# RUCAIBox/RecBole-CDR

Measured on AMD Instinct MI355X. Metric: training interactions/sec, higher is better.
Workload: dtype f32; 1 GPU; C5: EMCDR-BPR D=128, 50000000 users x 10000000 items/domain (union tables 71.7 GB fp32), step = source batch + target batch of 1048576 triples each per rank, fwd+bwd+row-wise adam; batch_per_domain_per_rank=1048576, k_neg=1, optimizer=rowwise-adam

## Files before the change

include/cdr_hip.h:

```cpp
#ifndef CDR_HIP_H
#define CDR_HIP_H

#include <stddef.h>
#include <stdint.h>

#ifdef __cplusplus
extern "C" {
#endif

#define CDR_OK 0
#define CDR_EINVAL (-1)
#define CDR_ENOMEM (-2)
#define CDR_ENODEV (-3)

typedef struct cdr_ctx cdr_ctx;

int cdr_ctx_create(int device, cdr_ctx** out);
int cdr_ctx_destroy(cdr_ctx* ctx);
const char* cdr_last_error(void);
int cdr_ctx_scrub_next(cdr_ctx* ctx, void* ptr, size_t bytes);
int cdr_ctx_set_id_counters(cdr_ctx* ctx, uint32_t* user_counts, int64_t user_rows, uint32_t* item_counts, int64_t item_rows,
                            void* list_ws, size_t list_ws_bytes);
int cdr_id_count_workspace_bytes(int64_t B, size_t* bytes);
int cdr_norm_rec_floats(void);
int cdr_row_norms_build(void* stream, const float* table, int64_t rows, int D, float* n2);
int cdr_ctx_set_norm_cache(cdr_ctx* ctx, float* user_n2, int64_t user_rows, float* item_n2, int64_t item_rows);
#define CDR_ABI_VERSION 64
int cdr_abi_version(void);

#define CDR_TAG_BPR_FWD 1
#define CDR_TAG_POINT_FWD 2
#define CDR_TAG_BPR_FWD_GRAD 3
#define CDR_TAG_APPLY_UNSIGNED 4
#define CDR_TAG_APPLY_SIGNED 5
#define CDR_TAG_SORT 6
#define CDR_TAG_POINT_FWD_GRAD 7
#define CDR_TAG_BPR_PARTIAL_DIFF 8
#define CDR_TAG_BPR_GRAD_FROM_DIFF 9
#define CDR_TAG_POINT_PARTIAL_DOT 10
#define CDR_TAG_POINT_GRAD_FROM_DOT 11
#define CDR_TAG_CONET_FWD 12
#define CDR_TAG_CONET_BWD 13
#define CDR_TAG_BPR_FWD_KMAJOR 15
#define CDR_TAG_MAP_STEP 16
#define CDR_TAG_CONET_WGRAD 14
#define CDR_TAG_OCC_FLAGS 17
#define CDR_TAG_BPR_FWD_APPLY 18
#define CDR_TAG_BATCH_NORMS 19
#define CDR_TAG_CONET_FB 20
#define CDR_TAG_TRIPLET_FWD_GRAD 21
#define CDR_TAG_CLFM_FWD_GRAD 22
#define CDR_TAG_DTCDR_FWD_GRAD 23
#define CDR_TAG_DEEPAPF_FWD_GRAD 24
#define CDR_TAG_DCDCSR_MAP_FWD_GRAD 25
int cdr_timing_enable(cdr_ctx* ctx, int capacity);
int cdr_timing_collect(cdr_ctx* ctx, int* tags, float* ms, int max_n, int* n_out);

int cdr_bpr_fwd(cdr_ctx* ctx, void* stream,
                const float* user_tab, const float* item_tab, int D,
                const int64_t* uid, const int64_t* pid, const int64_t* nid, int64_t B,
                float gamma, float reg_weight,
                float* out4, float* gcoef );

int cdr_bpr_bwd_dense(cdr_ctx* ctx, void* stream,
                      const float* user_tab, const float* item_tab, int D,
                      const int64_t* uid, const int64_t* pid, const int64_t* nid, int64_t B,
                      const float* gcoef, const float* out4, float reg_weight, const float* grad_out,
                      float* grad_user_tab, float* grad_item_tab);

#define CDR_LOSS_MSE 0
#define CDR_LOSS_BCE 1
int cdr_point_fwd(cdr_ctx* ctx, void* stream, int loss_kind,
                  const float* user_tab, const float* item_tab,
                  const float* reg_user_tab, const float* reg_item_tab, int D,
                  const int64_t* uid, const int64_t* iid, const float* label, int64_t B,
                  float reg_weight, float* out4, float* gcoef, float* scores);

int cdr_point_bwd_dense(cdr_ctx* ctx, void* stream,
                        const float* user_tab, const float* item_tab,
                        const float* reg_user_tab, const float* reg_item_tab, int D,
                        const int64_t* uid, const int64_t* iid, int64_t B,
                        const float* gcoef, const float* out4, float reg_weight, const float* grad_out,
                        float* grad_user_tab, float* grad_item_tab,
                        float* grad_reg_user_tab, float* grad_reg_item_tab);
int cdr_point_fwd_pair(cdr_ctx* ctx, void* stream, int loss_kind, const float* const* user_tab, const float* const* item_tab,
                       const float* const* reg_user_tab, const float* const* reg_item_tab, int D, const int64_t* const* uid,
                       const int64_t* const* iid, const float* const* label, const int64_t* B, const float* reg_weight,
                       float* const* out4, float* const* gcoef, float* const* scores, const float* w, float* total);
int cdr_point_fwd_pair_ex(cdr_ctx* ctx, void* stream, int loss_kind, const float* const* user_tab, const float* const* item_tab,
                          const float* const* reg_user_tab, const float* const* reg_item_tab, int D, int reg_D, const int64_t* const* uid,
                          const int64_t* const* iid, const float* const* label, const int64_t* B, const float* reg_weight,
                          float* const* out4, float* const* gcoef, float* const* scores, const float* w, float* total);
int cdr_point_bwd_dense_pair(cdr_ctx* ctx, void* stream, const float* const* user_tab, const float* const* item_tab,
                             const float* const* reg_user_tab, const float* const* reg_item_tab, int D, const int64_t* const* uid,
                             const int64_t* const* iid, const int64_t* B, const float* const* gcoef, const float* const* out4,
                             const float* reg_weight, const float* const* grad_out, const float* grad_scale,
                             float* const* grad_user_tab, float* const* grad_item_tab, float* const* grad_reg_user_tab,
                             float* const* grad_reg_item_tab);

int cdr_gather_rows(void* stream, const float* tab, int D, const int64_t* ids, int64_t n, float* out);
int cdr_scatter_add_rows(void* stream, float* grad_tab, int D, const int64_t* ids, int64_t n,
                         const float* src, const float* scale);
int cdr_gather_rows_multi(void* stream, int count, const float* const* tabs, int D, const int64_t* const* ids, const int64_t* n,
                          float* const* outs, int64_t* bump_counter);
int cdr_scatter_add_rows_multi(void* stream, int count, float* const* grad_tabs, int D, const int64_t* const* ids, const int64_t* n,
                               const float* const* srcs);

int cdr_select_mapped(void* stream, const float* mapped, const float* tab, int D,
                      const int64_t* ids, int64_t n, int64_t n_overlap, float* out);

#define CDR_ACT_NONE 0
#define CDR_ACT_TANH 1
#define CDR_ACT_RELU 2
#define CDR_ACT_SIGMOID 3
int cdr_gemm_f32(void* stream, int transA, int transB, int64_t M, int64_t N, int64_t K,
                 const float* A, int64_t lda, const float* B, int64_t ldb,
                 float* C, int64_t ldc, const float* bias, int act, int accumulate);

int cdr_fullsort_scores_f32(void* stream, const float* user_e, int64_t U, int D,
                            const float* slab0, int64_t n0, const float* slab1, int64_t n1,
                            float* scores );

int cdr_fullsort_topk_workspace_bytes(int64_t U, int D, int64_t n0, int64_t n1, int k, size_t* bytes);
int cdr_fullsort_topk_f32(void* stream, const float* user_e, int64_t U, int D,
                          const float* slab0, int64_t n0, const float* slab1, int64_t n1, int k,
                          const int64_t* hist_indptr, const int64_t* hist_cols, int exclude_first_col,
                          float* out_vals , int64_t* out_idx , void* workspace, size_t workspace_bytes);

int cdr_fullsort_neg_sqdist_f32(void* stream, const float* user_e, int64_t U, int D,
                                const float* items, int64_t N, float* norm_scratch, float* scores);

int cdr_row_sqnorm_f32(void* stream, const float* X, int64_t rows, int D, float* out );

int cdr_fullsort_neg_sqdist_topk_workspace_bytes(int64_t U, int D, int64_t n0, int64_t n1, int k, size_t* bytes);
int cdr_fullsort_neg_sqdist_topk_f32(void* stream, const float* user_e, int64_t U, int D,
                                     const float* slab0, int64_t n0, const float* slab1, int64_t n1,
                                     const float* col_sqnorm, int k,
                                     const int64_t* hist_indptr, const int64_t* hist_cols, int exclude_first_col,
                                     float* out_vals , int64_t* out_idx , void* workspace, size_t workspace_bytes);

int cdr_fullsort_rank_workspace_bytes(int64_t U, int D, int64_t n0, int64_t n1, int64_t P, size_t* bytes);
int cdr_fullsort_rank_f32(void* stream, const float* user_e, int64_t U, int D,
                          const float* slab0, int64_t n0, const float* slab1, int64_t n1,
                          const int64_t* pos_indptr , const int64_t* pos_cols ,
                          const int64_t* hist_indptr, const int64_t* hist_cols, int exclude_first_col,
                          float* pos_score , int32_t* gt, int32_t* eq, int32_t* eq_before ,
                          int32_t* n_unmasked , void* workspace, size_t workspace_bytes);
int cdr_fullsort_neg_sqdist_rank_workspace_bytes(int64_t U, int D, int64_t n0, int64_t n1, int64_t P, size_t* bytes);
int cdr_fullsort_neg_sqdist_rank_f32(void* stream, const float* user_e, int64_t U, int D,
                                     const float* slab0, int64_t n0, const float* slab1, int64_t n1, const float* col_sqnorm,
                                     const int64_t* pos_indptr , const int64_t* pos_cols ,
                                     const int64_t* hist_indptr, const int64_t* hist_cols, int exclude_first_col,
                                     float* pos_score , int32_t* gt, int32_t* eq, int32_t* eq_before ,
                                     int32_t* n_unmasked , void* workspace, size_t workspace_bytes);
int cdr_rank_rows_f32(void* stream, const float* scores, int64_t ld, int64_t U, int64_t N, int64_t col_off,
                      const int64_t* pos_indptr, const int64_t* pos_cols, const int64_t* hist_indptr, const int64_t* hist_cols,
                      int exclude_first_col, const float* pos_score, int32_t* gt, int32_t* eq, int32_t* eq_before,
                      int32_t* n_unmasked, int accumulate);

int cdr_fullsort_topk_wide_workspace_bytes(int64_t U, int D, int64_t n0, int64_t n1, int k, size_t* bytes);
int cdr_fullsort_topk_wide_f32(void* stream, const float* user_e, int64_t U, int D,
                               const float* slab0, int64_t n0, const float* slab1, int64_t n1, int k,
                               const int64_t* hist_indptr, const int64_t* hist_cols, int exclude_first_col,
                               float* out_vals , int64_t* out_idx , void* workspace, size_t workspace_bytes);
int cdr_fullsort_neg_sqdist_topk_wide_workspace_bytes(int64_t U, int D, int64_t n0, int64_t n1, int k, size_t* bytes);
int cdr_fullsort_neg_sqdist_topk_wide_f32(void* stream, const float* user_e, int64_t U, int D,
                                          const float* slab0, int64_t n0, const float* slab1, int64_t n1,
                                          const float* col_sqnorm, int k,
                                          const int64_t* hist_indptr, const int64_t* hist_cols, int exclude_first_col,
                                          float* out_vals , int64_t* out_idx , void* workspace, size_t workspace_bytes);
int cdr_topk_rows_workspace_bytes(int64_t U, int64_t N, int k, size_t* bytes);
int cdr_topk_rows_f32(void* stream, const float* scores, int64_t ld, int64_t U, int64_t N, int64_t col_off, int k,
                      const int64_t* hist_indptr, const int64_t* hist_cols, int exclude_first_col,
                      float* vals , int64_t* idx , int accumulate, void* workspace, size_t workspace_bytes);

int cdr_candidate_scores_f32(void* stream, const float* user_e, int64_t U, int D,
                             const float* slab0, int64_t n0, const float* slab1, int64_t n1,
                             const int64_t* cand_row , const int64_t* cand_cols , int64_t C, int form,
                             float* scores );
// ... 511 lines not shown
```

recbole-cdr_amd/binding.py:

```python
import contextlib
import ctypes
import gc
import os
import subprocess
import threading

import torch


@contextlib.contextmanager
def capturing(graph, stream):
    gc.collect()
    was = gc.isenabled()
    gc.disable()
    try:
        with torch.cuda.graph(graph, stream=stream):
            yield
    finally:
        if was:
            gc.enable()


_HERE = os.path.dirname(os.path.abspath(__file__))
_LIB_PATH = os.environ.get('CDR_LIB_PATH') or os.path.join(_HERE, 'lib', 'libcdrhip.so')
ABI_VERSION = 64
SIGNIN_WORDS = 288

CDR_LOSS_MSE, CDR_LOSS_BCE = 0, 1
ACT_NONE, ACT_TANH, ACT_RELU, ACT_SIGMOID = 0, 1, 2, 3


class NativeLibraryError(RuntimeError):
    pass


def lib_path():
    return _LIB_PATH


def build(force=False):
    csrc = os.path.join(_HERE, 'csrc')
    cmd = ['make', '-C', csrc, '-j', str(min(8, os.cpu_count() or 1))]
    if force:
        subprocess.run(['make', '-C', csrc, 'clean'], check=True, stdout=subprocess.DEVNULL)
    r = subprocess.run(cmd, stdout=subprocess.PIPE, stderr=subprocess.STDOUT, text=True)
    if r.returncode != 0:
        raise NativeLibraryError('building libcdrhip.so failed:\n' + r.stdout[-4000:])
    return _LIB_PATH


_c_i64, _c_int, _c_f32, _c_ptr = ctypes.c_int64, ctypes.c_int, ctypes.c_float, ctypes.c_void_p

_SIGNATURES = {
    'cdr_ctx_create': [_c_int, ctypes.POINTER(_c_ptr)],
    'cdr_ctx_destroy': [_c_ptr],
    'cdr_abi_version': [],
    'cdr_ctx_scrub_next': [_c_ptr, _c_ptr, ctypes.c_size_t],
    'cdr_ctx_set_id_counters': [_c_ptr, _c_ptr, _c_i64, _c_ptr, _c_i64, _c_ptr, ctypes.c_size_t],
    'cdr_id_count_workspace_bytes': [_c_i64, ctypes.POINTER(ctypes.c_size_t)],
    'cdr_norm_rec_floats': [],
    'cdr_row_norms_build': [_c_ptr, _c_ptr, _c_i64, _c_int, _c_ptr],
    'cdr_ctx_set_norm_cache': [_c_ptr, _c_ptr, _c_i64, _c_ptr, _c_i64],
    'cdr_bpr_fwd': [_c_ptr, _c_ptr, _c_ptr, _c_ptr, _c_int, _c_ptr, _c_ptr, _c_ptr, _c_i64, _c_f32, _c_f32, _c_ptr, _c_ptr],
    'cdr_bpr_bwd_dense': [_c_ptr, _c_ptr, _c_ptr, _c_ptr, _c_int, _c_ptr, _c_ptr, _c_ptr, _c_i64, _c_ptr, _c_ptr, _c_f32,
                          _c_ptr, _c_ptr, _c_ptr],
    'cdr_point_fwd': [_c_ptr, _c_ptr, _c_int, _c_ptr, _c_ptr, _c_ptr, _c_ptr, _c_int, _c_ptr, _c_ptr, _c_ptr, _c_i64,
                      _c_f32, _c_ptr, _c_ptr, _c_ptr],
    'cdr_point_bwd_dense': [_c_ptr, _c_ptr, _c_ptr, _c_ptr, _c_ptr, _c_ptr, _c_int, _c_ptr, _c_ptr, _c_i64, _c_ptr, _c_ptr,
                            _c_f32, _c_ptr, _c_ptr, _c_ptr, _c_ptr, _c_ptr],
    'cdr_gather_rows': [_c_ptr, _c_ptr, _c_int, _c_ptr, _c_i64, _c_ptr],
    'cdr_gather_rows_multi': [_c_ptr, _c_int, _c_ptr, _c_int, _c_ptr, _c_ptr, _c_ptr, _c_ptr],
    'cdr_scatter_add_rows_multi': [_c_ptr, _c_int, _c_ptr, _c_int, _c_ptr, _c_ptr, _c_ptr],
    'cdr_sscdr_map_loss': [_c_ptr, _c_ptr, _c_ptr, _c_ptr, _c_i64, _c_int, _c_f32, _c_f32, _c_f32, _c_ptr, _c_ptr, _c_ptr],
    'cdr_scale2_unless_one': [_c_ptr, _c_ptr, _c_ptr, _c_i64, _c_ptr, _c_i64],
    'cdr_scatter_add_rows': [_c_ptr, _c_ptr, _c_int, _c_ptr, _c_i64, _c_ptr, _c_ptr],
    'cdr_select_mapped': [_c_ptr, _c_ptr, _c_ptr, _c_int, _c_ptr, _c_i64, _c_i64, _c_ptr],
    'cdr_gemm_f32': [_c_ptr, _c_int, _c_int, _c_i64, _c_i64, _c_i64, _c_ptr, _c_i64, _c_ptr, _c_i64, _c_ptr, _c_i64, _c_ptr,
                     _c_int, _c_int],
    'cdr_fullsort_scores_f32': [_c_ptr, _c_ptr, _c_i64, _c_int, _c_ptr, _c_i64, _c_ptr, _c_i64, _c_ptr],
    'cdr_fullsort_neg_sqdist_f32': [_c_ptr, _c_ptr, _c_i64, _c_int, _c_ptr, _c_i64, _c_ptr, _c_ptr],
    'cdr_act_bwd': [_c_ptr, _c_int, _c_ptr, _c_ptr, _c_ptr, _c_i64],
    'cdr_colsum': [_c_ptr, _c_ptr, _c_ptr, _c_i64, _c_i64, _c_ptr, _c_int],
    'cdr_linear_wgrad_small': [_c_ptr, _c_ptr, _c_ptr, _c_ptr, _c_int, _c_ptr, _c_i64, _c_int, _c_int, _c_ptr, _c_ptr, _c_ptr, ctypes.c_size_t],
    'cdr_linear_wgrad_small_workspace': [_c_i64, _c_int, _c_int, ctypes.POINTER(ctypes.c_size_t)],
    'cdr_linear_small': [_c_ptr, _c_int, _c_ptr, _c_i64, _c_ptr, _c_i64, _c_i64, _c_int, _c_int, _c_ptr, _c_int, _c_ptr, _c_i64, _c_ptr, _c_int],
    'cdr_mse_fwd': [_c_ptr, _c_ptr, _c_ptr, _c_ptr, _c_i64, _c_ptr],
    'cdr_mse_bwd': [_c_ptr, _c_ptr, _c_ptr, _c_i64, _c_ptr, _c_ptr, _c_ptr],
    'cdr_bpr_fwd_grad': [_c_ptr, _c_ptr, _c_ptr, _c_ptr, _c_int, _c_ptr, _c_ptr, _c_ptr, _c_i64, _c_i64, _c_f32, _c_f32, _c_ptr,
                         _c_ptr, _c_ptr, _c_int],
    'cdr_loss_finish_sums': [_c_ptr, _c_ptr, _c_i64, _c_f32, _c_ptr],
    'cdr_triplet_fwd_grad': [_c_ptr, _c_ptr, _c_ptr, _c_ptr, _c_int, _c_ptr, _c_ptr, _c_ptr, _c_i64, _c_f32, _c_f32, _c_ptr, _c_ptr, _c_ptr],
    'cdr_clfm_fwd_grad_workspace_bytes': [_c_i64, _c_int, _c_int, ctypes.POINTER(ctypes.c_size_t)],
    'cdr_clfm_fwd_grad': [_c_ptr, _c_ptr, _c_ptr, _c_ptr, _c_int, _c_int, _c_ptr, _c_ptr, _c_ptr, _c_ptr, _c_i64, _c_f32, _c_f32, _c_ptr, _c_ptr,
                          _c_ptr, _c_ptr, _c_ptr, ctypes.c_size_t],
    'cdr_dtcdr_fwd_grad_workspace_bytes': [_c_i64, _c_int, _c_int, _c_ptr, ctypes.POINTER(ctypes.c_size_t)],
    'cdr_dtcdr_fwd_grad': [_c_ptr, _c_ptr, _c_ptr, _c_ptr, _c_ptr, _c_ptr, _c_int, _c_int, _c_ptr, _c_ptr, _c_ptr, _c_ptr, _c_ptr, _c_i64,
                           _c_f32, _c_f32, _c_ptr, ctypes.c_uint64, _c_i64, _c_ptr, _c_ptr, _c_ptr, _c_ptr, _c_ptr, _c_ptr, _c_ptr,
                           ctypes.c_size_t],
    'cdr_deepapf_fwd_grad_workspace_bytes': [_c_i64, _c_int, ctypes.POINTER(ctypes.c_size_t)],
    'cdr_deepapf_fwd_grad': [_c_ptr, _c_ptr, _c_ptr, _c_ptr, _c_ptr, _c_int, _c_ptr, _c_ptr, _c_ptr, _c_ptr, _c_i64, _c_i64, _c_f32, _c_i64,
                             _c_ptr, _c_ptr, _c_ptr, _c_ptr, _c_ptr, _c_ptr, ctypes.c_size_t],
    'cdr_dcdcsr_map_fwd_grad_workspace_bytes': [_c_i64, _c_int, ctypes.POINTER(_c_int), ctypes.POINTER(ctypes.c_size_t)],
    'cdr_dcdcsr_map_fwd_grad': [_c_ptr, _c_ptr, _c_ptr, _c_ptr, _c_ptr, _c_i64, _c_int, ctypes.POINTER(_c_int), _c_ptr, _c_ptr, _c_ptr, _c_ptr,
                                _c_ptr, ctypes.c_size_t],
    'cdr_bpr_step_fused_heads_words': [_c_i64, ctypes.POINTER(_c_i64)],
    'cdr_bpr_step_fused_kmajor_sizes': [_c_i64, _c_int, ctypes.POINTER(_c_i64), ctypes.POINTER(_c_i64)],
    'cdr_bpr_step_fused_kmajor': [_c_ptr, _c_ptr, _c_int, _c_ptr, _c_ptr, _c_ptr, _c_i64, _c_ptr, _c_ptr, _c_ptr, _c_i64, _c_int,
                                  _c_ptr, _c_ptr, _c_ptr, _c_i64, _c_int, _c_f32, _c_f32, _c_f32, _c_f32, _c_f32, _c_f32, _c_f32, _c_i64, _c_i64,
                                  _c_ptr, _c_ptr, _c_ptr, _c_ptr, _c_ptr, _c_ptr, _c_ptr, _c_ptr, ctypes.c_size_t],
    'cdr_bpr_step_fused': [_c_ptr, _c_ptr, _c_int, _c_ptr, _c_ptr, _c_ptr, _c_i64, _c_ptr, _c_ptr, _c_ptr, _c_i64, _c_int,
                           _c_ptr, _c_ptr, _c_ptr, _c_i64, _c_f32, _c_f32, _c_f32, _c_f32, _c_f32, _c_f32, _c_f32, _c_i64, _c_i64,
                           _c_ptr, _c_ptr, _c_ptr, _c_ptr, _c_ptr, _c_ptr, _c_ptr, _c_ptr, ctypes.c_size_t],
    'cdr_bpr_step_fused_dev': [_c_ptr, _c_ptr, _c_int, _c_ptr, _c_ptr, _c_ptr, _c_i64, _c_ptr, _c_ptr, _c_ptr, _c_i64, _c_int,
                               _c_ptr, _c_ptr, _c_ptr, _c_i64, _c_f32, _c_f32, _c_f32, _c_f32, _c_f32, _c_f32, _c_f32, _c_ptr, _c_ptr, _c_ptr,
                               _c_ptr, _c_ptr, _c_ptr, _c_ptr, _c_ptr, _c_ptr, _c_ptr, _c_ptr, ctypes.c_size_t],
    'cdr_bpr_step_presort': [_c_ptr, _c_ptr, _c_ptr, _c_ptr, _c_ptr, _c_i64, _c_i64, _c_i64, _c_ptr, _c_ptr, _c_ptr, _c_ptr, _c_ptr,
                             ctypes.c_size_t, _c_ptr],
    'cdr_bpr_step_from_diff': [_c_ptr, _c_ptr, _c_int, _c_ptr, _c_ptr, _c_ptr, _c_ptr, _c_ptr, _c_ptr, _c_int, _c_ptr, _c_ptr, _c_ptr, _c_i64,
                               _c_f32, _c_f32, _c_f32, _c_f32, _c_f32, _c_f32, _c_f32, _c_i64, _c_i64, _c_ptr, ctypes.c_uint32, _c_ptr, _c_ptr,
                               _c_ptr, _c_ptr, _c_ptr, _c_ptr, _c_ptr],
    'cdr_batch_norm_sums': [_c_ptr, _c_ptr, _c_ptr, _c_ptr, _c_int, _c_ptr, _c_ptr, _c_i64, _c_ptr],
    'cdr_bpr_shard_local_step': [_c_ptr, _c_ptr, _c_int, _c_ptr, _c_ptr, _c_ptr, _c_i64, _c_ptr, _c_int, _c_ptr, _c_ptr, _c_ptr, _c_i64, _c_i64,
                                 _c_f32, _c_f32, _c_f32, _c_f32, _c_f32, _c_f32, _c_f32, _c_i64, _c_ptr, _c_ptr, _c_ptr, _c_ptr, _c_ptr,
                                 _c_ptr, _c_ptr, _c_ptr, ctypes.c_size_t],
    'cdr_route_triples_workspace_bytes': [_c_i64, _c_int, ctypes.POINTER(ctypes.c_size_t)],
    'cdr_route_triples': [_c_ptr, _c_ptr, _c_ptr, _c_ptr, _c_ptr, _c_i64, _c_int, _c_ptr, _c_ptr, _c_ptr, ctypes.c_size_t],
    'cdr_bpr_shard_plan_sizes': [_c_i64, _c_i64, _c_i64, _c_int, ctypes.POINTER(_c_i64), ctypes.POINTER(ctypes.c_size_t)],
    'cdr_bpr_shard_plan': [_c_ptr, _c_ptr, _c_ptr, _c_i64, _c_i64, _c_i64, _c_int, _c_ptr, _c_ptr, _c_ptr, _c_ptr, _c_ptr, _c_ptr, _c_ptr, _c_ptr,
                           _c_ptr, _c_ptr, _c_ptr, ctypes.c_size_t],
    'cdr_gather_rows_norms': [_c_ptr, _c_ptr, _c_int, _c_ptr, _c_i64, _c_ptr, _c_ptr],
    'cdr_shard_norm_sums': [_c_ptr, _c_ptr, _c_ptr, _c_int, _c_ptr, _c_ptr, _c_ptr, _c_i64, _c_ptr],
    'cdr_bpr_shard_step': [_c_ptr, _c_ptr, _c_int, _c_ptr, _c_ptr, _c_ptr, _c_ptr, _c_int, _c_ptr, _c_ptr, _c_i64, _c_i64, _c_f32, _c_f32, _c_f32,
                           _c_f32, _c_f32, _c_f32, _c_f32, _c_i64, _c_ptr, _c_ptr, _c_ptr, _c_ptr, _c_ptr, _c_ptr, _c_ptr, _c_ptr, _c_ptr],
    'cdr_shard_owner_apply': [_c_ptr, _c_ptr, _c_int, _c_ptr, _c_ptr, _c_ptr, _c_i64, _c_int, _c_ptr, _c_i64, _c_int, _c_ptr, _c_f32, _c_f32, _c_f32,
                              _c_f32, _c_f32, _c_i64, _c_ptr, _c_ptr, _c_ptr, ctypes.c_size_t],
    'cdr_overlap_remap_dev_workspace_bytes': [_c_i64, _c_i64, ctypes.POINTER(ctypes.c_size_t)],
    'cdr_overlap_remap_dev': [_c_ptr, _c_ptr, _c_ptr, _c_ptr, _c_i64, _c_ptr, _c_ptr, _c_ptr, _c_i64, _c_ptr, _c_ptr, _c_ptr, _c_ptr,
                              ctypes.c_size_t, _c_ptr],
    'cdr_point_step_fused': [_c_ptr, _c_ptr, _c_int, _c_int, _c_ptr, _c_ptr, _c_ptr, _c_i64, _c_ptr, _c_ptr, _c_ptr, _c_i64, _c_int, _c_ptr, _c_ptr,
                             _c_ptr, _c_i64, _c_f32, _c_f32, _c_f32, _c_f32, _c_f32, _c_f32, _c_i64, _c_i64, _c_ptr, _c_ptr, _c_ptr, _c_ptr, _c_ptr,
                             _c_ptr, _c_ptr, _c_ptr, ctypes.c_size_t],
    'cdr_point_step_fused_pair_dev': [_c_ptr, _c_ptr, _c_int, _c_int, _c_ptr, _c_ptr, _c_ptr, _c_i64, _c_ptr, _c_ptr, _c_ptr, _c_i64, _c_int,
                                      _c_ptr, _c_ptr, _c_ptr, _c_i64, _c_ptr, _c_ptr, _c_ptr, _c_i64, _c_f32, _c_f32, _c_f32, _c_f32, _c_f32,
                                      _c_f32, _c_f32, _c_f32, _c_ptr, _c_ptr, _c_ptr, _c_ptr, _c_ptr, _c_ptr, _c_ptr, _c_ptr, _c_ptr, _c_ptr,
                                      _c_ptr, ctypes.c_size_t],
    'cdr_point_step_fused_pair': [_c_ptr, _c_ptr, _c_int, _c_int, _c_ptr, _c_ptr, _c_ptr, _c_i64, _c_ptr, _c_ptr, _c_ptr, _c_i64, _c_int,
                                  _c_ptr, _c_ptr, _c_ptr, _c_i64, _c_ptr, _c_ptr, _c_ptr, _c_i64, _c_f32, _c_f32, _c_f32, _c_f32, _c_f32,
                                  _c_f32, _c_ptr, _c_ptr, _c_ptr, _c_ptr, _c_ptr, _c_ptr, _c_ptr, _c_ptr, ctypes.c_size_t],
    'cdr_point_step_fused_kmajor': [_c_ptr, _c_ptr, _c_int, _c_int, _c_ptr, _c_ptr, _c_ptr, _c_i64, _c_ptr, _c_ptr, _c_ptr, _c_i64, _c_int, _c_ptr,
                                    _c_ptr, _c_ptr, _c_i64, _c_int, _c_f32, _c_f32, _c_f32, _c_f32, _c_f32, _c_f32, _c_i64, _c_i64, _c_ptr, _c_ptr, _c_ptr,
                                    _c_ptr, _c_ptr, _c_ptr, _c_ptr, _c_ptr, ctypes.c_size_t],
    'cdr_point_step_presort': [_c_ptr, _c_ptr, _c_ptr, _c_ptr, _c_i64, _c_i64, _c_i64, _c_ptr, _c_ptr, _c_ptr, _c_ptr, _c_ptr, ctypes.c_size_t, _c_ptr],
    'cdr_point_step_from_dot': [_c_ptr, _c_ptr, _c_int, _c_int, _c_ptr, _c_ptr, _c_ptr, _c_ptr, _c_ptr, _c_ptr, _c_int, _c_ptr, _c_ptr, _c_ptr, _c_i64,
                                _c_f32, _c_f32, _c_f32, _c_f32, _c_f32, _c_f32, _c_i64, _c_i64, _c_ptr, ctypes.c_uint32, _c_ptr, _c_ptr, _c_ptr,
                                _c_ptr, _c_ptr, _c_ptr, _c_ptr],
    'cdr_sort_workspace_bytes': [_c_i64, _c_i64, ctypes.POINTER(ctypes.c_size_t)],
    'cdr_timing_enable': [_c_ptr, _c_int],
    'cdr_timing_collect': [_c_ptr, ctypes.POINTER(_c_int), ctypes.POINTER(_c_f32), _c_int, ctypes.POINTER(_c_int)],
    'cdr_sort_ids': [_c_ptr, _c_ptr, _c_ptr, _c_i64, _c_ptr, _c_i64, _c_i64, _c_ptr, _c_ptr, _c_ptr, ctypes.c_size_t],
    'cdr_rowwise_apply': [_c_ptr, _c_ptr, _c_int, _c_ptr, _c_ptr, _c_ptr, _c_int, _c_ptr, _c_ptr, _c_i64, _c_ptr, _c_i64, _c_i64,
                          _c_ptr, _c_f32, _c_f32, _c_f32, _c_f32, _c_f32, _c_i64, _c_ptr, ctypes.c_uint32],
    'cdr_sort_ids_two_tables': [_c_ptr, _c_ptr, _c_ptr, _c_i64, _c_i64, _c_ptr, _c_i64, _c_ptr, _c_i64, _c_i64, _c_ptr, _c_ptr, _c_ptr,
                                _c_ptr, ctypes.c_size_t],
    'cdr_gemm_f32_ex': [_c_ptr, _c_int, _c_int, _c_i64, _c_i64, _c_i64, _c_ptr, _c_i64, _c_ptr, _c_i64, _c_ptr, _c_i64, _c_ptr,
                        _c_ptr, _c_int, _c_int],
    'cdr_gather_rows_ld': [_c_ptr, _c_ptr, _c_int, _c_ptr, _c_i64, _c_ptr, _c_i64],
    'cdr_scatter_add_rows_ld': [_c_ptr, _c_ptr, _c_int, _c_ptr, _c_i64, _c_ptr, _c_i64],
    'cdr_scatter_rows_sorted': [_c_ptr, _c_ptr, _c_int, _c_ptr, _c_ptr, _c_i64, _c_ptr, _c_i64],
    'cdr_ordered_bwd': [_c_ptr, _c_int, _c_ptr, _c_int],
    'cdr_overlap_mask': [_c_ptr, _c_ptr, _c_i64, _c_i64, _c_ptr],
    'cdr_rowscale': [_c_ptr, _c_ptr, _c_ptr, _c_i64, _c_i64, _c_ptr],
    'cdr_bcast_add_act': [_c_ptr, _c_ptr, _c_ptr, _c_i64, _c_i64, _c_int, _c_ptr],
    'cdr_bce_prob_fwd': [_c_ptr, _c_ptr, _c_ptr, _c_ptr, _c_i64, _c_ptr],
    'cdr_bce_prob_bwd': [_c_ptr, _c_ptr, _c_ptr, _c_i64, _c_ptr, _c_ptr],
    'cdr_frobenius_fwd': [_c_ptr, _c_ptr, _c_ptr, _c_i64, _c_ptr],
    'cdr_frobenius_bwd': [_c_ptr, _c_ptr, _c_i64, _c_ptr, _c_ptr, _c_ptr, _c_int],
    'cdr_sqnorm_normalize_fwd': [_c_ptr, _c_ptr, _c_i64, _c_int, _c_ptr, _c_ptr],
    'cdr_sqnorm_normalize_bwd': [_c_ptr, _c_ptr, _c_ptr, _c_ptr, _c_i64, _c_int, _c_ptr],
    'cdr_triplet_fwd': [_c_ptr, _c_ptr, _c_ptr, _c_ptr, _c_ptr, _c_i64, _c_int, _c_f32, _c_f32, _c_ptr, _c_ptr, _c_ptr],
    'cdr_triplet_bwd': [_c_ptr, _c_ptr, _c_ptr, _c_ptr, _c_i64, _c_int, _c_f32, _c_f32, _c_ptr, _c_ptr, _c_ptr, _c_ptr, _c_ptr,
                        _c_ptr],
    'cdr_spmm_csr_f32': [_c_ptr, _c_ptr, _c_ptr, _c_ptr, _c_i64, _c_ptr, _c_int, _c_ptr],
    'cdr_graph_layer_fwd': [_c_ptr, _c_ptr, _c_ptr, _c_ptr, _c_i64, _c_ptr, _c_int, _c_ptr, _c_ptr, _c_ptr],
    'cdr_graph_layer_bwd': [_c_ptr, _c_ptr, _c_ptr, _c_ptr, _c_i64, _c_ptr, _c_ptr, _c_ptr, _c_int, _c_ptr, _c_ptr, _c_ptr],
    'cdr_row_flags': [_c_ptr, _c_int, _c_ptr, _c_ptr, _c_ptr, _c_i64, _c_ptr, ctypes.c_size_t],
    'cdr_row_flags_layout': [_c_i64, _c_ptr],
    'cdr_graph_layer_fwd_rows': [_c_ptr, _c_ptr, _c_ptr, _c_ptr, _c_i64, _c_ptr, _c_ptr, _c_int, _c_ptr, _c_ptr],
    'cdr_mul_one_plus': [_c_ptr, _c_ptr, _c_ptr, _c_i64, _c_ptr],
    'cdr_graph_layer_bwd_rows': [_c_ptr, _c_ptr, _c_ptr, _c_ptr, _c_i64, _c_ptr, _c_ptr, _c_ptr, _c_int, _c_ptr],
    'cdr_transfer_fwd': [_c_ptr, _c_ptr, _c_ptr, _c_ptr, _c_ptr, _c_i64, _c_int, _c_i64, _c_f32, _c_f32, _c_ptr, _c_ptr],
    'cdr_transfer_bwd': [_c_ptr, _c_ptr, _c_ptr, _c_ptr, _c_ptr, _c_i64, _c_int, _c_i64, _c_f32, _c_f32, _c_ptr, _c_ptr],
    'cdr_bitgcf_mix_fwd': [_c_ptr] * 7 + [_c_i64, _c_i64, _c_int, _c_i64, _c_i64, _c_f32, _c_f32, _c_f32, ctypes.c_uint64, _c_ptr, ctypes.c_uint64,
                           ctypes.c_uint64, _c_ptr, _c_ptr, _c_ptr, _c_ptr, _c_i64, _c_ptr, _c_ptr, _c_ptr],
    'cdr_bitgcf_mix_bwd': [_c_ptr] * 7 + [_c_i64, _c_ptr, _c_ptr, _c_ptr, _c_ptr, _c_ptr, _c_ptr, _c_i64, _c_i64, _c_int, _c_i64, _c_i64, _c_f32, _c_f32,
                           _c_f32, ctypes.c_uint64, _c_ptr, ctypes.c_uint64, ctypes.c_uint64, _c_ptr, _c_ptr, _c_ptr],
    'cdr_transfer_drop_fwd': [_c_ptr, _c_ptr, _c_ptr, _c_ptr, _c_ptr, _c_i64, _c_int, _c_i64, _c_f32, _c_f32, _c_f32, ctypes.c_uint64, _c_ptr,
                              ctypes.c_uint64, ctypes.c_uint64, _c_i64, _c_ptr, _c_ptr],
    'cdr_transfer_drop_bwd': [_c_ptr, _c_ptr, _c_ptr, _c_ptr, _c_ptr, _c_i64, _c_int, _c_i64, _c_f32, _c_f32, _c_f32, ctypes.c_uint64, _c_ptr,
                              ctypes.c_uint64, ctypes.c_uint64, _c_i64, _c_ptr, _c_ptr],
    'cdr_l2_normalize_fwd': [_c_ptr, _c_ptr, _c_i64, _c_int, _c_ptr, _c_i64, _c_ptr],
    'cdr_l2_normalize_bwd': [_c_ptr, _c_ptr, _c_ptr, _c_ptr, _c_i64, _c_i64, _c_int, _c_ptr, _c_int],
    'cdr_copy_cols': [_c_ptr, _c_ptr, _c_i64, _c_i64, _c_int, _c_ptr, _c_i64, _c_int],
    'cdr_bitgcf_stack': [_c_ptr] * 5 + [_c_i64, _c_i64, _c_int, _c_ptr, _c_ptr, _c_ptr, _c_ptr, _c_i64],
    'cdr_bitgcf_unstack_bwd': [_c_ptr, _c_ptr, _c_ptr, _c_i64, _c_i64, _c_int, _c_ptr, _c_ptr],
    'cdr_colblock_mean_fwd': [_c_ptr, _c_ptr, _c_i64, _c_int, _c_int, _c_ptr],
    'cdr_colblock_mean_bwd': [_c_ptr, _c_ptr, _c_i64, _c_int, _c_int, _c_ptr],
    'cdr_dropout_dev': [_c_ptr, _c_ptr, _c_i64, _c_f32, _c_ptr, ctypes.c_uint64, _c_ptr],
    'cdr_gather_max2': [_c_ptr, _c_ptr, _c_ptr, _c_int, _c_ptr, _c_i64, _c_ptr, _c_i64],
    'cdr_gather_max2_bwd': [_c_ptr, _c_ptr, _c_ptr, _c_int, _c_ptr, _c_i64, _c_ptr, _c_i64, _c_ptr, _c_ptr],
    'cdr_apf_prod': [_c_ptr, _c_ptr, _c_ptr, _c_ptr, _c_i64, _c_int, _c_ptr],
    'cdr_apf_prod_bwd': [_c_ptr, _c_ptr, _c_ptr, _c_ptr, _c_ptr, _c_i64, _c_int, _c_ptr, _c_ptr, _c_ptr],
    'cdr_apf_combine': [_c_ptr, _c_ptr, _c_ptr, _c_ptr, _c_ptr, _c_ptr, _c_ptr, _c_i64, _c_i64, _c_int, _c_ptr, _c_ptr],
    'cdr_apf_combine_bwd': [_c_ptr, _c_ptr, _c_ptr, _c_ptr, _c_ptr, _c_ptr, _c_ptr, _c_ptr, _c_i64, _c_int, _c_ptr, _c_ptr, _c_ptr,
                            _c_ptr, _c_ptr],
    'cdr_maxmin_norm': [_c_ptr, _c_ptr, _c_i64, _c_int, _c_ptr, _c_ptr],
# ... 288 lines not shown
```

recbole-cdr_amd/csrc/cdr_common.h:

```cpp
#pragma once
#include <hip/hip_runtime.h>
#include <stdint.h>
#include <stdio.h>
#include "../../include/cdr_hip.h"

#define CDR_WAVE 64
#define CDR_NUM_CU 256
#define CDR_MAX_PARTIAL_BLOCKS 4096
#define CDR_PARTIAL_STRIDE 8
#define CDR_TICKETS 1024
constexpr int kBlock = 256;

struct cdr_ctx {
    int device;
    double* partials;
    unsigned* tickets;
    void* scratch;
    size_t scratch_bytes;
    void* scrub_ptr;
    size_t scrub_bytes;
    uint32_t* idc_user; int64_t idc_user_rows;
    uint32_t* idc_item; int64_t idc_item_rows;
    void* idc_list; size_t idc_list_bytes;
    float* n2_user; int64_t n2_user_rows;
    float* n2_item; int64_t n2_item_rows;
    unsigned long long* conet_tab_dev; unsigned long long* conet_tab_pin; unsigned long long* conet_tab_shadow; int conet_tab_cap, conet_tab_n;
    int conet_defer, conet_pending, conet_fin_grid;
    int64_t conet_fin_ns, conet_fin_R;
    float* conet_fin_out;
    void* conet_fin_stream;
    int timing_cap, timing_n;
    hipEvent_t* ev0;
    hipEvent_t* ev1;
    int* tags;
};

struct cdr_time_scope {
    cdr_ctx* c; hipStream_t s; int slot;
    cdr_time_scope(cdr_ctx* ctx, int tag, hipStream_t st) : c(ctx), s(st), slot(-1) {
        if (c && c->timing_cap > 0 && c->timing_n < c->timing_cap) {
            slot = c->timing_n++;
            c->tags[slot] = tag;
            (void)hipEventRecord(c->ev0[slot], s);
        }
    }
    ~cdr_time_scope() { if (slot >= 0) (void)hipEventRecord(c->ev1[slot], s); }
};

void cdr_set_error(const char* fmt, ...);
int cdr_ctx_scratch(cdr_ctx* ctx, size_t bytes, void** out);

#define CDR_CHECK_ARG(cond)                                                         \
    do {                                                                            \
        if (!(cond)) {                                                              \
            cdr_set_error("%s: invalid argument: %s", __func__, #cond);             \
            return CDR_EINVAL;                                                      \
        }                                                                           \
    } while (0)

#define CDR_HIP(expr)                                                               \
    do {                                                                            \
        hipError_t e_ = (expr);                                                     \
        if (e_ != hipSuccess) {                                                     \
            cdr_set_error("%s: %s -> %s", __func__, #expr, hipGetErrorString(e_));  \
            return (int)e_;                                                         \
        }                                                                           \
    } while (0)

#define CDR_LAUNCH_CHECK()                                                          \
    do {                                                                            \
        hipError_t e_ = hipGetLastError();                                          \
        if (e_ != hipSuccess) {                                                     \
            cdr_set_error("%s: launch failed: %s", __func__, hipGetErrorString(e_));\
            return (int)e_;                                                         \
        }                                                                           \
    } while (0)

template <int CTRL>
__device__ __forceinline__ float dpp_add_(float v) {
    return v + __int_as_float(__builtin_amdgcn_update_dpp(0, __float_as_int(v), CTRL, 0xF, 0xF, true));
}
template <int LPR>
__device__ __forceinline__ float group_sum(float v) {
    if (LPR >= 2) v = dpp_add_<0xB1>(v);
    if (LPR >= 4) v = dpp_add_<0x4E>(v);
    if (LPR >= 8) v = dpp_add_<0x141>(v);
    if (LPR >= 16) v = dpp_add_<0x140>(v);
    if (LPR >= 32) {
        const auto r = __builtin_amdgcn_permlane16_swap(__float_as_uint(v), __float_as_uint(v), false, false);
        v = __uint_as_float(r[0]) + __uint_as_float(r[1]);
    }
    if (LPR >= 64) {
        const auto r = __builtin_amdgcn_permlane32_swap(__float_as_uint(v), __float_as_uint(v), false, false);
        v = __uint_as_float(r[0]) + __uint_as_float(r[1]);
    }
    return v;
}

__device__ __forceinline__ double wave_sum_d(double v) {
#pragma unroll
    for (int off = 32; off > 0; off >>= 1) v += __shfl_xor(v, off, CDR_WAVE);
    return v;
}

template <int NV>
__device__ __forceinline__ void block_sum_d(double (&v)[NV], double* smem) {
    const int lane = threadIdx.x & 63, wave = threadIdx.x >> 6, nw = blockDim.x >> 6;
#pragma unroll
    for (int i = 0; i < NV; ++i) v[i] = wave_sum_d(v[i]);
    if (lane == 0) {
#pragma unroll
        for (int i = 0; i < NV; ++i) smem[wave * NV + i] = v[i];
    }
    __syncthreads();
    if (threadIdx.x == 0) {
#pragma unroll
        for (int i = 0; i < NV; ++i) {
            double s = 0.0;
            for (int w = 0; w < nw; ++w) s += smem[w * NV + i];
            v[i] = s;
        }
    }
}

static __global__ void cdr_zero_u32_kernel(uint32_t* __restrict__ p, int64_t n) {
    for (int64_t i = (int64_t)blockIdx.x * blockDim.x + threadIdx.x; i < n; i += (int64_t)gridDim.x * blockDim.x) p[i] = 0u;
}
static inline hipError_t cdr_zero_u32(void* p, int64_t n_words, hipStream_t s) {
    int64_t g = (n_words + 255) / 256;
    if (g > 1024) g = 1024;
    if (g < 1) g = 1;
    cdr_zero_u32_kernel<<<dim3((unsigned)g), dim3(256), 0, s>>>((uint32_t*)p, n_words);
    return hipGetLastError();
}

#if defined(__HIP_DEVICE_COMPILE__) && !defined(__gfx950__)
#error "cdr_common.h: the fence-free partial hand-over (cdr_sign_in_last) is only valid on gfx950; add __threadfence() pairs for another target"
#endif
__device__ __forceinline__ void cdr_store_sys(double* p, double v) { __hip_atomic_store(p, v, __ATOMIC_RELAXED, __HIP_MEMORY_SCOPE_SYSTEM); }
__device__ __forceinline__ double cdr_load_sys(const double* p) { return __hip_atomic_load(p, __ATOMIC_RELAXED, __HIP_MEMORY_SCOPE_SYSTEM); }
__device__ __forceinline__ bool cdr_sign_in_last(unsigned* ticket, unsigned nblocks) {
    __shared__ int cdr_last_flag_;
    asm volatile("s_waitcnt vmcnt(0)" ::: "memory");
    __syncthreads();
    if (threadIdx.x == 0) cdr_last_flag_ = atomicInc(ticket, nblocks - 1) == nblocks - 1 ? 1 : 0;
    __syncthreads();
    return cdr_last_flag_ != 0;
}
constexpr unsigned kSignGroups = 8, kSignStride = 32;
__device__ __forceinline__ bool cdr_sign_in_last_wide(unsigned* ticket, unsigned nblocks) {
    __shared__ int cdr_last_flag_w_;
    asm volatile("s_waitcnt vmcnt(0)" ::: "memory");
    __syncthreads();
    if (threadIdx.x == 0) {
        const unsigned bid = blockIdx.y * gridDim.x + blockIdx.x;
        const unsigned K = nblocks < kSignGroups ? nblocks : kSignGroups;
        const unsigned g = bid % K, ng = (nblocks - g + K - 1) / K;
        int last = 0;
        if (atomicInc(ticket + kSignStride * (1 + g), ng - 1) == ng - 1) last = atomicInc(ticket, K - 1) == K - 1 ? 1 : 0;
        cdr_last_flag_w_ = last;
    }
    __syncthreads();
    return cdr_last_flag_w_ != 0;
}
__device__ __forceinline__ void cdr_scrub(uint4* __restrict__ z, int64_t n16) {
    if (!z) return;
    const int64_t nth = (int64_t)gridDim.x * gridDim.y * blockDim.x;
    const int64_t me = ((int64_t)blockIdx.y * gridDim.x + blockIdx.x) * blockDim.x + threadIdx.x;
    const uint4 zero = make_uint4(0u, 0u, 0u, 0u);
    for (int64_t i = me; i < n16; i += nth) z[i] = zero;
}
static inline void cdr_take_scrub(cdr_ctx* ctx, uint4** z, int64_t* n16) {
    *z = (uint4*)ctx->scrub_ptr; *n16 = (int64_t)(ctx->scrub_bytes / 16);
    ctx->scrub_ptr = nullptr; ctx->scrub_bytes = 0;
}
constexpr int kSignInMaxBlocks = 512;

__device__ __forceinline__ float4 ld4(const float* p) { return *reinterpret_cast<const float4*>(p); }
// ... 65 lines not shown
```

recbole-cdr_amd/csrc/cdr_ctx.hip:

```cpp
#include <stdarg.h>
#include <string.h>
#include "cdr_common.h"
#include <stdlib.h>

static thread_local char g_err[512] = "";

void cdr_set_error(const char* fmt, ...) {
    va_list ap;
    va_start(ap, fmt);
    vsnprintf(g_err, sizeof(g_err), fmt, ap);
    va_end(ap);
}

extern "C" const char* cdr_last_error(void) { return g_err; }
extern "C" int cdr_abi_version(void) { return CDR_ABI_VERSION; }

extern "C" int cdr_ctx_create(int device, cdr_ctx** out) {
    CDR_CHECK_ARG(out != nullptr);
    *out = nullptr;
    int ndev = 0;
    if (hipGetDeviceCount(&ndev) != hipSuccess || device < 0 || device >= ndev) {
        cdr_set_error("cdr_ctx_create: device %d not available (%d visible)", device, ndev);
        return CDR_ENODEV;
    }
    int prev = 0;
    CDR_HIP(hipGetDevice(&prev));
    CDR_HIP(hipSetDevice(device));
    cdr_ctx* c = new cdr_ctx();
    c->device = device;
    c->timing_cap = c->timing_n = 0;
    c->ev0 = c->ev1 = nullptr;
    c->tags = nullptr;
    c->scratch = nullptr;
    c->scratch_bytes = 0;
    c->scrub_ptr = nullptr; c->scrub_bytes = 0;
    c->idc_user = c->idc_item = nullptr; c->idc_user_rows = c->idc_item_rows = 0; c->idc_list = nullptr; c->idc_list_bytes = 0;
    c->n2_user = c->n2_item = nullptr; c->n2_user_rows = c->n2_item_rows = 0;
    c->partials = nullptr;
    c->tickets = nullptr;
    hipError_t e = hipMalloc(&c->partials, sizeof(double) * CDR_MAX_PARTIAL_BLOCKS * CDR_PARTIAL_STRIDE);
    if (e == hipSuccess) e = hipMalloc(&c->tickets, sizeof(unsigned) * CDR_TICKETS);
    if (e == hipSuccess) e = hipMemset(c->tickets, 0, sizeof(unsigned) * CDR_TICKETS);
    (void)hipSetDevice(prev);
    if (e != hipSuccess) {
        if (c->partials) (void)hipFree(c->partials);
        if (c->tickets) (void)hipFree(c->tickets);
        delete c;
        cdr_set_error("cdr_ctx_create: scratch allocation failed: %s", hipGetErrorString(e));
        return CDR_ENOMEM;
    }
    *out = c;
    return CDR_OK;
}

int cdr_ctx_scratch(cdr_ctx* ctx, size_t bytes, void** out) {
    if (ctx->scratch_bytes < bytes) {
        int prev = 0;
        CDR_HIP(hipGetDevice(&prev));
        CDR_HIP(hipSetDevice(ctx->device));
        if (ctx->scratch) (void)hipFree(ctx->scratch);
        ctx->scratch = nullptr; ctx->scratch_bytes = 0;
        const size_t want = bytes + bytes / 4;
        hipError_t e = hipMalloc(&ctx->scratch, want);
        (void)hipSetDevice(prev);
        if (e != hipSuccess) { cdr_set_error("cdr_ctx_scratch: %zu bytes: %s", want, hipGetErrorString(e)); return CDR_ENOMEM; }
        ctx->scratch_bytes = want;
    }
    *out = ctx->scratch;
    return CDR_OK;
}

extern "C" int cdr_timing_enable(cdr_ctx* ctx, int capacity) {
    CDR_CHECK_ARG(ctx && capacity >= 0);
    for (int i = 0; i < ctx->timing_cap; ++i) { (void)hipEventDestroy(ctx->ev0[i]); (void)hipEventDestroy(ctx->ev1[i]); }
    delete[] ctx->ev0; delete[] ctx->ev1; delete[] ctx->tags;
    ctx->ev0 = ctx->ev1 = nullptr; ctx->tags = nullptr;
    ctx->timing_cap = ctx->timing_n = 0;
    if (capacity == 0) return CDR_OK;
    ctx->ev0 = new hipEvent_t[capacity];
    ctx->ev1 = new hipEvent_t[capacity];
    ctx->tags = new int[capacity];
    for (int i = 0; i < capacity; ++i) { CDR_HIP(hipEventCreate(&ctx->ev0[i])); CDR_HIP(hipEventCreate(&ctx->ev1[i])); }
    ctx->timing_cap = capacity;
    return CDR_OK;
}

extern "C" int cdr_timing_collect(cdr_ctx* ctx, int* tags, float* ms, int max_n, int* n_out) {
    CDR_CHECK_ARG(ctx && tags && ms && n_out && max_n >= 0);
    int n = ctx->timing_n < max_n ? ctx->timing_n : max_n;
    for (int i = 0; i < n; ++i) {
        CDR_HIP(hipEventSynchronize(ctx->ev1[i]));
        CDR_HIP(hipEventElapsedTime(&ms[i], ctx->ev0[i], ctx->ev1[i]));
        tags[i] = ctx->tags[i];
    }
    *n_out = n;
    ctx->timing_n = 0;
    return CDR_OK;
}

extern "C" int cdr_ctx_destroy(cdr_ctx* ctx) {
    if (!ctx) return CDR_OK;
    cdr_timing_enable(ctx, 0);
    if (ctx->partials) (void)hipFree(ctx->partials);
    if (ctx->tickets) (void)hipFree(ctx->tickets);
    if (ctx->scratch) (void)hipFree(ctx->scratch);
    if (ctx->conet_tab_dev) (void)hipFree(ctx->conet_tab_dev);
    if (ctx->conet_tab_pin) (void)hipHostFree(ctx->conet_tab_pin);
    free(ctx->conet_tab_shadow);
    delete ctx;
    return CDR_OK;
}

extern "C" int cdr_ctx_scrub_next(cdr_ctx* ctx, void* ptr, size_t bytes) {
    CDR_CHECK_ARG(ctx && ptr && bytes > 0 && (bytes & 15) == 0 && ((uintptr_t)ptr & 15) == 0);
    ctx->scrub_ptr = ptr; ctx->scrub_bytes = bytes;
    return CDR_OK;
}

extern "C" int cdr_ctx_set_id_counters(cdr_ctx* ctx, uint32_t* user_counts, int64_t user_rows, uint32_t* item_counts, int64_t item_rows,
                                       void* list_ws, size_t list_ws_bytes) {
    CDR_CHECK_ARG(ctx != nullptr);
    if (!user_counts || !item_counts || !list_ws) {
        ctx->idc_user = ctx->idc_item = nullptr; ctx->idc_user_rows = ctx->idc_item_rows = 0; ctx->idc_list = nullptr; ctx->idc_list_bytes = 0;
        return CDR_OK;
    }
    CDR_CHECK_ARG(user_rows > 0 && item_rows > 0 && list_ws_bytes > 0);
    ctx->idc_user = user_counts; ctx->idc_user_rows = user_rows; ctx->idc_item = item_counts; ctx->idc_item_rows = item_rows;
    ctx->idc_list = list_ws; ctx->idc_list_bytes = list_ws_bytes;
    return CDR_OK;
}

extern "C" int cdr_ctx_set_norm_cache(cdr_ctx* ctx, float* user_n2, int64_t user_rows, float* item_n2, int64_t item_rows) {
    CDR_CHECK_ARG(ctx != nullptr);
    if (!user_n2 || !item_n2) {
        ctx->n2_user = ctx->n2_item = nullptr; ctx->n2_user_rows = ctx->n2_item_rows = 0;
        return CDR_OK;
    }
    const uintptr_t rec = (uintptr_t)cdr_norm_rec_floats() * sizeof(float);
    CDR_CHECK_ARG(user_rows > 0 && item_rows > 0 && (uintptr_t)user_n2 % rec == 0 && (uintptr_t)item_n2 % rec == 0);
    ctx->n2_user = user_n2; ctx->n2_user_rows = user_rows; ctx->n2_item = item_n2; ctx->n2_item_rows = item_rows;
    return CDR_OK;
}
```

recbole-cdr_amd/csrc/cdr_step.hip:

```cpp
#include <cstdlib>
#include <cstring>
#include <string.h>
#include <rocprim/device/device_radix_sort.hpp>
#include <rocprim/device/device_scan.hpp>
#include <rocprim/iterator/counting_iterator.hpp>
#include <rocprim/iterator/transform_iterator.hpp>
#include "cdr_common.h"
#include "cdr_adam_math.h"
#include "cdr_opt_math.h"
#include "cdr_loss_math.h"

namespace {

constexpr int kUnroll = 4;

#ifndef CDR_NORM_REC_FLOATS
#define CDR_NORM_REC_FLOATS 16
#endif
constexpr int kNormRecFloats = CDR_NORM_REC_FLOATS;
static_assert(kNormRecFloats == 16 || kNormRecFloats == 32, "a record is one 64-byte or one 128-byte burst");

template <int LPR>
__device__ __forceinline__ float sqnorm4(float4 a) {
    if constexpr (LPR >= 32) {
// ... 112 lines not shown
                v[r] = ld4n<(LPR >= 32)>(I + ii[r] * D + 4 * sub);
            }
        }
#pragma unroll
        for (int r = 0; r < kUnroll; ++r) {
            const int64_t t = base + (int64_t)r * TG;
            const float dx = group_sum<LPR>(dot4(u[r], v[r]));
            const float su = group_sum<LPR>(dot4(u[r], u[r]));
            const float si = group_sum<LPR>(dot4(v[r], v[r]));
            if (t < B) {
                const float y = yl[r];
                float l, g;
                if (loss_kind == CDR_LOSS_MSE) {
                    const float d = dx - y;
                    l = d * d; g = 2.0f * d * invB;
                } else {
                    const float p = sigmoidf_(dx);
                    l = (y - 1.0f) * fmaxf(logf(1.0f - p), -100.0f) - y * fmaxf(logf(p), -100.0f);
                    const float pq = (1.0f - p) * p;
                    g = (p - y) / fmaxf(pq, 1e-12f) * invB * pq;
                }
                if (live) {
                    st4n<(LPR >= 32)>(GU + t * D + 4 * sub, make_float4(g * v[r].x, g * v[r].y, g * v[r].z, g * v[r].w));
                    st4n<(LPR >= 32)>(GI + t * D + 4 * sub, make_float4(g * u[r].x, g * u[r].y, g * u[r].z, g * u[r].w));
                }
                if (sub == 0) { acc[0] += (double)l; acc[1] += (double)su; acc[2] += (double)si; }
            }
        }
    }
    block_sum_d<3>(acc, smem);
    if (threadIdx.x == 0) store_partials(partials, acc);
}

template <int LPR>
__device__ __forceinline__ float4 sqnorm_bwd4(float4 x, float4 g, float L) {
    const float d = group_sum<LPR>(dot4(x, g));
    return make_float4(sqnorm_bwd_elem(x.x, g.x, L, d), sqnorm_bwd_elem(x.y, g.y, L, d), sqnorm_bwd_elem(x.z, g.z, L, d),
                       sqnorm_bwd_elem(x.w, g.w, L, d));
}

template <int LPR>
__global__ __launch_bounds__(kBlock) void triplet_fwd_grad_kernel(const float* __restrict__ U, const float* __restrict__ I, int D,
                                                                  const int64_t* __restrict__ uid, const int64_t* __restrict__ pid,
                                                                  const int64_t* __restrict__ nid, int64_t B, float margin, float eps,
                                                                  float invB, float* __restrict__ GU, float* __restrict__ GI,
                                                                  double* __restrict__ partials) {
    constexpr int GPB = kBlock / LPR;
    __shared__ double smem[2 * (kBlock / 64)];
    const int sub = threadIdx.x % LPR;
    const int64_t gg = (int64_t)blockIdx.x * GPB + threadIdx.x / LPR;
    const int64_t TG = (int64_t)gridDim.x * GPB;
    const int D4 = D >> 2;
    double acc[2] = {0.0, 0.0};
    const bool live = sub < D4;
    const float e = live ? eps : 0.f;

    for (int64_t base = gg; base < B; base += TG * kUnroll) {
        float4 u[kUnroll], p[kUnroll], n[kUnroll];
        int64_t iu[kUnroll], ip[kUnroll], in[kUnroll];
#pragma unroll
        for (int r = 0; r < kUnroll; ++r) {
            const int64_t t = base + (int64_t)r * TG;
            const int64_t tc = t < B ? t : B - 1;
            iu[r] = uid[tc]; ip[r] = pid[tc]; in[r] = nid[tc];
        }
#pragma unroll
        for (int r = 0; r < kUnroll; ++r) {
            const int64_t t = base + (int64_t)r * TG;
            u[r] = p[r] = n[r] = make_float4(0.f, 0.f, 0.f, 0.f);
            if (t < B && live) {
                u[r] = ld4n<(LPR >= 32)>(U + iu[r] * D + 4 * sub);
                p[r] = ld4n<(LPR >= 32)>(I + ip[r] * D + 4 * sub);
                n[r] = ld4n<(LPR >= 32)>(I + in[r] * D + 4 * sub);
            }
        }
#pragma unroll
        for (int r = 0; r < kUnroll; ++r) {
            const int64_t t = base + (int64_t)r * TG;
            const float Lu = group_sum<LPR>(dot4(u[r], u[r]));
            const float Lp = group_sum<LPR>(dot4(p[r], p[r]));
            const float Ln = group_sum<LPR>(dot4(n[r], n[r]));
            const float su = sqnorm_scale(Lu), sp = sqnorm_scale(Lp), sn = sqnorm_scale(Ln);
            const float4 yu = make_float4(u[r].x / su, u[r].y / su, u[r].z / su, u[r].w / su);
            const float4 dp = make_float4(yu.x - p[r].x / sp + e, yu.y - p[r].y / sp + e, yu.z - p[r].z / sp + e, yu.w - p[r].w / sp + e);
            const float4 dn = make_float4(yu.x - n[r].x / sn + e, yu.y - n[r].y / sn + e, yu.z - n[r].z / sn + e, yu.w - n[r].w / sn + e);
            const float d1 = sqrtf(group_sum<LPR>(dot4(dp, dp)));
            const float d2 = sqrtf(group_sum<LPR>(dot4(dn, dn)));
            bool on;
            const float hinge = triplet_hinge(d1, d2, margin, on);
            const float4 u1 = make_float4(unit_dir(on, dp.x, d1), unit_dir(on, dp.y, d1), unit_dir(on, dp.z, d1), unit_dir(on, dp.w, d1));
            const float4 u2 = make_float4(unit_dir(on, dn.x, d2), unit_dir(on, dn.y, d2), unit_dir(on, dn.z, d2), unit_dir(on, dn.w, d2));
            const float4 gu = sqnorm_bwd4<LPR>(u[r], scale_diff4(invB, u1, u2), Lu);
            const float4 gp = sqnorm_bwd4<LPR>(p[r], neg_scale4(invB, u1), Lp);
            const float4 gn = sqnorm_bwd4<LPR>(n[r], scale4(invB, u2), Ln);
            if (t < B) {
                if (live) {
                    st4n<(LPR >= 32)>(GU + t * D + 4 * sub, gu);
                    st4n<(LPR >= 32)>(GI + t * D + 4 * sub, gp);
                    st4n<(LPR >= 32)>(GI + (B + t) * D + 4 * sub, gn);
                }
                if (sub == 0) {
                    acc[0] += (double)hinge;
                    acc[1] += on ? 1.0 : 0.0;
                }
            }
        }
    }
    block_sum_d<2>(acc, smem);
    if (threadIdx.x == 0) store_partials(partials, acc);
}

__global__ __launch_bounds__(kBlock) void triplet_finish_kernel(const double* __restrict__ partials, int nblocks, int64_t B,
                                                                float* __restrict__ out3) {
    __shared__ double smem[2 * (kBlock / 64)];
    double acc[2] = {0.0, 0.0};
    sum_partials<2, kBlock>(partials, nblocks, acc, smem);
    if (threadIdx.x == 0) {
        out3[0] = (float)(acc[0] / (double)B);
        out3[1] = (float)acc[1];
        out3[2] = 0.f;
    }
}

__global__ __launch_bounds__(kBlock) void step_finish_kernel(const double* __restrict__ partials, int nblocks, int64_t B,
                                                             float reg_weight, float* __restrict__ out6) {
    __shared__ double smem[3 * (kBlock / 64)];
    double acc[3] = {0.0, 0.0, 0.0};
    sum_partials<3, kBlock>(partials, nblocks, acc, smem);
    if (threadIdx.x == 0) {
        const float main_loss = (float)(acc[0] / (double)B);
        const float nu = (float)sqrt(acc[1]), ni = (float)sqrt(acc[2]);
        out6[1] = main_loss; out6[2] = nu; out6[3] = ni;
        out6[0] = main_loss + reg_weight * ((nu + ni) / (float)B);
        out6[4] = embloss_coef(reg_weight, B, nu);
        out6[5] = embloss_coef(reg_weight, B, ni);
        out6[6] = (float)acc[0]; out6[7] = (float)acc[1]; out6[8] = (float)acc[2];
    }
}

__global__ void finish_sums_kernel(const float* __restrict__ sums3, int64_t B, float reg_weight, float* __restrict__ out6) {
    if (threadIdx.x == 0 && blockIdx.x == 0) {
        const float main_loss = sums3[0] / (float)B;
        const float nu = sqrtf(sums3[1]), ni = sqrtf(sums3[2]);
        out6[1] = main_loss; out6[2] = nu; out6[3] = ni;
        out6[0] = main_loss + reg_weight * ((nu + ni) / (float)B);
        out6[4] = embloss_coef(reg_weight, B, nu);
        out6[5] = embloss_coef(reg_weight, B, ni);
    }
}

__device__ __forceinline__ void sort_state_clear(uint32_t* __restrict__ zspan, int64_t zwords) {
    if (!zspan) return;
    for (int64_t i = (int64_t)blockIdx.x * blockDim.x + threadIdx.x; i < zwords; i += (int64_t)gridDim.x * blockDim.x) zspan[i] = 0u;
}

__global__ __launch_bounds__(kBlock) void make_keys_kernel(const int64_t* __restrict__ ids0, int64_t n0,
                                                           const int64_t* __restrict__ ids1, int64_t n1,
                                                           uint32_t* __restrict__ keys, uint32_t* __restrict__ vals,
                                                           uint32_t* __restrict__ zspan, int64_t zwords) {
    sort_state_clear(zspan, zwords);
    const int64_t n = n0 + n1, stride = (int64_t)gridDim.x * kBlock;
    for (int64_t e = (int64_t)blockIdx.x * kBlock + threadIdx.x; e < n; e += stride) {
        keys[e] = (uint32_t)(e < n0 ? ids0[e] : ids1[e - n0]);
        vals[e] = (uint32_t)e;
    }
}

constexpr int kLongSeg = 32;
constexpr int kPiece = 256;

struct seg_long { int64_t head, len, base; };
struct seg_piece { int64_t start; int64_t len; };

struct apply_hp { float lr, b1, b2, eps, wd, step_size, bc2_sqrt; const float* dev; };
#define HP_FROM_DEV(h) do { if ((h).dev) { (h).step_size = (h).dev[0]; (h).bc2_sqrt = (h).dev[1]; } } while (0)

template <int LPR, int OPT>
__device__ __forceinline__ float4 apply_update(float* __restrict__ wp, float* __restrict__ mp, float* __restrict__ vp, float4 w,
                                               float4 acc, float rc, const apply_hp& h) {
    float4 gr = make_float4(acc.x + rc * w.x, acc.y + rc * w.y, acc.z + rc * w.z, acc.w + rc * w.w);
    float4 wn;
    if constexpr (OPT == 2) {
        float4 sm = ld4n<(LPR >= 32)>(vp);
        if (h.wd != 0.f) { gr.x += h.wd * w.x; gr.y += h.wd * w.y; gr.z += h.wd * w.z; gr.w += h.wd * w.w; }
        wn = make_float4(cdr_adagrad_elem(w.x, gr.x, sm.x, h.lr, h.eps, 0.f), cdr_adagrad_elem(w.y, gr.y, sm.y, h.lr, h.eps, 0.f),
                         cdr_adagrad_elem(w.z, gr.z, sm.z, h.lr, h.eps, 0.f), cdr_adagrad_elem(w.w, gr.w, sm.w, h.lr, h.eps, 0.f));
        st4n<(LPR >= 32)>(vp, sm);
    } else if (OPT == 0) {
        if (h.wd != 0.f) { gr.x += h.wd * w.x; gr.y += h.wd * w.y; gr.z += h.wd * w.z; gr.w += h.wd * w.w; }
        wn = make_float4(w.x - h.lr * gr.x, w.y - h.lr * gr.y, w.z - h.lr * gr.z, w.w - h.lr * gr.w);
    } else {
        float4 m = ld4n<(LPR >= 32)>(mp), v = ld4n<(LPR >= 32)>(vp);
        if (h.wd != 0.f) { gr.x += h.wd * w.x; gr.y += h.wd * w.y; gr.z += h.wd * w.z; gr.w += h.wd * w.w; }
        m.x += (gr.x - m.x) * (1.0f - h.b1); m.y += (gr.y - m.y) * (1.0f - h.b1);
        m.z += (gr.z - m.z) * (1.0f - h.b1); m.w += (gr.w - m.w) * (1.0f - h.b1);
        v.x = h.b2 * v.x + (1.0f - h.b2) * gr.x * gr.x; v.y = h.b2 * v.y + (1.0f - h.b2) * gr.y * gr.y;
        v.z = h.b2 * v.z + (1.0f - h.b2) * gr.z * gr.z; v.w = h.b2 * v.w + (1.0f - h.b2) * gr.w * gr.w;
        st4n<(LPR >= 32)>(mp, m); st4n<(LPR >= 32)>(vp, v);
        wn = make_float4(w.x - cdr_adam_term(m.x, v.x, h.step_size, h.bc2_sqrt, h.eps), w.y - cdr_adam_term(m.y, v.y, h.step_size, h.bc2_sqrt, h.eps),
                         w.z - cdr_adam_term(m.z, v.z, h.step_size, h.bc2_sqrt, h.eps), w.w - cdr_adam_term(m.w, v.w, h.step_size, h.bc2_sqrt, h.eps));
    }
    st4n<(LPR >= 32)>(wp, wn);
    return wn;
}

template <int LPR, int OPT, bool SIGNED>
__global__ __launch_bounds__(kBlock) void rowwise_apply_kernel(float* __restrict__ W, float* __restrict__ Mo,
                                                               float* __restrict__ Vo, int D,
                                                               const uint32_t* __restrict__ keys,
                                                               const uint32_t* __restrict__ perm, int64_t n,
                                                               const float* __restrict__ G, int64_t neg_start,
                                                               int64_t reg_limit, const float* __restrict__ reg_coef,
                                                               apply_hp hp, const int64_t* __restrict__ occ_ids,
                                                               unsigned* __restrict__ counters, seg_long* __restrict__ longs,
                                                               seg_piece* __restrict__ pieces) {
    HP_FROM_DEV(hp);
    constexpr int GPB = kBlock / LPR;
    const int sub = threadIdx.x % LPR;
    const int64_t gg = (int64_t)blockIdx.x * GPB + threadIdx.x / LPR;
    const int64_t TG = (int64_t)gridDim.x * GPB;
    const int D4 = D >> 2;
    const float c = reg_coef ? reg_coef[0] : 0.f;
    for (int64_t q = gg; q < n; q += TG) {
        const uint32_t row = keys[q];
        const uint32_t before = keys[q > 0 ? q - 1 : 0];
        const uint32_t far = keys[q + kLongSeg < n ? q + kLongSeg : n - 1];
        const bool head = !(q > 0 && before == row);
        const bool is_long = q + kLongSeg < n && far == row;
        if (head && !is_long) {
            for (int ch = sub; ch < D4; ch += LPR) {
                float* wp = W + (int64_t)row * D + 4 * ch;
                const float4 w = ld4n<(LPR >= 32)>(wp);
                float4 acc = make_float4(0.f, 0.f, 0.f, 0.f);
                int cnt = 0;
                for (int64_t e = q; e < n && keys[e] == row; ++e) {
                    const int64_t o = perm[e];
                    const bool neg = SIGNED && o >= neg_start;
                    const float4 g = ld4n<(LPR >= 32)>(G + (neg ? o - neg_start : o) * D + 4 * ch);
                    if (neg) { acc.x -= g.x; acc.y -= g.y; acc.z -= g.z; acc.w -= g.w; }
                    else { acc.x += g.x; acc.y += g.y; acc.z += g.z; acc.w += g.w; }
                    cnt += occ_ids ? (int)((occ_ids[o] >> 62) & 1) : ((o < reg_limit) ? 1 : 0);
                }
                apply_update<LPR, OPT>(wp, OPT == 1 ? Mo + (int64_t)row * D + 4 * ch : nullptr, OPT ? Vo + (int64_t)row * D + 4 * ch : nullptr,
                                  w, acc, c * (float)cnt, hp);
            }
        }
    }
    if (counters == nullptr) return;
    for (int64_t q = (int64_t)blockIdx.x * kBlock + threadIdx.x; q + kLongSeg < n; q += (int64_t)gridDim.x * kBlock) {
        const uint32_t row = keys[q];
        const uint32_t before = keys[q > 0 ? q - 1 : 0];
        const uint32_t far = keys[q + kLongSeg];
        if ((q > 0 && before == row) || far != row) continue;
        int64_t lo = q + kLongSeg, hi = n;
        while (lo + 1 < hi) {
            const int64_t mid = (lo + hi) >> 1;
            if (keys[mid] == row) lo = mid; else hi = mid;
        }
        const int64_t len = hi - q;
        const unsigned np = (unsigned)((len + kPiece - 1) / kPiece);
        const unsigned base = atomicAdd(&counters[0], np);
        const unsigned li = atomicAdd(&counters[1], 1u);
        longs[li] = seg_long{q, len, (int64_t)base};
        for (unsigned k = 0; k < np; ++k) {
            const int64_t st = q + (int64_t)k * kPiece;
            pieces[base + k] = seg_piece{st, (hi - st) < kPiece ? (hi - st) : (int64_t)kPiece};
        }
    }
}

constexpr int kSubPiece = 32, kSubs = kPiece / kSubPiece;
template <int LPR, bool SIGNED>
__device__ __forceinline__ void seg_piece_sum_body(int D, const uint32_t* __restrict__ perm,
                                                   const float* __restrict__ G, int64_t neg_start, int64_t reg_limit,
                                                   const int64_t* __restrict__ occ_ids,
                                                   const unsigned* __restrict__ counters,
                                                   const seg_piece* __restrict__ pieces, float* __restrict__ partial,
                                                   int* __restrict__ pcnt) {
    constexpr int GPB = kBlock / LPR;
    constexpr int UN = 16;
    __shared__ float4 sub_sum[kSubs][64];
    __shared__ int sub_cnt[kSubs];
    const int sub = threadIdx.x % LPR, gid = threadIdx.x / LPR;
    const int D4 = D >> 2;
    const int64_t np = counters[0];
    for (int64_t pi = blockIdx.x; pi < np; pi += gridDim.x) {
        const seg_piece pc = pieces[pi];
        for (int ch0 = 0; ch0 < D4; ch0 += 64) {
            for (int sp = gid; sp < kSubs; sp += GPB) {
                const int64_t s0 = (int64_t)sp * kSubPiece, slen = pc.len - s0 < kSubPiece ? pc.len - s0 : (int64_t)kSubPiece;
                int cnt = 0;
                for (int ch = ch0 + sub; ch < D4 && ch < ch0 + 64; ch += LPR) {
                    float4 acc = make_float4(0.f, 0.f, 0.f, 0.f);
                    cnt = 0;
                    for (int64_t e0 = 0; e0 < slen; e0 += UN) {
                        int64_t o[UN]; float4 g[UN]; bool neg[UN];
#pragma unroll
                        for (int j = 0; j < UN; ++j) o[j] = (e0 + j < slen) ? (int64_t)perm[pc.start + s0 + e0 + j] : -1;
#pragma unroll
                        for (int j = 0; j < UN; ++j) {
                            neg[j] = SIGNED && o[j] >= neg_start;
                            g[j] = o[j] >= 0 ? ld4n<(LPR >= 32)>(G + (neg[j] ? o[j] - neg_start : o[j]) * D + 4 * ch) : make_float4(0.f, 0.f, 0.f, 0.f);
                        }
#pragma unroll
                        for (int j = 0; j < UN; ++j) {
                            if (o[j] < 0) continue;
                            if (neg[j]) { acc.x -= g[j].x; acc.y -= g[j].y; acc.z -= g[j].z; acc.w -= g[j].w; }
                            else { acc.x += g[j].x; acc.y += g[j].y; acc.z += g[j].z; acc.w += g[j].w; }
                            cnt += occ_ids ? (int)((occ_ids[o[j]] >> 62) & 1) : ((o[j] < reg_limit) ? 1 : 0);
                        }
                    }
                    sub_sum[sp][ch - ch0] = acc;
                }
                if (sub == 0 && ch0 == 0) sub_cnt[sp] = slen > 0 ? cnt : 0;
            }
            __syncthreads();
            const int nsub = (int)((pc.len + kSubPiece - 1) / kSubPiece);
            for (int c = threadIdx.x; c < 64 && ch0 + c < D4; c += kBlock) {
                float4 acc = sub_sum[0][c];
                for (int sp = 1; sp < nsub; ++sp) { const float4 x = sub_sum[sp][c]; acc.x += x.x; acc.y += x.y; acc.z += x.z; acc.w += x.w; }
                st4n<(LPR >= 32)>(partial + pi * D + 4 * (ch0 + c), acc);
            }
            if (threadIdx.x == 0 && ch0 == 0) {
                int cn = 0;
                for (int sp = 0; sp < nsub; ++sp) cn += sub_cnt[sp];
                pcnt[pi] = cn;
            }
            __syncthreads();
        }
    }
}
template <int LPR, bool SIGNED>
__global__ __launch_bounds__(kBlock) void seg_piece_sum_kernel(int D, const uint32_t* __restrict__ perm,
                                                               const float* __restrict__ G, int64_t neg_start, int64_t reg_limit,
                                                               const int64_t* __restrict__ occ_ids,
                                                               const unsigned* __restrict__ counters,
                                                               const seg_piece* __restrict__ pieces, float* __restrict__ partial,
                                                               int* __restrict__ pcnt) {
    seg_piece_sum_body<LPR, SIGNED>(D, perm, G, neg_start, reg_limit, occ_ids, counters, pieces, partial, pcnt);
}

template <int LPR, int OPT, bool NC = false>
__device__ __forceinline__ void seg_long_finish_body(float* __restrict__ W, float* __restrict__ Mo, float* __restrict__ Vo,
                                                     int D, const uint32_t* __restrict__ keys,
                                                     const float* __restrict__ reg_coef, apply_hp hp,
                                                     const unsigned* __restrict__ counters,
                                                     const seg_long* __restrict__ longs,
                                                     const float* __restrict__ partial, const int* __restrict__ pcnt,
                                                     float* __restrict__ n2 = nullptr) {
    HP_FROM_DEV(hp);
    constexpr int GPB = kBlock / LPR;
    const int sub = threadIdx.x % LPR;
    const int64_t gg = (int64_t)blockIdx.x * GPB + threadIdx.x / LPR;
    const int64_t TG = (int64_t)gridDim.x * GPB;
    const int D4 = D >> 2;
    const float c = reg_coef ? reg_coef[0] : 0.f;
    const int64_t nl = counters[1];
    for (int64_t li = gg; li < nl; li += TG) {
        const seg_long sg = longs[li];
        const uint32_t row = keys[sg.head];
        const int64_t np = (sg.len + kPiece - 1) / kPiece;
        float4 wnew = make_float4(0.f, 0.f, 0.f, 0.f);
        for (int ch = sub; ch < D4; ch += LPR) {
            float* wp = W + (int64_t)row * D + 4 * ch;
            const float4 w = ld4n<(LPR >= 32)>(wp);
            float4 acc = make_float4(0.f, 0.f, 0.f, 0.f);
            int cnt = 0;
            for (int64_t k0 = 0; k0 < np; k0 += 8) {
                float4 g[8]; int c[8];
#pragma unroll
                for (int j = 0; j < 8; ++j) {
                    const bool in = k0 + j < np;
                    g[j] = in ? ld4n<(LPR >= 32)>(partial + (sg.base + k0 + j) * D + 4 * ch) : make_float4(0.f, 0.f, 0.f, 0.f);
                    c[j] = in ? pcnt[sg.base + k0 + j] : 0;
                }
#pragma unroll
                for (int j = 0; j < 8; ++j) {
                    if (k0 + j < np) { acc.x += g[j].x; acc.y += g[j].y; acc.z += g[j].z; acc.w += g[j].w; cnt += c[j]; }
                }
            }
            wnew = apply_update<LPR, OPT>(wp, OPT == 1 ? Mo + (int64_t)row * D + 4 * ch : nullptr, OPT ? Vo + (int64_t)row * D + 4 * ch : nullptr,
                                          w, acc, c * (float)cnt, hp);
        }
        if (NC) norm_rec_store<LPR>(n2 + (int64_t)row * kNormRecFloats, group_sum<LPR>(sqnorm4<LPR>(wnew)), sub);
    }
}
template <int LPR, int OPT>
__global__ __launch_bounds__(kBlock) void seg_long_finish_kernel(float* __restrict__ W, float* __restrict__ Mo, float* __restrict__ Vo,
                                                                 int D, const uint32_t* __restrict__ keys,
                                                                 const float* __restrict__ reg_coef, apply_hp hp,
                                                                 const unsigned* __restrict__ counters,
                                                                 const seg_long* __restrict__ longs,
                                                                 const float* __restrict__ partial, const int* __restrict__ pcnt) {
    seg_long_finish_body<LPR, OPT>(W, Mo, Vo, D, keys, reg_coef, hp, counters, longs, partial, pcnt);
}

__global__ __launch_bounds__(kBlock) void make_keys2_kernel(const int64_t* __restrict__ a, int64_t na, const int64_t* __restrict__ b0,
                                                            int64_t nb0, const int64_t* __restrict__ b1, int64_t nb1, uint32_t key_base,
                                                            uint32_t* __restrict__ keys, uint32_t* __restrict__ vals,
                                                            uint32_t* __restrict__ zspan, int64_t zwords) {
    sort_state_clear(zspan, zwords);
    const int64_t n = na + nb0 + nb1, stride = (int64_t)gridDim.x * kBlock;
    for (int64_t e = (int64_t)blockIdx.x * kBlock + threadIdx.x; e < n; e += stride) {
        if (e < na) { keys[e] = (uint32_t)a[e]; vals[e] = (uint32_t)e; }
        else {
            const int64_t o = e - na;
            keys[e] = key_base + (uint32_t)(o < nb0 ? b0[o] : b1[o - nb0]);
            vals[e] = (uint32_t)o;
        }
    }
}

constexpr unsigned kSortBlock = 1024, kSortItems = 8, kSortRadixBits = 9, kSortRadix = 1u << kSortRadixBits;
constexpr unsigned kSortMaxPlaces = (32 + kSortRadixBits - 1) / kSortRadixBits;
using sort_offs_t = size_t;

__global__ __launch_bounds__(kSortBlock) void make_keys2_offsets_kernel(const int64_t* __restrict__ a, int64_t na, const int64_t* __restrict__ b0,
                                                                        int64_t nb0, const int64_t* __restrict__ b1, int64_t nb1,
                                                                        uint32_t key_base, uint32_t* __restrict__ keys, uint32_t* __restrict__ vals,
                                                                        uint32_t* __restrict__ zspan, int64_t zwords,
                                                                        sort_offs_t* __restrict__ counts, unsigned* __restrict__ ticket, unsigned places) {
    constexpr unsigned kStripes = 4;
    __shared__ unsigned hist[kSortMaxPlaces * kSortRadix * kStripes];
    sort_state_clear(zspan, zwords);
    const unsigned tid = threadIdx.x, bins = places * kSortRadix;
    for (unsigned i = tid; i < bins * kStripes; i += kSortBlock) hist[i] = 0u;
    __syncthreads();
    const unsigned stripe = tid % kStripes;
    const int64_t n = na + nb0 + nb1, stride = (int64_t)gridDim.x * kSortBlock;
    for (int64_t e = (int64_t)blockIdx.x * kSortBlock + tid; e < n; e += stride) {
        uint32_t k, v;
        if (e < na) { k = (uint32_t)a[e]; v = (uint32_t)e; }
        else {
            const int64_t o = e - na;
            k = key_base + (uint32_t)(o < nb0 ? b0[o] : b1[o - nb0]);
            v = (uint32_t)o;
        }
        keys[e] = k; vals[e] = v;
        for (unsigned p = 0; p < places; ++p) {
            const unsigned digit = (k >> (p * kSortRadixBits)) & (kSortRadix - 1u);
            atomicAdd(&hist[(p * kSortRadix + digit) * kStripes + stripe], 1u);
        }
    }
    __syncthreads();
    for (unsigned i = tid; i < bins; i += kSortBlock) {
        unsigned t = 0;
#pragma unroll
        for (unsigned j = 0; j < kStripes; ++j) t += hist[i * kStripes + j];
        if (t) atomicAdd(reinterpret_cast<unsigned long long*>(counts + i), (unsigned long long)t);
    }
    if (!cdr_sign_in_last(ticket, gridDim.x)) return;
    unsigned* sc = hist;
    for (unsigned p = 0; p < places; ++p) {
        unsigned c = 0;
        if (tid < kSortRadix) {
            c = (unsigned)__hip_atomic_load(reinterpret_cast<unsigned long long*>(counts + p * kSortRadix + tid), __ATOMIC_RELAXED, __HIP_MEMORY_SCOPE_AGENT);
            sc[tid] = c;
        }
        __syncthreads();
        for (unsigned d = 1; d < kSortRadix; d <<= 1) {
            const unsigned t = (tid < kSortRadix && tid >= d) ? sc[tid - d] : 0u;
            __syncthreads();
            if (tid < kSortRadix) sc[tid] += t;
            __syncthreads();
        }
        if (tid < kSortRadix) counts[p * kSortRadix + tid] = (sort_offs_t)(sc[tid] - c);
        __syncthreads();
    }
}


struct tab_ptrs { float* W; float* M; float* V; };

template <int OPT>
__device__ __forceinline__ float4 upd_math(float4 w, float4& m, float4& v, float4 acc, float rc, const apply_hp& h) {
    float4 gr = make_float4(acc.x + rc * w.x, acc.y + rc * w.y, acc.z + rc * w.z, acc.w + rc * w.w);
    if (h.wd != 0.f) { gr.x += h.wd * w.x; gr.y += h.wd * w.y; gr.z += h.wd * w.z; gr.w += h.wd * w.w; }
    if (OPT == 0) return make_float4(w.x - h.lr * gr.x, w.y - h.lr * gr.y, w.z - h.lr * gr.z, w.w - h.lr * gr.w);
    if constexpr (OPT == 2)
        return make_float4(cdr_adagrad_elem(w.x, gr.x, v.x, h.lr, h.eps, 0.f), cdr_adagrad_elem(w.y, gr.y, v.y, h.lr, h.eps, 0.f),
                           cdr_adagrad_elem(w.z, gr.z, v.z, h.lr, h.eps, 0.f), cdr_adagrad_elem(w.w, gr.w, v.w, h.lr, h.eps, 0.f));
    m.x += (gr.x - m.x) * (1.0f - h.b1); m.y += (gr.y - m.y) * (1.0f - h.b1);
    m.z += (gr.z - m.z) * (1.0f - h.b1); m.w += (gr.w - m.w) * (1.0f - h.b1);
    v.x = h.b2 * v.x + (1.0f - h.b2) * gr.x * gr.x; v.y = h.b2 * v.y + (1.0f - h.b2) * gr.y * gr.y;
    v.z = h.b2 * v.z + (1.0f - h.b2) * gr.z * gr.z; v.w = h.b2 * v.w + (1.0f - h.b2) * gr.w * gr.w;
    return make_float4(w.x - cdr_adam_term(m.x, v.x, h.step_size, h.bc2_sqrt, h.eps), w.y - cdr_adam_term(m.y, v.y, h.step_size, h.bc2_sqrt, h.eps),
                       w.z - cdr_adam_term(m.z, v.z, h.step_size, h.bc2_sqrt, h.eps), w.w - cdr_adam_term(m.w, v.w, h.step_size, h.bc2_sqrt, h.eps));
}

template <int LPR, int OPT>
__device__ __forceinline__ void row_moments(const tab_ptrs& T, int64_t off, float4& m, float4& v) {
    if constexpr (OPT == 1) { m = ld4n<(LPR >= 32)>(T.M + off); v = ld4n<(LPR >= 32)>(T.V + off); }
    if constexpr (OPT == 2) v = ld4n<(LPR >= 32)>(T.V + off);
}
template <int LPR, int OPT>
__device__ __forceinline__ void row_store(const tab_ptrs& T, int64_t off, float4 w, const float4& m, const float4& v) {
    if constexpr (OPT == 1) { st4n<(LPR >= 32)>(T.M + off, m); st4n<(LPR >= 32)>(T.V + off, v); }
    if constexpr (OPT == 2) st4n<(LPR >= 32)>(T.V + off, v);
    st4n<(LPR >= 32)>(T.W + off, w);
}

template <int LPR>
__global__ __launch_bounds__(kBlock) void batch_norms_kernel(const float* __restrict__ U, const float* __restrict__ I, int D,
                                                             const int64_t* __restrict__ uid, const int64_t* __restrict__ pid, int64_t B,
                                                             double* __restrict__ partials) {
    constexpr int GPB = kBlock / LPR;
    constexpr int UNR = 8;
    __shared__ double smem[2 * (kBlock / 64)];
    const int sub = threadIdx.x % LPR;
    const int64_t gg = (int64_t)blockIdx.x * GPB + threadIdx.x / LPR;
    const int64_t TG = (int64_t)gridDim.x * GPB;
    const bool live = sub < (D >> 2);
    double acc[2] = {0.0, 0.0};
    for (int64_t base = gg; base < B; base += TG * UNR) {
        int64_t iu[UNR], ip[UNR];
        float4 u[UNR], p[UNR];
#pragma unroll
        for (int r = 0; r < UNR; ++r) {
            const int64_t t = base + (int64_t)r * TG;
            const int64_t tc = t < B ? t : B - 1;
            iu[r] = uid[tc]; ip[r] = pid[tc];
        }
#pragma unroll
        for (int r = 0; r < UNR; ++r) {
            const int64_t t = base + (int64_t)r * TG;
            u[r] = p[r] = make_float4(0.f, 0.f, 0.f, 0.f);
            if (t < B && live) { u[r] = ld4n<(LPR >= 32)>(U + iu[r] * D + 4 * sub); p[r] = ld4n<(LPR >= 32)>(I + ip[r] * D + 4 * sub); }
        }
#pragma unroll
        for (int r = 0; r < UNR; ++r) {
            const float su = group_sum<LPR>(dot4(u[r], u[r])), sp = group_sum<LPR>(dot4(p[r], p[r]));
            if (sub == 0) { acc[0] += (double)su; acc[1] += (double)sp; }
        }
    }
    block_sum_d<2>(acc, smem);
    if (threadIdx.x == 0) store_partials(partials, acc);
}

template <int LPR>
__global__ __launch_bounds__(kBlock) void batch_norms_cached_kernel(const float* __restrict__ NU, const float* __restrict__ NI,
                                                                    const int64_t* __restrict__ uid, const int64_t* __restrict__ pid, int64_t B,
                                                                    double* __restrict__ partials) {
    constexpr int GPB = kBlock / LPR;
    constexpr int UNR = 8;
    __shared__ double smem[2 * (kBlock / 64)];
    const int sub = threadIdx.x % LPR;
    const int64_t gg = (int64_t)blockIdx.x * GPB + threadIdx.x / LPR;
    const int64_t TG = (int64_t)gridDim.x * GPB;
    double acc[2] = {0.0, 0.0};
    for (int64_t base = gg; base < B; base += TG * UNR) {
        int64_t iu[UNR], ip[UNR];
        float su[UNR], sp[UNR];
#pragma unroll
        for (int r = 0; r < UNR; ++r) {
            const int64_t t = base + (int64_t)r * TG;
            const int64_t tc = t < B ? t : B - 1;
            iu[r] = uid[tc]; ip[r] = pid[tc];
        }
#pragma unroll
        for (int r = 0; r < UNR; ++r) {
            const int64_t t = base + (int64_t)r * TG;
            su[r] = sp[r] = 0.f;
            if (t < B && sub == 0) { su[r] = NU[iu[r] * kNormRecFloats]; sp[r] = NI[ip[r] * kNormRecFloats]; }
        }
#pragma unroll
        for (int r = 0; r < UNR; ++r) {
            if (sub == 0) { acc[0] += (double)su[r]; acc[1] += (double)sp[r]; }
        }
    }
    block_sum_d<2>(acc, smem);
    if (threadIdx.x == 0) store_partials(partials, acc);
}

template <int LPR>
__global__ __launch_bounds__(kBlock) void row_norms_build_kernel(const float* __restrict__ W, int64_t rows, int D, float* __restrict__ n2) {
    constexpr int GPB = kBlock / LPR;
    const int sub = threadIdx.x % LPR;
    const int64_t gg = (int64_t)blockIdx.x * GPB + threadIdx.x / LPR;
    const int64_t TG = (int64_t)gridDim.x * GPB;
    const bool live = sub < (D >> 2);
    for (int64_t base = gg; base < rows; base += TG * kUnroll) {
        float4 w[kUnroll];
#pragma unroll
        for (int r = 0; r < kUnroll; ++r) {
            const int64_t row = base + (int64_t)r * TG;
            w[r] = (row < rows && live) ? ld4n<(LPR >= 32)>(W + row * D + 4 * sub) : make_float4(0.f, 0.f, 0.f, 0.f);
        }
#pragma unroll
        for (int r = 0; r < kUnroll; ++r) {
            const int64_t row = base + (int64_t)r * TG;
            const float s = group_sum<LPR>(sqnorm4<LPR>(w[r]));
            if (row < rows) norm_rec_store<LPR>(n2 + row * kNormRecFloats, s, sub);
        }
    }
}

constexpr int kFlagIT = 8;
__global__ __launch_bounds__(kBlock) void occ_flags_kernel(const uint32_t* __restrict__ keys, const uint32_t* __restrict__ perm,
                                                           int64_t nA, int64_t n, int fstride, uint8_t* __restrict__ flags,
                                                           uint32_t* __restrict__ headsA, uint32_t* __restrict__ headsB,
                                                           unsigned* __restrict__ cnt, bool stat = false) {
    constexpr int NW = kBlock / 64;
    __shared__ unsigned wcnt[3][NW], wbase[2][NW];
    const int lane = threadIdx.x & 63, wave = threadIdx.x >> 6;
    for (int64_t base = (int64_t)blockIdx.x * kBlock * kFlagIT; base < n; base += (int64_t)gridDim.x * kBlock * kFlagIT) {
        const int64_t q0 = base + (int64_t)threadIdx.x * kFlagIT;
        uint32_t k[kFlagIT + 2], o[kFlagIT];
#pragma unroll
        for (int j = 0; j < kFlagIT + 2; ++j) {
            const int64_t q = q0 - 1 + j;
            k[j] = (q >= 0 && q < n) ? keys[q] : 0u;
        }
#pragma unroll
        for (int j = 0; j < kFlagIT; ++j) o[j] = q0 + j < n ? perm[q0 + j] : 0u;
        unsigned hA = 0, hB = 0, nd = 0;
#pragma unroll
        for (int j = 0; j < kFlagIT; ++j) {
            const int64_t q = q0 + j;
            if (q < n) {
                const uint32_t row = k[j + 1];
                const bool first = q == 0 || k[j] != row, last = q + 1 >= n || k[j + 2] != row;
                nd += (first && last) ? 0u : 1u;
                if (q < nA) {
                    flags[(int64_t)fstride * o[j]] = (uint8_t)(first && last);
                    hA |= (unsigned)(first && !last) << j;
                } else {
                    const int64_t ob = o[j];
                    int64_t fi;
                    if (ob < nA) fi = fstride * ob + 1;
                    else { const int64_t r_ = ob - nA, m_ = r_ / nA; fi = fstride * (r_ - m_ * nA) + 2 + m_; }
                    flags[fi] = (uint8_t)(first && last);
                    hB |= (unsigned)(first && !last) << j;
                }
            }
        }
        unsigned cA = (unsigned)__popc(hA), cB = (unsigned)__popc(hB), pA = cA, pB = cB;
#pragma unroll
        for (int d = 1; d < 64; d <<= 1) {
            const unsigned a = __shfl_up(pA, d, 64), b = __shfl_up(pB, d, 64);
            if (lane >= d) { pA += a; pB += b; }
        }
        if (stat) {
#pragma unroll
            for (int d = 1; d < 64; d <<= 1) nd += __shfl_xor(nd, d, 64);
        }
        if (lane == 63) { wcnt[0][wave] = pA; wcnt[1][wave] = pB; wcnt[2][wave] = nd; }
        __syncthreads();
        if (stat && threadIdx.x == 2) {
            unsigned tot = 0;
            for (int w = 0; w < NW; ++w) tot += wcnt[2][w];
            if (tot) atomicAdd(&cnt[2], tot);
        }
        if (threadIdx.x < 2) {
            const int t = threadIdx.x;
            unsigned tot = 0;
            for (int w = 0; w < NW; ++w) { wbase[t][w] = tot; tot += wcnt[t][w]; }
            const unsigned b = tot ? atomicAdd(&cnt[t], tot) : 0u;
            for (int w = 0; w < NW; ++w) wbase[t][w] += b;
        }
        __syncthreads();
        unsigned sA = wbase[0][wave] + pA - cA, sB = wbase[1][wave] + pB - cB;
#pragma unroll
        for (int j = 0; j < kFlagIT; ++j) {
            if ((hA >> j) & 1u) headsA[sA++] = (uint32_t)(q0 + j);
            if ((hB >> j) & 1u) headsB[sB++] = (uint32_t)(q0 + j - nA);
        }
        __syncthreads();
    }
}

__global__ __launch_bounds__(kBlock) void coef_finish_kernel(const double* __restrict__ partials, int nblocks, int64_t B,
                                                             float reg_weight, float* __restrict__ out9, int kmul = 1,
                                                             int64_t* __restrict__ step_u_dev = nullptr, int64_t* __restrict__ step_i_dev = nullptr,
                                                             float* __restrict__ hp_dev = nullptr, float lr = 0.f, float b1 = 0.f, float b2 = 0.f,
                                                             unsigned* __restrict__ zero4 = nullptr, const float* __restrict__ norms2 = nullptr,
                                                             uint32_t* __restrict__ zspan = nullptr, int zwords = 0) {
    __shared__ double smem[2 * (kBlock / 64)];
    if (zero4 && threadIdx.x >= 64 && threadIdx.x < 68) zero4[threadIdx.x - 64] = 0u;
    if (zspan) {
        for (int i = threadIdx.x; i < zwords; i += kBlock) zspan[i] = 0u;
    }
    if (hp_dev && threadIdx.x < 2) {
        int64_t* c = threadIdx.x == 0 ? step_u_dev : step_i_dev;
        const int64_t st = c[0] + 1;
        c[0] = st;
        cdr_adam_hp((double)st, lr, b1, b2, hp_dev[2 * threadIdx.x], hp_dev[2 * threadIdx.x + 1]);
    }
    double acc[2] = {0.0, 0.0};
    sum_partials<2, kBlock>(partials, nblocks, acc, smem);
    if (threadIdx.x == 0) {
        if (norms2) { acc[0] = (double)norms2[0]; acc[1] = (double)norms2[1]; }
        const float nu = (float)sqrt((double)kmul * acc[0]), ni = (float)sqrt((double)kmul * acc[1]);
        out9[4] = (reg_weight != 0.f && nu > 0.f) ? (float)kmul * (reg_weight / ((float)B * nu)) : 0.f;
        out9[5] = (reg_weight != 0.f && ni > 0.f) ? (float)kmul * (reg_weight / ((float)B * ni)) : 0.f;
    }
}

__global__ __launch_bounds__(kBlock) void step_finish_keep_kernel(const double* __restrict__ partials, int nblocks, int64_t B,
                                                                  float reg_weight, float* __restrict__ out9,
                                                                  unsigned* __restrict__ zero_a = nullptr, unsigned* __restrict__ zero_b = nullptr,
                                                                  const float* __restrict__ norms2 = nullptr) {
    __shared__ double smem[3 * (kBlock / 64)];
    if (zero_a && threadIdx.x >= 64 && threadIdx.x < 68) zero_a[threadIdx.x - 64] = 0u;
    if (zero_b && threadIdx.x >= 128 && threadIdx.x < 132) zero_b[threadIdx.x - 128] = 0u;
    double acc[3] = {0.0, 0.0, 0.0};
    sum_partials<3, kBlock>(partials, nblocks, acc, smem);
    if (threadIdx.x == 0) {
        if (norms2) { acc[1] = (double)norms2[0]; acc[2] = (double)norms2[1]; }
        const float main_loss = (float)(acc[0] / (double)B);
        const float nu = (float)sqrt(acc[1]), ni = (float)sqrt(acc[2]);
        out9[1] = main_loss; out9[2] = nu; out9[3] = ni;
        out9[0] = main_loss + reg_weight * ((nu + ni) / (float)B);
        out9[6] = (float)acc[0]; out9[7] = (float)acc[1]; out9[8] = (float)acc[2];
    }
}

__global__ __launch_bounds__(kBlock) void norm_sums_kernel(const double* __restrict__ partials, int nblocks, float* __restrict__ sums3) {
    __shared__ double smem[2 * (kBlock / 64)];
    double acc[2] = {0.0, 0.0};
    sum_partials<2, kBlock>(partials, nblocks, acc, smem);
    if (threadIdx.x == 0) { sums3[0] = 0.f; sums3[1] = (float)acc[0]; sums3[2] = (float)acc[1]; }
}

__global__ __launch_bounds__(kBlock) void shard_sums_kernel(const double* __restrict__ partials, int nblocks, float* __restrict__ out9,
                                                            unsigned* __restrict__ zero_a) {
    __shared__ double smem[3 * (kBlock / 64)];
    if (zero_a && threadIdx.x >= 64 && threadIdx.x < 68) zero_a[threadIdx.x - 64] = 0u;
    double acc[3] = {0.0, 0.0, 0.0};
    sum_partials<3, kBlock>(partials, nblocks, acc, smem);
    if (threadIdx.x == 0) { out9[6] = (float)acc[0]; out9[7] = (float)acc[1]; out9[8] = (float)acc[2]; }
}

template <int LPR, int OPT, int UN, bool XD = false, bool SH = false, bool NC = false>
__global__ __launch_bounds__(kBlock) void bpr_fwd_apply_kernel(tab_ptrs TU, tab_ptrs TI, int D, const int64_t* __restrict__ uid,
                                                               const int64_t* __restrict__ pid, const int64_t* __restrict__ nid,
                                                               const uint32_t* __restrict__ flags4, int64_t B, float gamma, float invB,
                                                               const float* __restrict__ coef, apply_hp hu, apply_hp hi,
                                                               float* __restrict__ GU, float* __restrict__ GP,
                                                               double* __restrict__ partials, const float* __restrict__ xdiff = nullptr,
                                                               float* __restrict__ GS = nullptr, float* __restrict__ NU = nullptr,
                                                               float* __restrict__ NI = nullptr) {
    static_assert(!NC || (!XD && !SH), "the norm cache belongs to the plain step");
    HP_FROM_DEV(hu); HP_FROM_DEV(hi);
    constexpr int GPB = kBlock / LPR;
    __shared__ double smem[3 * (kBlock / 64)];
    const int sub = threadIdx.x % LPR;
    const int64_t gg = (int64_t)blockIdx.x * GPB + threadIdx.x / LPR;
    const int64_t TG = (int64_t)gridDim.x * GPB;
    const int D4 = D >> 2;
    const bool live = sub < D4;
    const float cu = coef[0], ci = coef[1];
    const float4 z4 = make_float4(0.f, 0.f, 0.f, 0.f);
    double acc[3] = {0.0, 0.0, 0.0};

    uint32_t iu[UN], ip[UN], in[UN], fl[UN];
    float xd[UN];
#pragma unroll
    for (int r = 0; r < UN; ++r) {
        const int64_t t = gg + (int64_t)r * TG;
        const int64_t tc = t < B ? t : B - 1;
        iu[r] = (uint32_t)uid[tc]; ip[r] = (uint32_t)pid[tc]; in[r] = (uint32_t)nid[tc];
        fl[r] = flags4[tc];
        xd[r] = XD ? xdiff[tc] : 0.f;
    }
#pragma unroll
    for (int r = 0; r < UN; ++r) asm volatile("" : "+v"(iu[r]), "+v"(ip[r]), "+v"(in[r]), "+v"(fl[r]), "+v"(xd[r]));
    for (int64_t base = gg; base < B; base += TG * UN) {
        float4 u[UN], p[UN], n[UN], um[UN], uv[UN], pm[UN], pv[UN], nm[UN], nv[UN];
        int64_t ou[UN], op[UN], on[UN];
        bool fu[UN], fp[UN], fn[UN];
#pragma unroll
        for (int r = 0; r < UN; ++r) {
            const int64_t t = base + (int64_t)r * TG;
            const bool ok = t < B && live;
            fu[r] = (fl[r] & 0xFFu) != 0 && t < B; fp[r] = (fl[r] & 0xFF00u) != 0 && t < B; fn[r] = (fl[r] & 0xFF0000u) != 0 && t < B;
            ou[r] = (int64_t)iu[r] * D + 4 * sub; op[r] = (int64_t)ip[r] * D + 4 * sub; on[r] = (int64_t)in[r] * D + 4 * sub;
            u[r] = ok ? ld4n<(LPR >= 32)>(TU.W + ou[r]) : z4;
            p[r] = ok ? ld4n<(LPR >= 32)>(TI.W + op[r]) : z4;
            n[r] = ok ? ld4n<(LPR >= 32)>(TI.W + on[r]) : z4;
            um[r] = uv[r] = pm[r] = pv[r] = nm[r] = nv[r] = z4;
            if (ok && fu[r]) row_moments<LPR, OPT>(TU, ou[r], um[r], uv[r]);
            if (!SH && ok && fp[r]) row_moments<LPR, OPT>(TI, op[r], pm[r], pv[r]);
            if (!SH && ok && fn[r]) row_moments<LPR, OPT>(TI, on[r], nm[r], nv[r]);
        }
        uint32_t ju[UN], jp[UN], jn[UN], gl[UN];
        float yd[UN];
#pragma unroll
        for (int r = 0; r < UN; ++r) {
            const int64_t t = base + (int64_t)(UN + r) * TG;
            const int64_t tc = t < B ? t : B - 1;
            ju[r] = (uint32_t)uid[tc]; jp[r] = (uint32_t)pid[tc]; jn[r] = (uint32_t)nid[tc];
            gl[r] = flags4[tc];
            yd[r] = XD ? xdiff[tc] : 0.f;
        }
        __builtin_amdgcn_sched_barrier(0);
        float gco[UN], sus[UN], sps[UN], lss[UN];
#pragma unroll
        for (int r = 0; r < UN; ++r) {
            float x;
            if (XD) { x = xd[r]; sus[r] = sps[r] = 0.f; }
            else {
                const float dp = group_sum<LPR>(dot4(u[r], p[r]));
                const float dn = group_sum<LPR>(dot4(u[r], n[r]));
                sus[r] = group_sum<LPR>(dot4(u[r], u[r]));
                sps[r] = group_sum<LPR>(dot4(p[r], p[r]));
                x = dp - dn;
            }
            bpr_term(x, gamma, invB, lss[r], gco[r]);
        }
#pragma unroll
        for (int r = 0; r < UN; ++r) asm volatile("" : "+v"(ju[r]), "+v"(jp[r]), "+v"(jn[r]), "+v"(gl[r]), "+v"(yd[r]));
        __builtin_amdgcn_sched_barrier(0);
#pragma unroll
        for (int r = 0; r < UN; ++r) {
            const int64_t t = base + (int64_t)r * TG;
            const float g = gco[r];
            const float4 gu = make_float4(g * (p[r].x - n[r].x), g * (p[r].y - n[r].y), g * (p[r].z - n[r].z), g * (p[r].w - n[r].w));
            const float4 gi = make_float4(g * u[r].x, g * u[r].y, g * u[r].z, g * u[r].w);
// ... 177 lines not shown
        if (fp) {
            const float4 wp = upd_math<OPT>(p, pm, pv, gp, ci, hi);
            if (live) row_store<LPR, OPT>(TI, op, wp, pm, pv);
        } else if (live) st4n<(LPR >= 32)>(GI + j * D + 4 * sub, gp);
    }
    block_sum_d<3>(acc, smem);
    if (threadIdx.x == 0) store_partials(partials, acc);
}

template <int LPR>
__global__ __launch_bounds__(kBlock) void point_norms_kmajor_kernel(const float* __restrict__ U, const float* __restrict__ I, int D,
                                                                    const int64_t* __restrict__ uid, const int64_t* __restrict__ iid, int64_t S,
                                                                    int k, double* __restrict__ partials) {
    constexpr int GPB = kBlock / LPR;
    __shared__ double smem[2 * (kBlock / 64)];
    const int sub = threadIdx.x % LPR;
    const bool live = sub < (D >> 2);
    const float4 z4 = make_float4(0.f, 0.f, 0.f, 0.f);
    double acc[2] = {0.0, 0.0};
    for (int64_t j = (int64_t)blockIdx.x * GPB + threadIdx.x / LPR; j < S; j += (int64_t)gridDim.x * GPB) {
        const float4 u = live ? ld4n<(LPR >= 32)>(U + uid[j] * D + 4 * sub) : z4;
        float si = 0.f;
        for (int r0 = 0; r0 <= k; r0 += 4) {
            float4 v[4];
#pragma unroll
            for (int c = 0; c < 4; ++c) v[c] = (live && r0 + c <= k) ? ld4n<(LPR >= 32)>(I + iid[j + (int64_t)(r0 + c) * S] * D + 4 * sub) : z4;
#pragma unroll
            for (int c = 0; c < 4; ++c) si += dot4(v[c], v[c]);
        }
        const float su = group_sum<LPR>(dot4(u, u)), st = group_sum<LPR>(si);
        if (sub == 0) { acc[0] += (double)(1 + k) * (double)su; acc[1] += (double)st; }
    }
    block_sum_d<2>(acc, smem);
    if (threadIdx.x == 0) store_partials(partials, acc);
}

__global__ __launch_bounds__(kBlock) void point_coef_kmajor_kernel(const double* __restrict__ partials, int nblocks, int64_t B, int k,
                                                                   float reg_weight, float* __restrict__ out9, unsigned* __restrict__ zero4) {
    __shared__ double smem[2 * (kBlock / 64)];
    if (zero4 && threadIdx.x >= 64 && threadIdx.x < 68) zero4[threadIdx.x - 64] = 0u;
    double acc[2] = {0.0, 0.0};
    sum_partials<2, kBlock>(partials, nblocks, acc, smem);
    if (threadIdx.x == 0) {
        const float nu = (float)sqrt(acc[0]), ni = (float)sqrt(acc[1]);
        out9[4] = embloss_coef(reg_weight, B, nu);
        out9[5] = embloss_coef(reg_weight, B, ni);
        out9[9] = (float)(1 + k) * out9[4];
    }
}

template <int LPR, int OPT, int KC>
__global__ __launch_bounds__(kBlock) void point_fwd_apply_kmajor_kernel(int loss_kind, tab_ptrs TU, tab_ptrs TI, int D, const int64_t* __restrict__ uid,
                                                                        const int64_t* __restrict__ iid, const float* __restrict__ label,
                                                                        const uint8_t* __restrict__ flags, int fstride, int64_t S, int k,
                                                                        float invB, const float* __restrict__ coef, apply_hp hu, apply_hp hi,
                                                                        float* __restrict__ GU, float* __restrict__ GI,
                                                                        double* __restrict__ partials) {
    HP_FROM_DEV(hu); HP_FROM_DEV(hi);
    constexpr int GPB = kBlock / LPR;
    __shared__ double smem[3 * (kBlock / 64)];
    const int sub = threadIdx.x % LPR;
    const bool live = sub < (D >> 2);
    const float cu = coef[5], ci = coef[1];
    const float4 z4 = make_float4(0.f, 0.f, 0.f, 0.f);
    double acc[3] = {0.0, 0.0, 0.0};
    for (int64_t j = (int64_t)blockIdx.x * GPB + threadIdx.x / LPR; j < S; j += (int64_t)gridDim.x * GPB) {
        const uint8_t* fl = flags + j * fstride;
        const int64_t iu = uid[j];
        const bool fu = fl[0] != 0;
        const int64_t ou = iu * D + 4 * sub;
        float4 u = z4, um = z4, uv = z4;
        if (live) {
            u = ld4n<(LPR >= 32)>(TU.W + ou);
            if (fu) row_moments<LPR, OPT>(TU, ou, um, uv);
        }
        float4 gu = z4;
        float su = 0.f;
        for (int r0 = 0; r0 <= k; r0 += KC) {
            int64_t oi[KC]; bool fi[KC]; float yl[KC];
            float4 v[KC], vm[KC], vv[KC];
#pragma unroll
            for (int c = 0; c < KC; ++c) {
                const int r = r0 + c <= k ? r0 + c : k;
                oi[c] = iid[j + (int64_t)r * S] * D + 4 * sub;
                fi[c] = fl[1 + r] != 0 && r0 + c <= k;
                yl[c] = label[j + (int64_t)r * S];
            }
#pragma unroll
            for (int c = 0; c < KC; ++c) {
                v[c] = live ? ld4n<(LPR >= 32)>(TI.W + oi[c]) : z4;
                vm[c] = vv[c] = z4;
                if (live && fi[c]) row_moments<LPR, OPT>(TI, oi[c], vm[c], vv[c]);
            }
            if (r0 == 0) su = group_sum<LPR>(dot4(u, u));
#pragma unroll
            for (int c = 0; c < KC; ++c) {
                const float dx = group_sum<LPR>(dot4(u, v[c]));
                const float si = group_sum<LPR>(dot4(v[c], v[c]));
                if (r0 + c <= k) {
                    const float y = yl[c];
                    float l, g;
                    point_term(loss_kind, dx, y, invB, l, g);
                    gu.x += g * v[c].x; gu.y += g * v[c].y; gu.z += g * v[c].z; gu.w += g * v[c].w;
                    if (sub == 0) { acc[0] += (double)l; acc[2] += (double)si; }
                    const float4 gi = make_float4(g * u.x, g * u.y, g * u.z, g * u.w);
                    if (fi[c]) {
                        const float4 wi = upd_math<OPT>(v[c], vm[c], vv[c], gi, ci, hi);
                        if (live) row_store<LPR, OPT>(TI, oi[c], wi, vm[c], vv[c]);
                    } else if (live) st4n<(LPR >= 32)>(GI + (j + (int64_t)(r0 + c) * S) * D + 4 * sub, gi);
                }
            }
        }
        if (sub == 0) acc[1] += (double)(1 + k) * (double)su;
        if (fu) {
            const float4 wu = upd_math<OPT>(u, um, uv, gu, cu, hu);
            if (live) row_store<LPR, OPT>(TU, ou, wu, um, uv);
        } else if (live) st4n<(LPR >= 32)>(GU + j * D + 4 * sub, gu);
    }
    block_sum_d<3>(acc, smem);
    if (threadIdx.x == 0) store_partials(partials, acc);
}

template <int LPR>
__device__ __forceinline__ int64_t seg_end_probe(const uint32_t* __restrict__ keys, int64_t q, int64_t n, uint32_t row) {
    if constexpr (LPR >= 32) {
        const int lane = threadIdx.x & 63, l = lane & 31;
        const int64_t p = q + 3 + l;
        const bool same = (LPR == 32 || lane < 32) && p < n && p <= q + kLongSeg && keys[p] == row;
        const unsigned long long m = __ballot(!same);
        const uint32_t mg = LPR == 32 ? (uint32_t)(m >> (lane & 32)) : (uint32_t)m;
        return q + 3 + (mg ? (int64_t)(__ffs((int)mg) - 1) : 32);
    } else {
        int64_t end = q + 3;
        while (end < n && end <= q + kLongSeg && keys[end] == row) ++end;
        return end;
    }
}

template <int LPR>
__device__ __forceinline__ uint32_t seg_occ_fetch(const uint32_t* __restrict__ perm, int64_t q, int64_t end) {
    if constexpr (LPR >= 32) {
        const int l = threadIdx.x & 31;
        return ((LPR == 32 || (threadIdx.x & 63) < 32) && q + 2 + l < end) ? perm[q + 2 + l] : 0u;
    } else {
        return 0u;
    }
}
template <int LPR>
__device__ __forceinline__ int64_t seg_occ_at(const uint32_t* __restrict__ perm, uint32_t mine, int64_t q, int64_t e) {
    if constexpr (LPR >= 32) return (int64_t)__shfl(mine, (int)(e - (q + 2)), LPR);
    else return (int64_t)perm[e];
}

template <int LPR, int OPT, bool SIGNED, bool NC = false>
__device__ __forceinline__ void rowwise_apply_dups_body(float* __restrict__ W, float* __restrict__ Mo, float* __restrict__ Vo,
                                                        int D, const uint32_t* __restrict__ keys,
                                                        const uint32_t* __restrict__ perm, int64_t n,
                                                        const uint32_t* __restrict__ heads, const unsigned* __restrict__ nheads,
                                                        const float* __restrict__ G, int64_t neg_start, int64_t reg_limit,
                                                        const float* __restrict__ reg_coef, apply_hp hp,
                                                        unsigned* __restrict__ counters, seg_long* __restrict__ longs,
                                                        seg_piece* __restrict__ pieces, float* __restrict__ n2 = nullptr) {
    HP_FROM_DEV(hp);
    const tab_ptrs T{W, Mo, Vo};
    constexpr int GPB = kBlock / LPR;
    constexpr int SU = 4;
    const int sub = threadIdx.x % LPR;
    const int64_t gg = (int64_t)blockIdx.x * GPB + threadIdx.x / LPR;
    const int64_t TG = (int64_t)gridDim.x * GPB;
    const int D4 = D >> 2;
    const float c = reg_coef ? reg_coef[0] : 0.f;
    const int64_t nh = (int64_t)nheads[0];
    if (D4 <= LPR) {
        const bool live = sub < D4;
        const float4 z4 = make_float4(0.f, 0.f, 0.f, 0.f);
        for (int64_t h0 = gg * SU; h0 < nh; h0 += TG * SU) {
            int64_t q[SU]; uint32_t row[SU], k1[SU], k2[SU]; bool ok[SU];
#pragma unroll
            for (int j = 0; j < SU; ++j) { ok[j] = h0 + j < nh; q[j] = ok[j] ? (int64_t)heads[h0 + j] : 0; }
#pragma unroll
            for (int j = 0; j < SU; ++j) {
                row[j] = keys[q[j]];
                k1[j] = q[j] + 1 < n ? keys[q[j] + 1] : ~0u;
                k2[j] = q[j] + 2 < n ? keys[q[j] + 2] : ~0u;
            }
            uint32_t far[SU], o0[SU], o1[SU];
#pragma unroll
            for (int j = 0; j < SU; ++j) {
                far[j] = q[j] + kLongSeg < n ? keys[q[j] + kLongSeg] : ~0u;
                o0[j] = perm[q[j]]; o1[j] = q[j] + 1 < n ? perm[q[j] + 1] : 0u;
            }
            float4 w[SU], m[SU], v[SU], g0[SU], g1[SU];
            int64_t off[SU];
#pragma unroll
            for (int j = 0; j < SU; ++j) {
                ok[j] = ok[j] && !(far[j] == row[j] && row[j] != ~0u && q[j] + kLongSeg < n);
                off[j] = (int64_t)row[j] * D + 4 * sub;
                w[j] = m[j] = v[j] = g0[j] = g1[j] = z4;
                if (ok[j] && live) {
                    w[j] = ld4n<(LPR >= 32)>(W + off[j]);
                    row_moments<LPR, OPT>(T, off[j], m[j], v[j]);
                    const bool n0 = SIGNED && (int64_t)o0[j] >= neg_start, n1 = SIGNED && (int64_t)o1[j] >= neg_start;
                    g0[j] = ld4n<(LPR >= 32)>(G + (n0 ? (int64_t)o0[j] - neg_start : (int64_t)o0[j]) * D + 4 * sub);
                    g1[j] = ld4n<(LPR >= 32)>(G + (n1 ? (int64_t)o1[j] - neg_start : (int64_t)o1[j]) * D + 4 * sub);
                }
            }
#pragma unroll
            for (int j = 0; j < SU; ++j) {
                if (!ok[j]) continue;
                float4 acc = z4;
                int cnt = 0;
                {
                    const bool n0 = SIGNED && (int64_t)o0[j] >= neg_start, n1 = SIGNED && (int64_t)o1[j] >= neg_start;
                    if (n0) { acc.x -= g0[j].x; acc.y -= g0[j].y; acc.z -= g0[j].z; acc.w -= g0[j].w; }
                    else { acc.x += g0[j].x; acc.y += g0[j].y; acc.z += g0[j].z; acc.w += g0[j].w; }
                    cnt += ((int64_t)o0[j] < reg_limit) ? 1 : 0;
                    if (n1) { acc.x -= g1[j].x; acc.y -= g1[j].y; acc.z -= g1[j].z; acc.w -= g1[j].w; }
                    else { acc.x += g1[j].x; acc.y += g1[j].y; acc.z += g1[j].z; acc.w += g1[j].w; }
                    cnt += ((int64_t)o1[j] < reg_limit) ? 1 : 0;
                }
                if (k2[j] == row[j]) {
                    const int64_t end = seg_end_probe<LPR>(keys, q[j], n, row[j]);
                    const uint32_t occ_l = seg_occ_fetch<LPR>(perm, q[j], end);
                    for (int64_t e0 = q[j] + 2; e0 < end; e0 += 8) {
                        int64_t o[8]; float4 g[8];
#pragma unroll
                        for (int u = 0; u < 8; ++u) { const int64_t ov = seg_occ_at<LPR>(perm, occ_l, q[j], e0 + u < end ? e0 + u : q[j] + 2); o[u] = e0 + u < end ? ov : -1; }
#pragma unroll
                        for (int u = 0; u < 8; ++u) {
                            const bool neg = SIGNED && o[u] >= neg_start;
                            g[u] = (o[u] >= 0 && live) ? ld4n<(LPR >= 32)>(G + (neg ? o[u] - neg_start : o[u]) * D + 4 * sub) : z4;
                        }
#pragma unroll
                        for (int u = 0; u < 8; ++u) {
                            if (o[u] < 0) continue;
                            if (SIGNED && o[u] >= neg_start) { acc.x -= g[u].x; acc.y -= g[u].y; acc.z -= g[u].z; acc.w -= g[u].w; }
                            else { acc.x += g[u].x; acc.y += g[u].y; acc.z += g[u].z; acc.w += g[u].w; }
                            cnt += (o[u] < reg_limit) ? 1 : 0;
                        }
                    }
                }
                const float4 wn = upd_math<OPT>(w[j], m[j], v[j], acc, c * (float)cnt, hp);
                if (live) row_store<LPR, OPT>(T, off[j], wn, m[j], v[j]);
                if (NC) norm_rec_store<LPR>(n2 + (int64_t)row[j] * kNormRecFloats, group_sum<LPR>(sqnorm4<LPR>(wn)), sub);
            }
        }
    } else {
        for (int64_t h = gg; h < nh; h += TG) {
            const int64_t q = heads[h];
            const uint32_t row = keys[q];
            const bool is_long = q + kLongSeg < n && keys[q + kLongSeg] == row;
            if (is_long) continue;
            for (int ch = sub; ch < D4; ch += LPR) {
                const int64_t off = (int64_t)row * D + 4 * ch;
                const float4 w = ld4n<(LPR >= 32)>(W + off);
                float4 m = make_float4(0.f, 0.f, 0.f, 0.f), v = m;
                row_moments<LPR, OPT>(T, off, m, v);
                float4 acc = make_float4(0.f, 0.f, 0.f, 0.f);
                int cnt = 0;
                for (int64_t e = q; e < n && keys[e] == row; ++e) {
                    const int64_t o = perm[e];
                    const bool neg = SIGNED && o >= neg_start;
                    const float4 g = ld4n<(LPR >= 32)>(G + (neg ? o - neg_start : o) * D + 4 * ch);
                    if (neg) { acc.x -= g.x; acc.y -= g.y; acc.z -= g.z; acc.w -= g.w; }
                    else { acc.x += g.x; acc.y += g.y; acc.z += g.z; acc.w += g.w; }
                    cnt += (o < reg_limit) ? 1 : 0;
                }
                const float4 wn = upd_math<OPT>(w, m, v, acc, c * (float)cnt, hp);
                row_store<LPR, OPT>(T, off, wn, m, v);
            }
        }
    }
    if (counters == nullptr) return;
    for (int64_t q = (int64_t)blockIdx.x * kBlock + threadIdx.x; q + kLongSeg < n; q += (int64_t)gridDim.x * kBlock) {
        const uint32_t row = keys[q];
        const uint32_t before = keys[q > 0 ? q - 1 : 0];
        const uint32_t far = keys[q + kLongSeg];
        if ((q > 0 && before == row) || far != row || row == ~0u) continue;
        int64_t lo = q + kLongSeg, hi = n;
        while (lo + 1 < hi) {
            const int64_t mid = (lo + hi) >> 1;
            if (keys[mid] == row) lo = mid; else hi = mid;
        }
        const int64_t len = hi - q;
        const unsigned np = (unsigned)((len + kPiece - 1) / kPiece);
        const unsigned base = atomicAdd(&counters[0], np);
        const unsigned li = atomicAdd(&counters[1], 1u);
        longs[li] = seg_long{q, len, (int64_t)base};
        for (unsigned k = 0; k < np; ++k) {
            const int64_t st = q + (int64_t)k * kPiece;
            pieces[base + k] = seg_piece{st, (hi - st) < kPiece ? (hi - st) : (int64_t)kPiece};
        }
    }
}
struct dup_side {
    float* W; float* M; float* V; const uint32_t* keys; const uint32_t* perm; int64_t n; const uint32_t* heads; const unsigned* nheads;
    const float* G; int64_t neg_start, reg_limit; const float* reg_coef; apply_hp hp;
    unsigned* counters; seg_long* longs; seg_piece* pieces; int* pcnt; float* partial;
    float* out = nullptr; const uint32_t* uidx = nullptr;
    float* n2 = nullptr;
};
template <int LPR, int OPT, bool NC = false>
__global__ __launch_bounds__(kBlock) void rowwise_apply_dups2_kernel(int D, dup_side a, dup_side b) {
    const dup_side& t = blockIdx.y ? b : a;
    rowwise_apply_dups_body<LPR, OPT, true, NC>(t.W, t.M, t.V, D, t.keys, t.perm, t.n, t.heads, t.nheads, t.G, t.neg_start, t.reg_limit, t.reg_coef, t.hp,
                                                t.counters, t.longs, t.pieces, t.n2);
}
template <int LPR>
__global__ __launch_bounds__(kBlock) void seg_piece_sum2_kernel(int D, dup_side a, dup_side b) {
    const dup_side& t = blockIdx.y ? b : a;
    if (t.counters == nullptr) return;
    seg_piece_sum_body<LPR, true>(D, t.perm, t.G, t.neg_start, t.reg_limit, nullptr, t.counters, t.pieces, t.partial, t.pcnt);
}
template <int LPR, int OPT, bool NC = false>
__global__ __launch_bounds__(kBlock) void seg_long_finish2_kernel(int D, dup_side a, dup_side b) {
    const dup_side& t = blockIdx.y ? b : a;
    if (t.counters == nullptr) return;
    seg_long_finish_body<LPR, OPT, NC>(t.W, t.M, t.V, D, t.keys, t.reg_coef, t.hp, t.counters, t.longs, t.partial, t.pcnt, t.n2);
}

__global__ __launch_bounds__(kBlock) void shard_keys_kernel(const int64_t* __restrict__ recv3, int64_t Bl, uint32_t G, unsigned lb,
                                                            uint32_t key_base, int64_t* __restrict__ u_loc, uint32_t* __restrict__ keys,
                                                            uint32_t* __restrict__ vals, unsigned* __restrict__ cnt,
                                                            uint32_t* __restrict__ zspan, int64_t zwords) {
    sort_state_clear(zspan, zwords);
    if (blockIdx.x == 0 && threadIdx.x < 4) cnt[threadIdx.x] = 0u;
    for (int64_t t = (int64_t)blockIdx.x * kBlock + threadIdx.x; t < Bl; t += (int64_t)gridDim.x * kBlock) {
        const int64_t u = recv3[3 * t];
        const uint32_t p = (uint32_t)recv3[3 * t + 1], n = (uint32_t)recv3[3 * t + 2];
        u_loc[t] = u;
        keys[t] = (uint32_t)u; vals[t] = (uint32_t)t;
        keys[Bl + t] = key_base + (((p % G) << lb) | (p / G)); vals[Bl + t] = (uint32_t)t;
        keys[2 * Bl + t] = key_base + (((n % G) << lb) | (n / G)); vals[2 * Bl + t] = (uint32_t)(Bl + t);
    }
}

struct head_flag_op {
    const uint32_t* keys;
    __device__ uint32_t operator()(uint32_t q) const { return (q == 0u || keys[q] != keys[q - 1]) ? 1u : 0u; }
};

__global__ __launch_bounds__(kBlock) void shard_emit_kernel(const uint32_t* __restrict__ keys, const uint32_t* __restrict__ perm,
                                                            const uint32_t* __restrict__ excl, int64_t n, int world, unsigned lb,
                                                            uint32_t key_base, uint32_t* __restrict__ uidx, int64_t* __restrict__ uniq_local,
                                                            int64_t* __restrict__ umap, int64_t* __restrict__ starts,
                                                            int64_t* __restrict__ n_uniq) {
    const uint32_t lmask = (1u << lb) - 1u;
    for (int64_t q = (int64_t)blockIdx.x * kBlock + threadIdx.x; q < n; q += (int64_t)gridDim.x * kBlock) {
        const uint32_t key = keys[q] - key_base;
        const uint32_t prev = q > 0 ? keys[q - 1] - key_base : 0u;
        const bool head = q == 0 || prev != key;
        const uint32_t j = excl[q] + (head ? 1u : 0u) - 1u;
        uidx[q] = j;
        umap[perm[q]] = (int64_t)j;
        if (head) {
            uniq_local[j] = (int64_t)(key & lmask);
            const int owner = (int)(key >> lb), before = q > 0 ? (int)(prev >> lb) : -1;
            for (int k = before + 1; k <= owner; ++k) starts[k] = (int64_t)j;
        }
        if (q == n - 1) {
            n_uniq[0] = (int64_t)j + 1;
            for (int k = (int)(key >> lb) + 1; k <= world; ++k) starts[k] = (int64_t)j + 1;
        }
    }
}
__global__ void shard_counts_kernel(int64_t* __restrict__ starts_counts, int world) {
    if (threadIdx.x == 0 && blockIdx.x == 0)
        for (int k = 0; k < world; ++k) starts_counts[k] = starts_counts[k + 1] - starts_counts[k];
}

template <int LPR>
__global__ __launch_bounds__(kBlock) void shard_norms_kernel(const float* __restrict__ U, int D, const int64_t* __restrict__ uid,
                                                             const float* __restrict__ nrm2, const int64_t* __restrict__ ip, int64_t B,
                                                             double* __restrict__ partials) {
    constexpr int GPB = kBlock / LPR;
    constexpr int UNR = 8;
    __shared__ double smem[2 * (kBlock / 64)];
    const int sub = threadIdx.x % LPR;
    const int64_t gg = (int64_t)blockIdx.x * GPB + threadIdx.x / LPR;
    const int64_t TG = (int64_t)gridDim.x * GPB;
    const bool live = sub < (D >> 2);
    double acc[2] = {0.0, 0.0};
    for (int64_t base = gg; base < B; base += TG * UNR) {
        int64_t iu[UNR], ii[UNR];
        float4 u[UNR];
        float pn[UNR];
#pragma unroll
        for (int r = 0; r < UNR; ++r) {
            const int64_t t = base + (int64_t)r * TG;
            const int64_t tc = t < B ? t : B - 1;
            iu[r] = uid[tc]; ii[r] = ip[tc];
        }
#pragma unroll
        for (int r = 0; r < UNR; ++r) {
            const int64_t t = base + (int64_t)r * TG;
            u[r] = (t < B && live) ? ld4n<(LPR >= 32)>(U + iu[r] * D + 4 * sub) : make_float4(0.f, 0.f, 0.f, 0.f);
            pn[r] = (t < B && sub == 0) ? nrm2[ii[r]] : 0.f;
        }
#pragma unroll
        for (int r = 0; r < UNR; ++r) {
            const float su = group_sum<LPR>(dot4(u[r], u[r]));
            if (sub == 0) { acc[0] += (double)su; acc[1] += (double)pn[r]; }
        }
    }
    block_sum_d<2>(acc, smem);
    if (threadIdx.x == 0) store_partials(partials, acc);
}

template <int LPR>
__device__ __forceinline__ void segsum_dups_body(int D, const dup_side& t) {
    constexpr int GPB = kBlock / LPR;
    constexpr int SU = 4;
    const uint32_t* __restrict__ keys = t.keys; const uint32_t* __restrict__ perm = t.perm; const uint32_t* __restrict__ heads = t.heads;
    const float* __restrict__ G = t.G; const float* __restrict__ rows = t.W; float* __restrict__ out = t.out;
    const uint32_t* __restrict__ uidx = t.uidx;
    const int64_t n = t.n, neg_start = t.neg_start, reg_limit = t.reg_limit;
    const int sub = threadIdx.x % LPR;
    const int64_t gg = (int64_t)blockIdx.x * GPB + threadIdx.x / LPR;
    const int64_t TG = (int64_t)gridDim.x * GPB;
    const int D4 = D >> 2;
    const float c = t.reg_coef ? t.reg_coef[0] : 0.f;
    const int64_t nh = (int64_t)t.nheads[0];
    const bool live = sub < D4;
    const float4 z4 = make_float4(0.f, 0.f, 0.f, 0.f);
    for (int64_t h0 = gg * SU; h0 < nh; h0 += TG * SU) {
        int64_t q[SU]; uint32_t row[SU], k2[SU]; bool ok[SU];
#pragma unroll
        for (int j = 0; j < SU; ++j) { ok[j] = h0 + j < nh; q[j] = ok[j] ? (int64_t)heads[h0 + j] : 0; }
        uint32_t far[SU], o0[SU], o1[SU], ju[SU];
#pragma unroll
        for (int j = 0; j < SU; ++j) {
            row[j] = keys[q[j]];
            k2[j] = q[j] + 2 < n ? keys[q[j] + 2] : ~0u;
            far[j] = q[j] + kLongSeg < n ? keys[q[j] + kLongSeg] : ~0u;
            o0[j] = perm[q[j]]; o1[j] = q[j] + 1 < n ? perm[q[j] + 1] : 0u;
            ju[j] = uidx[q[j]];
        }
        float4 w[SU], g0[SU], g1[SU];
#pragma unroll
        for (int j = 0; j < SU; ++j) {
            ok[j] = ok[j] && !(far[j] == row[j] && row[j] != ~0u && q[j] + kLongSeg < n);
            w[j] = g0[j] = g1[j] = z4;
            if (ok[j] && live) {
                if (c != 0.f) w[j] = ld4n<(LPR >= 32)>(rows + (int64_t)ju[j] * D + 4 * sub);
                const bool n0 = (int64_t)o0[j] >= neg_start, n1 = (int64_t)o1[j] >= neg_start;
                g0[j] = ld4n<(LPR >= 32)>(G + (n0 ? (int64_t)o0[j] - neg_start : (int64_t)o0[j]) * D + 4 * sub);
                g1[j] = ld4n<(LPR >= 32)>(G + (n1 ? (int64_t)o1[j] - neg_start : (int64_t)o1[j]) * D + 4 * sub);
            }
        }
#pragma unroll
        for (int j = 0; j < SU; ++j) {
            if (!ok[j]) continue;
            float4 acc = z4;
            int cnt = 0;
            {
                const bool n0 = (int64_t)o0[j] >= neg_start, n1 = (int64_t)o1[j] >= neg_start;
                if (n0) { acc.x -= g0[j].x; acc.y -= g0[j].y; acc.z -= g0[j].z; acc.w -= g0[j].w; }
                else { acc.x += g0[j].x; acc.y += g0[j].y; acc.z += g0[j].z; acc.w += g0[j].w; }
                cnt += ((int64_t)o0[j] < reg_limit) ? 1 : 0;
// ... 381 lines not shown
    hipStream_t s = (hipStream_t)stream;
    const int lpr = cdr_lpr_for(D);
    const int grid = grid_for((B + kUnroll - 1) / kUnroll, kBlock / lpr);
    {
        cdr_time_scope ts(ctx, CDR_TAG_POINT_FWD_GRAD, s);
        DISPATCH_LPR(lpr, point_fwd_grad_kernel<L><<<dim3(grid), dim3(kBlock), 0, s>>>(loss_kind, user_tab, item_tab, D, uid, iid, label, B,
                                                                                        1.0f / (float)B, GU, GI, ctx->partials));
    }
    CDR_LAUNCH_CHECK();
    step_finish_kernel<<<dim3(1), dim3(kBlock), 0, s>>>(ctx->partials, grid, B, reg_weight, out9);
    CDR_LAUNCH_CHECK();
    return CDR_OK;
}

extern "C" int cdr_triplet_fwd_grad(cdr_ctx* ctx, void* stream, const float* user_tab, const float* item_tab, int D,
                                    const int64_t* uid, const int64_t* pid, const int64_t* nid, int64_t B, float margin, float eps,
                                    float* out3, float* GU, float* GI) {
    CDR_CHECK_ARG(ctx && user_tab && item_tab && uid && pid && nid && out3 && GU && GI);
    CDR_CHECK_ARG(D > 0 && (D & 3) == 0 && D <= 256 && B > 0);
    hipStream_t s = (hipStream_t)stream;
    const int lpr = cdr_lpr_for(D);
    const int grid = grid_for((B + kUnroll - 1) / kUnroll, kBlock / lpr);
    {
        cdr_time_scope ts(ctx, CDR_TAG_TRIPLET_FWD_GRAD, s);
        DISPATCH_LPR(lpr, triplet_fwd_grad_kernel<L><<<dim3(grid), dim3(kBlock), 0, s>>>(user_tab, item_tab, D, uid, pid, nid, B, margin, eps,
                                                                                          1.0f / (float)B, GU, GI, ctx->partials));
    }
    CDR_LAUNCH_CHECK();
    triplet_finish_kernel<<<dim3(1), dim3(kBlock), 0, s>>>(ctx->partials, grid, B, out3);
    CDR_LAUNCH_CHECK();
    return CDR_OK;
}

extern "C" int cdr_loss_finish_sums(void* stream, const float* sums3, int64_t B_mean, float reg_weight, float* out6) {
    CDR_CHECK_ARG(sums3 && out6 && B_mean > 0);
    finish_sums_kernel<<<dim3(1), dim3(64), 0, (hipStream_t)stream>>>(sums3, B_mean, reg_weight, out6);
    CDR_LAUNCH_CHECK();
    return CDR_OK;
}

using big_sort_config = rocprim::radix_sort_config<
    rocprim::default_config, rocprim::default_config,
    rocprim::radix_sort_onesweep_config<rocprim::kernel_config<kSortBlock, kSortItems>, rocprim::kernel_config<kSortBlock, kSortItems>, kSortRadixBits,
                                        rocprim::block_radix_rank_algorithm::match>,
    (size_t)1 << 17>;
constexpr int64_t kBigSort = 1 << 18;

static inline hipError_t sort_pairs(void* tmp, size_t& tmp_bytes, const uint32_t* kin, uint32_t* kout, const uint32_t* vin, uint32_t* vout,
                                    size_t n, unsigned bits, hipStream_t s) {
    if ((int64_t)n >= kBigSort) return rocprim::radix_sort_pairs<big_sort_config>(tmp, tmp_bytes, kin, kout, vin, vout, n, 0u, bits, s);
    return rocprim::radix_sort_pairs(tmp, tmp_bytes, kin, kout, vin, vout, n, 0u, bits, s);
}

static inline unsigned bits_for(int64_t num_rows) {
    unsigned b = 1;
    while (b < 32 && ((int64_t)1 << b) < num_rows) ++b;
    return b;
}

#if ROCPRIM_VERSION == 400200
#define CDR_HAVE_OWN_SORT 1
namespace {

namespace rpd = rocprim::detail;
using sort_bid_t = rpd::block_id_wrapper<unsigned int, true>;

__global__ __launch_bounds__(kSortBlock) void sort_hist_kernel(const uint32_t* keys, sort_offs_t* counts, sort_offs_t size, sort_offs_t full_blocks,
                                                               unsigned end_bit) {
    rpd::onesweep_histograms<kSortBlock, kSortItems, kSortRadixBits, false>(keys, counts, size, full_blocks, rocprim::identity_decomposer{}, 0u, end_bit);
}
__global__ __launch_bounds__(kSortBlock) void sort_scan_kernel(sort_offs_t* counts) {
    rpd::onesweep_scan_histograms<kSortBlock, kSortRadixBits>(counts);
}
__global__ __launch_bounds__(kSortBlock) void sort_pass_kernel(const uint32_t* keys_in, uint32_t* keys_out, const uint32_t* vals_in, uint32_t* vals_out,
                                                               unsigned size, sort_offs_t* offs_in, sort_offs_t* offs_out,
                                                               rpd::onesweep_lookback_state* lookback, unsigned bit, unsigned cur_bits,
                                                               unsigned full_blocks, sort_bid_t bid) {
    rpd::onesweep_iteration<kSortBlock, kSortItems, kSortRadixBits, false, rocprim::block_radix_rank_algorithm::match>(
        keys_in, keys_out, vals_in, vals_out, size, offs_in, offs_out, lookback, rocprim::identity_decomposer{}, bit, cur_bits, full_blocks, bid);
}

struct own_sort_plan {
    unsigned blocks = 0, full_blocks = 0, places = 0;
    int64_t wordsA = 0, wordsB = 0;
    size_t o_ids = 0, o_lookback = 0, o_offs_tmp = 0, o_keys_tmp = 0, o_vals_tmp = 0, bytes = 0;
    own_sort_plan(size_t n, unsigned bits) {
        constexpr size_t per_block = (size_t)kSortBlock * kSortItems;
        blocks = (unsigned)((n + per_block - 1) / per_block);
        full_blocks = n % per_block == 0 ? blocks : blocks - 1;
        places = (bits + kSortRadixBits - 1) / kSortRadixBits;
        const size_t arr = ((n * sizeof(uint32_t)) + 255) & ~(size_t)255;
        wordsA = (int64_t)(places * kSortRadix * (sizeof(sort_offs_t) / 4) + 32);
        o_ids = (size_t)wordsA * 4;
        o_lookback = o_ids + (size_t)kSortMaxPlaces * 128;
        const size_t lb_bytes = (size_t)places * blocks * kSortRadix * sizeof(rpd::onesweep_lookback_state);
        wordsB = (int64_t)((o_lookback + lb_bytes - o_ids) / 4);
        o_offs_tmp = (o_lookback + lb_bytes + 255) & ~(size_t)255;
        o_keys_tmp = o_offs_tmp + kSortRadix * sizeof(sort_offs_t);
        o_vals_tmp = o_keys_tmp + arr;
        bytes = o_vals_tmp + arr;
    }
    sort_offs_t* counts(char* tmp) const { return (sort_offs_t*)tmp; }
    unsigned* ticket(char* tmp) const { return (unsigned*)(tmp + (size_t)wordsA * 4 - 128); }
};
static_assert(sizeof(rpd::onesweep_lookback_state) == 4 && sizeof(sort_offs_t) % 4 == 0, "the zero span is counted in 32-bit words");

constexpr int64_t kOwnSortMax = (int64_t)1 << 30;

inline bool own_sort_on(int64_t n) {
    static const bool on = [] { const char* e = getenv("CDR_OWN_SORT"); return !(e && e[0] == '0'); }();
    return on && n >= kBigSort && n <= kOwnSortMax;
}

inline hipError_t own_sort_offsets(const own_sort_plan& P, char* tmp, const uint32_t* keys_in, size_t n, unsigned bits, hipStream_t s) {
    sort_hist_kernel<<<dim3(P.blocks), dim3(kSortBlock), 0, s>>>(keys_in, P.counts(tmp), (sort_offs_t)n, (sort_offs_t)P.full_blocks, bits);
    sort_scan_kernel<<<dim3(P.places), dim3(kSortBlock), 0, s>>>(P.counts(tmp));
    return hipGetLastError();
}

inline hipError_t own_sort_passes(const own_sort_plan& P, char* tmp, const uint32_t* keys_in, uint32_t* keys_out, const uint32_t* vals_in,
                                  uint32_t* vals_out, size_t n, unsigned bits, hipStream_t s) {
    uint32_t* keys_tmp = (uint32_t*)(tmp + P.o_keys_tmp);
    uint32_t* vals_tmp = (uint32_t*)(tmp + P.o_vals_tmp);
    auto* lookback = (rpd::onesweep_lookback_state*)(tmp + P.o_lookback);
    bool to_output = (P.places - 1) % 2 == 0, from_input = true;
    unsigned place = 0;
    for (unsigned bit = 0; bit < bits; bit += kSortRadixBits, ++place) {
        const uint32_t* ki = from_input ? keys_in : (to_output ? keys_tmp : keys_out);
        const uint32_t* vi = from_input ? vals_in : (to_output ? vals_tmp : vals_out);
        const unsigned cur_bits = bits - bit < kSortRadixBits ? bits - bit : kSortRadixBits;
        sort_pass_kernel<<<dim3(P.blocks), dim3(kSortBlock), 0, s>>>(
            ki, to_output ? keys_out : keys_tmp, vi, to_output ? vals_out : vals_tmp, (unsigned)n, P.counts(tmp) + (size_t)place * kSortRadix,
            (sort_offs_t*)(tmp + P.o_offs_tmp), lookback + (size_t)place * P.blocks * kSortRadix, bit, cur_bits, P.full_blocks,
            sort_bid_t::create(tmp + P.o_ids + (size_t)place * 128));
        from_input = false;
        to_output = !to_output;
    }
    return hipGetLastError();
}

}
#else
#define CDR_HAVE_OWN_SORT 0
#endif

namespace {

inline size_t up256(size_t b) { return (b + 255) & ~(size_t)255; }

struct heads_view {
    unsigned* cnt; uint32_t* headsA; uint32_t* headsB;
    heads_view(uint32_t* heads, int64_t n_a) : cnt((unsigned*)heads), headsA(heads + 4), headsB(headsA + (n_a / 2 + 1)) {}
    static int64_t words(int64_t n_a, int64_t n_b) { return 4 + (n_a / 2 + 1) + (n_b / 2 + 1); }
};

inline size_t count_list_bytes(int64_t B) {
    int64_t P = 1024;
    while (P < 3 * B) P <<= 1;
    return (size_t)(P + kListHdr) * sizeof(uint64_t);
}

inline unsigned two_table_bits(int64_t rows_a, int64_t rows_b) {
    const unsigned a = bits_for(rows_a), b = bits_for(rows_b);
    return a > b ? a : b;
}

apply_hp make_hp(int opt, float lr, float beta1, float beta2, float eps, float wd, int64_t step) {
    float step_size = lr, bc2_sqrt = 1.f;
    if (opt == 1) {
        cdr_adam_hp((double)step, lr, beta1, beta2, step_size, bc2_sqrt);
    }
    return apply_hp{lr, beta1, beta2, eps, wd, step_size, bc2_sqrt};
}

struct long_scratch {
    int64_t long_cap = 0, piece_cap = 0;
    size_t o_long = 0, o_piece = 0, o_cnt = 0, o_part = 0, bytes = 0;
    long_scratch() = default;
    long_scratch(int64_t n, int D) {
        if (n <= kLongSeg) return;
        long_cap = n / (kLongSeg + 1) + 1;
        piece_cap = n / kPiece + long_cap + 1;
        o_long = 256; o_piece = o_long + up256(sizeof(seg_long) * long_cap); o_cnt = o_piece + up256(sizeof(seg_piece) * piece_cap);
        o_part = o_cnt + up256(sizeof(int) * piece_cap); bytes = o_part + sizeof(float) * (size_t)piece_cap * D;
    }
    void bind(char* base, dup_side& t) const {
        t.counters = (unsigned*)base; t.longs = (seg_long*)(base + o_long); t.pieces = (seg_piece*)(base + o_piece);
        t.pcnt = (int*)(base + o_cnt); t.partial = (float*)(base + o_part);
    }
};

}

extern "C" int cdr_sort_workspace_bytes(int64_t n, int64_t num_rows, size_t* bytes) {
    CDR_CHECK_ARG(bytes && n > 0 && num_rows > 0 && num_rows <= (int64_t)0xFFFFFFFFu && n <= (int64_t)0x7FFFFFFF);
    size_t tmp = 0;
    hipError_t e = sort_pairs(nullptr, tmp, nullptr, nullptr, nullptr, nullptr, (size_t)n, bits_for(num_rows), (hipStream_t)0);
    if (e != hipSuccess) { cdr_set_error("cdr_sort_workspace_bytes: %s", hipGetErrorString(e)); return (int)e; }
#if CDR_HAVE_OWN_SORT
    if (n >= kBigSort && n <= kOwnSortMax) {
        const size_t own = own_sort_plan((size_t)n, bits_for(num_rows)).bytes;
        if (own > tmp) tmp = own;
    }
#endif
    *bytes = up256(tmp) + 2 * up256((size_t)n * sizeof(uint32_t));
    return CDR_OK;
}

struct sort_clear { uint32_t* p; int64_t words; };

template <class MakeKeys>
static int sort_ids_with(cdr_ctx* ctx, hipStream_t s, int64_t n, int64_t key_space, uint32_t* keys_sorted, uint32_t* perm, void* ws,
                         size_t ws_bytes, MakeKeys&& make_keys, bool keys_make_offsets = false) {
    size_t need = 0;
    int rc = cdr_sort_workspace_bytes(n, key_space, &need);
    if (rc) return rc;
    CDR_CHECK_ARG(ws_bytes >= need);
    const size_t arr = up256((size_t)n * sizeof(uint32_t));
    uint32_t* keys_in = (uint32_t*)ws;
    uint32_t* vals_in = (uint32_t*)((char*)ws + arr);
    char* tmp = (char*)ws + 2 * arr;
    size_t tmp_bytes = ws_bytes - 2 * arr;
    const unsigned bits = bits_for(key_space);
    cdr_time_scope ts(ctx, CDR_TAG_SORT, s);
#if CDR_HAVE_OWN_SORT
    if (own_sort_on(n)) {
        CDR_CHECK_ARG(((uintptr_t)tmp & 127) == 0);
        const own_sort_plan P((size_t)n, bits);
        if (keys_make_offsets) {
            make_keys(keys_in, vals_in, sort_clear{(uint32_t*)(tmp + P.o_ids), P.wordsB});
            CDR_LAUNCH_CHECK();
        } else {
            make_keys(keys_in, vals_in, sort_clear{(uint32_t*)tmp, P.wordsA + P.wordsB});
            CDR_LAUNCH_CHECK();
            CDR_HIP(own_sort_offsets(P, tmp, keys_in, (size_t)n, bits, s));
        }
        CDR_HIP(own_sort_passes(P, tmp, keys_in, keys_sorted, vals_in, perm, (size_t)n, bits, s));
        return CDR_OK;
    }
#endif
    make_keys(keys_in, vals_in, sort_clear{nullptr, 0});
    CDR_LAUNCH_CHECK();
    CDR_HIP(sort_pairs(tmp, tmp_bytes, keys_in, keys_sorted, vals_in, perm, (size_t)n, bits, s));
    return CDR_OK;
}

#if CDR_HAVE_OWN_SORT
static sort_clear own_sort_span_a(int64_t n, int64_t key_space, void* ws, size_t ws_bytes) {
    size_t need = 0;
    if (!own_sort_on(n) || cdr_sort_workspace_bytes(n, key_space, &need) != CDR_OK || ws_bytes < need) return {nullptr, 0};
    return {(uint32_t*)((char*)ws + 2 * up256((size_t)n * sizeof(uint32_t))), own_sort_plan((size_t)n, bits_for(key_space)).wordsA};
}
#else
static sort_clear own_sort_span_a(int64_t, int64_t, void*, size_t) { return {nullptr, 0}; }
#endif

extern "C" int cdr_sort_ids(cdr_ctx* ctx, void* stream, const int64_t* ids0, int64_t n0, const int64_t* ids1, int64_t n1,
                            int64_t num_rows, uint32_t* keys_sorted, uint32_t* perm, void* workspace,
                            size_t workspace_bytes) {
    const int64_t n = n0 + n1;
    CDR_CHECK_ARG(ids0 && n0 > 0 && (n1 == 0 || ids1) && keys_sorted && perm && workspace);
    hipStream_t s = (hipStream_t)stream;
    return sort_ids_with(ctx, s, n, num_rows, keys_sorted, perm, workspace, workspace_bytes, [&](uint32_t* keys_in, uint32_t* vals_in, sort_clear z) {
        make_keys_kernel<<<dim3(grid_for(n, kBlock)), dim3(kBlock), 0, s>>>(ids0, n0, ids1, n1, keys_in, vals_in, z.p, z.words);
    });
}

static inline uint32_t two_table_key_base(int64_t rows_a, int64_t rows_b) {
    const unsigned hb = two_table_bits(rows_a, rows_b);
    return hb < 31 ? 1u << hb : 0u;
}

static int sort_two_tables(cdr_ctx* ctx, void* stream, const int64_t* ids_a, int64_t n_a, int64_t rows_a, const int64_t* ids_b0,
                           int64_t n_b0, const int64_t* ids_b1, int64_t n_b1, int64_t rows_b, uint32_t* keys_sorted, uint32_t* perm,
                           uint32_t* key_base_out, void* workspace, size_t workspace_bytes, sort_clear span_a) {
    const int64_t n = n_a + n_b0 + n_b1;
    CDR_CHECK_ARG(ids_a && n_a > 0 && ids_b0 && n_b0 > 0 && (n_b1 == 0 || ids_b1) && keys_sorted && perm && key_base_out && workspace);
    CDR_CHECK_ARG(rows_a > 0 && rows_b > 0);
    const uint32_t key_base = two_table_key_base(rows_a, rows_b);
    CDR_CHECK_ARG(key_base != 0u);
    hipStream_t s = (hipStream_t)stream;
    int rc = sort_ids_with(ctx, s, n, (int64_t)key_base * 2, keys_sorted, perm, workspace, workspace_bytes, [&](uint32_t* keys_in, uint32_t* vals_in, sort_clear z) {
        if (span_a.p && z.p) {
            const unsigned places = (bits_for((int64_t)key_base * 2) + kSortRadixBits - 1) / kSortRadixBits;
            const unsigned kgrid = (unsigned)((n + (int64_t)kSortBlock * kSortItems - 1) / ((int64_t)kSortBlock * kSortItems));
            make_keys2_offsets_kernel<<<dim3(kgrid), dim3(kSortBlock), 0, s>>>(ids_a, n_a, ids_b0, n_b0, ids_b1, n_b1, key_base, keys_in, vals_in, z.p, z.words,
                                                                               (sort_offs_t*)span_a.p, (unsigned*)span_a.p + span_a.words - 32, places);
        } else {
            make_keys2_kernel<<<dim3(grid_for(n, kBlock)), dim3(kBlock), 0, s>>>(ids_a, n_a, ids_b0, n_b0, ids_b1, n_b1, key_base, keys_in, vals_in, z.p, z.words);
        }
    }, span_a.p != nullptr);
    if (rc) return rc;
    *key_base_out = key_base;
    return CDR_OK;
}

extern "C" int cdr_sort_ids_two_tables(cdr_ctx* ctx, void* stream, const int64_t* ids_a, int64_t n_a, int64_t rows_a,
                                       const int64_t* ids_b0, int64_t n_b0, const int64_t* ids_b1, int64_t n_b1, int64_t rows_b,
                                       uint32_t* keys_sorted, uint32_t* perm, uint32_t* key_base_out, void* workspace,
                                       size_t workspace_bytes) {
    return sort_two_tables(ctx, stream, ids_a, n_a, rows_a, ids_b0, n_b0, ids_b1, n_b1, rows_b, keys_sorted, perm, key_base_out, workspace,
                           workspace_bytes, sort_clear{nullptr, 0});
}

extern "C" int cdr_rowwise_apply(cdr_ctx* ctx, void* stream, int opt, float* table, float* exp_avg, float* exp_avg_sq, int D,
                                 const uint32_t* keys_sorted, const uint32_t* perm, int64_t n, const float* G,
                                 int64_t neg_start, int64_t reg_limit, const float* reg_coef, float lr, float beta1,
                                 float beta2, float eps, float weight_decay, int64_t step, const int64_t* occ_ids, uint32_t key_base) {
    CDR_CHECK_ARG(table && keys_sorted && perm && G && n > 0);
    CDR_CHECK_ARG(D > 0 && (D & 3) == 0);
    CDR_CHECK_ARG(opt == 0 || (opt == 1 && exp_avg && exp_avg_sq && step > 0) || (opt == CDR_OPT_ADAGRAD && !exp_avg && exp_avg_sq));
    hipStream_t s = (hipStream_t)stream;
    if (key_base) {
        table -= (int64_t)key_base * D;
        if (exp_avg) exp_avg -= (int64_t)key_base * D;
        if (exp_avg_sq) exp_avg_sq -= (int64_t)key_base * D;
    }
    const int lpr = cdr_lpr_for(D);
    const int grid = grid_for(n, kBlock / lpr);
    const bool is_signed = neg_start < n;
    const apply_hp hp = make_hp(opt, lr, beta1, beta2, eps, weight_decay, step);
    const long_scratch ls(n, D);
    dup_side sc{};
    if (ls.bytes) {
        CDR_CHECK_ARG(ctx != nullptr);
        void* base = nullptr;
        int rc = cdr_ctx_scratch(ctx, ls.bytes, &base);
        if (rc != CDR_OK) return rc;
        ls.bind((char*)base, sc);
        CDR_HIP(cdr_zero_u32(sc.counters, 4, s));
    }
    cdr_time_scope ts(ctx, is_signed ? CDR_TAG_APPLY_SIGNED : CDR_TAG_APPLY_UNSIGNED, s);
    DISPATCH_LPR_OPT3(lpr, opt, {
        auto kern = is_signed ? rowwise_apply_kernel<L, O, true> : rowwise_apply_kernel<L, O, false>;
        kern<<<dim3(grid), dim3(kBlock), 0, s>>>(table, exp_avg, exp_avg_sq, D, keys_sorted, perm, n, G, neg_start, reg_limit, reg_coef, hp, occ_ids,
                                                 sc.counters, sc.longs, sc.pieces);
    });
    CDR_LAUNCH_CHECK();
    if (ls.bytes) {
        const int gp = (int)(ls.piece_cap < 2048 ? ls.piece_cap : 2048);
        DISPATCH_LPR(lpr, {
            auto kern = is_signed ? seg_piece_sum_kernel<L, true> : seg_piece_sum_kernel<L, false>;
            kern<<<dim3(gp), dim3(kBlock), 0, s>>>(D, perm, G, neg_start, reg_limit, occ_ids, sc.counters, sc.pieces, sc.partial, sc.pcnt);
        });
        CDR_LAUNCH_CHECK();
        const int gl = grid_for(ls.long_cap < 4096 ? ls.long_cap : 4096, kBlock / lpr);
        DISPATCH_LPR_OPT3(lpr, opt, seg_long_finish_kernel<L, O><<<dim3(gl), dim3(kBlock), 0, s>>>(table, exp_avg, exp_avg_sq, D, keys_sorted, reg_coef, hp, sc.counters,
                                                                                                 sc.longs, sc.partial, sc.pcnt));
        CDR_LAUNCH_CHECK();
    }
    return CDR_OK;
}

namespace {

struct step_tables { tab_ptrs TU, TI; apply_hp hu, hi; };
step_tables make_tables(int opt_user, float* user_tab, float* user_m, float* user_v, int64_t step_user, int opt_item, float* item_tab,
                        float* item_m, float* item_v, int64_t step_item, float lr, float beta1, float beta2, float eps, float wd) {
    return {{user_tab, user_m, user_v}, {item_tab, item_m, item_v}, make_hp(opt_user, lr, beta1, beta2, eps, wd, step_user),
            make_hp(opt_item, lr, beta1, beta2, eps, wd, step_item)};
}

int embloss_head(cdr_ctx* ctx, hipStream_t s, const float* user_tab, const float* item_tab, int D, const int64_t* uid, const int64_t* pid,
                 int64_t n_rows, int64_t B, int kmul, float reg_weight, float* out9, unsigned* cnt, int64_t* step_user_dev = nullptr,
                 int64_t* step_item_dev = nullptr, float* hp_dev = nullptr, float lr = 0.f, float beta1 = 0.f, float beta2 = 0.f,
                 const float* user_n2 = nullptr, const float* item_n2 = nullptr, sort_clear zspan = {nullptr, 0}) {
    int ngrid = 0;
    if (reg_weight != 0.f) {
        const int lpr = cdr_lpr_for(D);
        ngrid = grid_for((n_rows + 7) / 8, kBlock / lpr);
        cdr_time_scope ts(ctx, CDR_TAG_BATCH_NORMS, s);
        if (user_n2 && item_n2) {
            DISPATCH_LPR(lpr, batch_norms_cached_kernel<L><<<dim3(ngrid), dim3(kBlock), 0, s>>>(user_n2, item_n2, uid, pid, n_rows, ctx->partials));
        } else {
            DISPATCH_LPR(lpr, batch_norms_kernel<L><<<dim3(ngrid), dim3(kBlock), 0, s>>>(user_tab, item_tab, D, uid, pid, n_rows, ctx->partials));
        }
        CDR_LAUNCH_CHECK();
    }
    coef_finish_kernel<<<dim3(1), dim3(kBlock), 0, s>>>(ctx->partials, ngrid, B, ngrid ? reg_weight : 0.f, out9, kmul, step_user_dev, step_item_dev, hp_dev,
                                                        lr, beta1, beta2, cnt, nullptr, zspan.p, (int)zspan.words);
    CDR_LAUNCH_CHECK();
    return CDR_OK;
}

int occ_flags(cdr_ctx* ctx, hipStream_t s, const uint32_t* keys, const uint32_t* perm, int64_t n_a, int64_t n, int fstride, uint8_t* flags,
              const heads_view& hv, bool stat = false) {
    cdr_time_scope ts(ctx, CDR_TAG_OCC_FLAGS, s);
    occ_flags_kernel<<<dim3(grid_for(n, kBlock * kFlagIT)), dim3(kBlock), 0, s>>>(keys, perm, n_a, n, fstride, flags, hv.headsA, hv.headsB, hv.cnt, stat);
    CDR_LAUNCH_CHECK();
    return CDR_OK;
}

struct dup_host { tab_ptrs T; const uint32_t* keys; const uint32_t* perm; int64_t n; const uint32_t* heads; const unsigned* nheads;
                  const float* G; int64_t neg_start, reg_limit; const float* reg_coef; apply_hp hp; uint32_t key_base;
                  float* out = nullptr; const uint32_t* uidx = nullptr; float* n2 = nullptr; };
struct dups_plan { dup_side side[2]; long_scratch ls[2]; };

void make_sides(dup_host (&sides)[2], const step_tables& T, const uint32_t* keys, const uint32_t* perm, const heads_view& hv, const float* GU,
                const float* GI, int64_t n_user, int64_t n_item, int64_t neg_start_item, int64_t reg_limit_item, const float* coef_user,
                const float* coef_item, uint32_t key_base) {
    sides[0] = {T.TU, keys, perm, n_user, hv.headsA, hv.cnt, GU, n_user, n_user, coef_user, T.hu, 0};
    sides[1] = {T.TI, keys + n_user, perm + n_user, n_item, hv.headsB, hv.cnt + 1, GI, neg_start_item, reg_limit_item, coef_item, T.hi, key_base};
}

int dups_plan_make(cdr_ctx* ctx, int D, const dup_host (&h)[2], dups_plan& pl) {
    size_t off[2], total = 0;
    for (int i = 0; i < 2; ++i) {
        pl.ls[i] = long_scratch(h[i].n, D);
        off[i] = total;
        total += up256(pl.ls[i].bytes);
    }
    char* base = nullptr;
    if (total) {
        void* b = nullptr;
        int rc = cdr_ctx_scratch(ctx, total, &b);
        if (rc != CDR_OK) return rc;
        base = (char*)b;
    }
    for (int i = 0; i < 2; ++i) {
        dup_side& t = pl.side[i];
        const int64_t kb = (int64_t)h[i].key_base * D;
        t.W = h[i].T.W - kb; t.M = h[i].T.M ? h[i].T.M - kb : nullptr; t.V = h[i].T.V ? h[i].T.V - kb : nullptr;
        t.keys = h[i].keys; t.perm = h[i].perm; t.n = h[i].n; t.heads = h[i].heads; t.nheads = h[i].nheads; t.G = h[i].G;
        t.neg_start = h[i].neg_start; t.reg_limit = h[i].reg_limit; t.reg_coef = h[i].reg_coef; t.hp = h[i].hp;
        t.counters = nullptr; t.longs = nullptr; t.pieces = nullptr; t.pcnt = nullptr; t.partial = nullptr;
        t.out = h[i].out; t.uidx = h[i].uidx;
        t.n2 = h[i].n2 ? h[i].n2 - (int64_t)h[i].key_base * kNormRecFloats : nullptr;
        if (pl.ls[i].bytes) pl.ls[i].bind(base + off[i], t);
    }
    return CDR_OK;
}

struct table_dups {
    static constexpr bool adagrad = true;
    template <int L, int OPT> static constexpr auto dups = rowwise_apply_dups2_kernel<L, OPT>;
    template <int L, int OPT> static constexpr auto long_finish = seg_long_finish2_kernel<L, OPT>;
};
struct table_dups_nc {
    static constexpr bool adagrad = true;
    template <int L, int OPT> static constexpr auto dups = rowwise_apply_dups2_kernel<L, OPT, true>;
    template <int L, int OPT> static constexpr auto long_finish = seg_long_finish2_kernel<L, OPT, true>;
};
struct shard_dups {
    static constexpr bool adagrad = false;
    template <int L, int OPT> static constexpr auto dups = shard_dups_kernel<L, OPT>;
    template <int L, int OPT> static constexpr auto long_finish = shard_long_finish_kernel<L, OPT>;
};

template <class K>
int apply_dups_pair(cdr_ctx* ctx, hipStream_t s, int opt, int D, const dups_plan& pl) {
    const int lpr = cdr_lpr_for(D);
    const int64_t nmax = pl.side[0].n > pl.side[1].n ? pl.side[0].n : pl.side[1].n;
    const int grid = grid_for(nmax / 16 + 1, kBlock / lpr);
    {
        cdr_time_scope ts(ctx, CDR_TAG_APPLY_SIGNED, s);
        if constexpr (K::adagrad) DISPATCH_LPR_OPT3(lpr, opt, K::template dups<L, O><<<dim3(grid, 2), dim3(kBlock), 0, s>>>(D, pl.side[0], pl.side[1]));
        else DISPATCH_LPR_OPT(lpr, opt, K::template dups<L, O><<<dim3(grid, 2), dim3(kBlock), 0, s>>>(D, pl.side[0], pl.side[1]));
    }
    CDR_LAUNCH_CHECK();
    if (pl.ls[0].long_cap || pl.ls[1].long_cap) {
        const int64_t pc = pl.ls[0].piece_cap > pl.ls[1].piece_cap ? pl.ls[0].piece_cap : pl.ls[1].piece_cap;
        const int64_t lc = pl.ls[0].long_cap > pl.ls[1].long_cap ? pl.ls[0].long_cap : pl.ls[1].long_cap;
        const int gp = (int)(pc < 2048 ? pc : 2048);
        DISPATCH_LPR(lpr, seg_piece_sum2_kernel<L><<<dim3(gp, 2), dim3(kBlock), 0, s>>>(D, pl.side[0], pl.side[1]));
        CDR_LAUNCH_CHECK();
        const int gl = grid_for(lc < 4096 ? lc : 4096, kBlock / lpr);
        if constexpr (K::adagrad) DISPATCH_LPR_OPT3(lpr, opt, K::template long_finish<L, O><<<dim3(gl, 2), dim3(kBlock), 0, s>>>(D, pl.side[0], pl.side[1]));
        else DISPATCH_LPR_OPT(lpr, opt, K::template long_finish<L, O><<<dim3(gl, 2), dim3(kBlock), 0, s>>>(D, pl.side[0], pl.side[1]));
        CDR_LAUNCH_CHECK();
    }
    return CDR_OK;
}

template <class K = table_dups, class Finish>
int finish_and_apply_dups(cdr_ctx* ctx, hipStream_t s, int opt, int D, const dup_host (&sides)[2], Finish&& finish) {
    dups_plan pl;
    int rc = dups_plan_make(ctx, D, sides, pl);
    if (rc) return rc;
    finish(pl.side[0].counters, pl.side[1].counters);
    CDR_LAUNCH_CHECK();
    return apply_dups_pair<K>(ctx, s, opt, D, pl);
}

}

extern "C" int cdr_bpr_step_fused_heads_words(int64_t B, int64_t* words) {
    CDR_CHECK_ARG(words && B > 0);
    *words = heads_view::words(B, 2 * B);
    return CDR_OK;
}

static int bpr_step_fused_impl(cdr_ctx* ctx, void* stream, int opt, float* user_tab, float* user_m, float* user_v, int64_t user_rows,
                               float* item_tab, float* item_m, float* item_v, int64_t item_rows, int D, const int64_t* uid,
                               const int64_t* pid, const int64_t* nid, int64_t B, float gamma, float reg_weight, float lr,
                               float beta1, float beta2, float eps, float weight_decay, int64_t step_user, int64_t step_item,
                               int64_t* step_user_dev, int64_t* step_item_dev, float* hp_dev,
                               float* out9, float* GU, float* GP, uint32_t* keys, uint32_t* perm, uint8_t* flags, uint32_t* heads,
                               void* sort_ws, size_t sort_ws_bytes) {
    hipStream_t s = (hipStream_t)stream;
    const int lpr = cdr_lpr_for(D);
    const heads_view hv(heads, B);
    uint32_t key_base = 0;
    int rc;
    const bool count_path = ctx->idc_user && ctx->idc_item && ctx->idc_user_rows == user_rows && ctx->idc_item_rows == item_rows &&
                            B >= kCountMinB && B <= kCountMaxB && ctx->idc_list_bytes >= count_list_bytes(B);
    const bool cached = !count_path && ctx->n2_user && ctx->n2_item && ctx->n2_user_rows == user_rows && ctx->n2_item_rows == item_rows;
    float* NU = cached ? ctx->n2_user : nullptr;
    float* NI = cached ? ctx->n2_item : nullptr;
    if (count_path) {
        const unsigned hb = two_table_bits(user_rows, item_rows);
        CDR_CHECK_ARG(hb < 31);
        key_base = 1u << hb;
        const int ngrid = grid_for((B + 7) / 8, kBlock / lpr);
        {
            cdr_time_scope ts(ctx, CDR_TAG_BATCH_NORMS, s);
            DISPATCH_LPR(lpr, {
                auto kern = reg_weight != 0.f ? batch_norms_count_kernel<L, true> : batch_norms_count_kernel<L, false>;
                kern<<<dim3(ngrid), dim3(kBlock), 0, s>>>(user_tab, item_tab, D, uid, pid, nid, B, ctx->idc_user, ctx->idc_item, keys, (uint64_t*)ctx->idc_list, ctx->partials);
            });
        }
        CDR_LAUNCH_CHECK();
        coef_finish_kernel<<<dim3(1), dim3(kBlock), 0, s>>>(ctx->partials, reg_weight != 0.f ? ngrid : 0, B, reg_weight, out9, 1, step_user_dev, step_item_dev, hp_dev,
                                                            lr, beta1, beta2, hv.cnt);
        CDR_LAUNCH_CHECK();
        {
            cdr_time_scope ts(ctx, CDR_TAG_OCC_FLAGS, s);
            count_flags_kernel<<<dim3(grid_for(B, kBlock)), dim3(kBlock), 0, s>>>(uid, pid, nid, B, ctx->idc_user, ctx->idc_item, key_base, (uint32_t*)flags,
                                                                                 (uint64_t*)ctx->idc_list, hv.cnt);
            CDR_LAUNCH_CHECK();
            count_sort_kernel<<<dim3(kRankBlocks + 128), dim3(1024), 0, s>>>(uid, pid, nid, B, ctx->idc_user, ctx->idc_item, key_base,
                                                                                            (uint64_t*)ctx->idc_list, keys, perm, hv.headsA, hv.headsB, hv.cnt);
        }
        CDR_LAUNCH_CHECK();
    } else {
        static const bool keys_make_offsets = [] { const char* e = getenv("CDR_OWN_SORT"); return !(e && e[0] == '1'); }();
        const uint32_t kb = two_table_key_base(user_rows, item_rows);
        const sort_clear span_a = keys_make_offsets && kb ? own_sort_span_a(3 * B, (int64_t)kb * 2, sort_ws, sort_ws_bytes) : sort_clear{nullptr, 0};
        rc = embloss_head(ctx, s, user_tab, item_tab, D, uid, pid, B, B, 1, reg_weight, out9, hv.cnt, step_user_dev, step_item_dev, hp_dev, lr, beta1, beta2,
                          NU, NI, span_a);
        if (rc) return rc;
        rc = sort_two_tables(ctx, stream, uid, B, user_rows, pid, B, nid, B, item_rows, keys, perm, &key_base, sort_ws, sort_ws_bytes, span_a);
        if (rc) return rc;
        rc = occ_flags(ctx, s, keys, perm, B, 3 * B, 4, flags, hv, B <= kCountMaxB);
        if (rc) return rc;
    }
    step_tables T = make_tables(opt, user_tab, user_m, user_v, step_user, opt, item_tab, item_m, item_v, step_item, lr, beta1, beta2, eps, weight_decay);
    if (hp_dev && opt == 1) { T.hu.dev = hp_dev; T.hi.dev = hp_dev + 2; }
    static const int un = [] { const char* e = getenv("CDR_FWD_APPLY_UN"); return (e && e[0] == '2') ? 2 : 1; }();
    const int grid = grid_for((B + un - 1) / un, kBlock / lpr);
    {
        cdr_time_scope ts(ctx, CDR_TAG_BPR_FWD_APPLY, s);
        DISPATCH_LPR_OPT3(lpr, opt, {
            constexpr int U2 = O == 1 ? 2 : 1;
            auto kern = cached ? (un == 2 ? bpr_fwd_apply_kernel<L, O, U2, false, false, true> : bpr_fwd_apply_kernel<L, O, 1, false, false, true>)
                               : (un == 2 ? bpr_fwd_apply_kernel<L, O, U2> : bpr_fwd_apply_kernel<L, O, 1>);
            kern<<<dim3(grid), dim3(kBlock), 0, s>>>(T.TU, T.TI, D, uid, pid, nid, (const uint32_t*)flags, B, gamma, 1.0f / (float)B, out9 + 4, T.hu, T.hi, GU, GP,
                                                     ctx->partials, nullptr, nullptr, NU, NI);
        });
    }
    CDR_LAUNCH_CHECK();
    dup_host sides[2];
    make_sides(sides, T, keys, perm, hv, GU, GP, B, 2 * B, B, B, out9 + 4, out9 + 5, key_base);
    sides[0].n2 = NU; sides[1].n2 = NI;
    auto finish = [&](unsigned* za, unsigned* zb) {
        step_finish_keep_kernel<<<dim3(1), dim3(kBlock), 0, s>>>(ctx->partials, grid, B, reg_weight, out9, za, zb);
    };
    return cached ? finish_and_apply_dups<table_dups_nc>(ctx, s, opt, D, sides, finish) : finish_and_apply_dups(ctx, s, opt, D, sides, finish);
}

extern "C" int cdr_norm_rec_floats(void) { return kNormRecFloats; }

extern "C" int cdr_row_norms_build(void* stream, const float* table, int64_t rows, int D, float* n2) {
    CDR_CHECK_ARG(table && n2 && rows > 0 && D > 0 && (D & 3) == 0 && D <= 256);
    CDR_CHECK_ARG((uintptr_t)n2 % (kNormRecFloats * sizeof(float)) == 0);
    hipStream_t s = (hipStream_t)stream;
    const int lpr = cdr_lpr_for(D);
    const int grid = grid_for((rows + kUnroll - 1) / kUnroll, kBlock / lpr);
    DISPATCH_LPR(lpr, row_norms_build_kernel<L><<<dim3(grid), dim3(kBlock), 0, s>>>(table, rows, D, n2));
    CDR_LAUNCH_CHECK();
    return CDR_OK;
}

extern "C" int cdr_id_count_workspace_bytes(int64_t B, size_t* bytes) {
    CDR_CHECK_ARG(bytes && B > 0 && 3 * B <= (int64_t)0x7FFFFFFF);
    *bytes = count_list_bytes(B);
    return CDR_OK;
}

extern "C" int cdr_bpr_step_fused(cdr_ctx* ctx, void* stream, int opt, float* user_tab, float* user_m, float* user_v, int64_t user_rows,
                                  float* item_tab, float* item_m, float* item_v, int64_t item_rows, int D, const int64_t* uid,
                                  const int64_t* pid, const int64_t* nid, int64_t B, float gamma, float reg_weight, float lr,
                                  float beta1, float beta2, float eps, float weight_decay, int64_t step_user, int64_t step_item,
                                  float* out9, float* GU, float* GP, uint32_t* keys, uint32_t* perm, uint8_t* flags, uint32_t* heads,
                                  void* sort_ws, size_t sort_ws_bytes) {
    CDR_CHECK_ARG(ctx && user_tab && item_tab && uid && pid && nid && out9 && GU && GP && keys && perm && flags && heads && sort_ws);
    CDR_CHECK_ARG(D > 0 && (D & 3) == 0 && D <= 256 && B > 0 && 3 * B <= (int64_t)0x7FFFFFFF);
    CDR_CHECK_ARG(opt == 0 || (opt == 1 && user_m && user_v && item_m && item_v && step_user > 0 && step_item > 0) ||
                  (opt == CDR_OPT_ADAGRAD && !user_m && user_v && !item_m && item_v));
    CDR_CHECK_ARG(((uintptr_t)flags & 3) == 0);
    return bpr_step_fused_impl(ctx, stream, opt, user_tab, user_m, user_v, user_rows, item_tab, item_m, item_v, item_rows, D, uid, pid, nid, B, gamma,
                               reg_weight, lr, beta1, beta2, eps, weight_decay, step_user, step_item, nullptr, nullptr, nullptr, out9, GU, GP,
                               keys, perm, flags, heads, sort_ws, sort_ws_bytes);
}

extern "C" int cdr_bpr_step_fused_dev(cdr_ctx* ctx, void* stream, int opt, float* user_tab, float* user_m, float* user_v, int64_t user_rows,
                                      float* item_tab, float* item_m, float* item_v, int64_t item_rows, int D, const int64_t* uid,
                                      const int64_t* pid, const int64_t* nid, int64_t B, float gamma, float reg_weight, float lr,
                                      float beta1, float beta2, float eps, float weight_decay, int64_t* step_user_dev, int64_t* step_item_dev,
                                      float* hp_dev, float* out9, float* GU, float* GP, uint32_t* keys, uint32_t* perm, uint8_t* flags,
                                      uint32_t* heads, void* sort_ws, size_t sort_ws_bytes) {
    CDR_CHECK_ARG(ctx && user_tab && item_tab && uid && pid && nid && out9 && GU && GP && keys && perm && flags && heads && sort_ws);
    CDR_CHECK_ARG(D > 0 && (D & 3) == 0 && D <= 256 && B > 0 && 3 * B <= (int64_t)0x7FFFFFFF);
    CDR_CHECK_ARG(opt == 1 && user_m && user_v && item_m && item_v && step_user_dev && step_item_dev && hp_dev);
    CDR_CHECK_ARG(((uintptr_t)flags & 3) == 0);
    return bpr_step_fused_impl(ctx, stream, opt, user_tab, user_m, user_v, user_rows, item_tab, item_m, item_v, item_rows, D, uid, pid, nid, B, gamma,
                               reg_weight, lr, beta1, beta2, eps, weight_decay, 1, 1, step_user_dev, step_item_dev, hp_dev, out9, GU, GP,
                               keys, perm, flags, heads, sort_ws, sort_ws_bytes);
}


extern "C" int cdr_point_step_fused(cdr_ctx* ctx, void* stream, int loss_kind, int opt, float* user_tab, float* user_m, float* user_v,
                                    int64_t user_rows, float* item_tab, float* item_m, float* item_v, int64_t item_rows, int D,
                                    const int64_t* uid, const int64_t* iid, const float* label, int64_t B, float reg_weight, float lr,
                                    float beta1, float beta2, float eps, float weight_decay, int64_t step_user, int64_t step_item,
                                    float* out9, float* GU, float* GI, uint32_t* keys, uint32_t* perm, uint8_t* flags, uint32_t* heads,
                                    void* sort_ws, size_t sort_ws_bytes) {
    CDR_CHECK_ARG(ctx && user_tab && item_tab && uid && iid && label && out9 && GU && GI && keys && perm && flags && heads && sort_ws);
    CDR_CHECK_ARG((loss_kind == CDR_LOSS_MSE || loss_kind == CDR_LOSS_BCE) && D > 0 && (D & 3) == 0 && D <= 256 && B > 0 && 2 * B <= (int64_t)0x7FFFFFFF);
    CDR_CHECK_ARG(opt == 0 || (opt == 1 && user_m && user_v && item_m && item_v && step_user > 0 && step_item > 0) ||
                  (opt == CDR_OPT_ADAGRAD && !user_m && user_v && !item_m && item_v));
    CDR_CHECK_ARG(((uintptr_t)flags & 3) == 0);
    hipStream_t s = (hipStream_t)stream;
    const int lpr = cdr_lpr_for(D);
    const heads_view hv(heads, B);
    int rc = embloss_head(ctx, s, user_tab, item_tab, D, uid, iid, B, B, 1, reg_weight, out9, hv.cnt);
    if (rc) return rc;
    uint32_t key_base = 0;
    rc = cdr_sort_ids_two_tables(ctx, stream, uid, B, user_rows, iid, B, nullptr, 0, item_rows, keys, perm, &key_base, sort_ws, sort_ws_bytes);
    if (rc) return rc;
    rc = occ_flags(ctx, s, keys, perm, B, 2 * B, 4, flags, hv);
    if (rc) return rc;
    const step_tables T = make_tables(opt, user_tab, user_m, user_v, step_user, opt, item_tab, item_m, item_v, step_item, lr, beta1, beta2, eps, weight_decay);
    const int grid = grid_for(B, kBlock / lpr);
    {
        cdr_time_scope ts(ctx, CDR_TAG_POINT_FWD_GRAD, s);
        DISPATCH_LPR_OPT3(lpr, opt, point_fwd_apply_kernel<L, O><<<dim3(grid), dim3(kBlock), 0, s>>>(loss_kind, T.TU, T.TI, D, uid, iid, label, (const uint32_t*)flags, B,
                                                                                                   1.0f / (float)B, out9 + 4, T.hu, T.hi, GU, GI, ctx->partials));
    }
    CDR_LAUNCH_CHECK();
    dup_host sides[2];
    make_sides(sides, T, keys, perm, hv, GU, GI, B, B, B, B, out9 + 4, out9 + 5, key_base);
    return finish_and_apply_dups(ctx, s, opt, D, sides, [&](unsigned* za, unsigned* zb) {
        step_finish_keep_kernel<<<dim3(1), dim3(kBlock), 0, s>>>(ctx->partials, grid, B, reg_weight, out9, za, zb);
    });
}

extern "C" int cdr_point_step_fused_kmajor(cdr_ctx* ctx, void* stream, int loss_kind, int opt, float* user_tab, float* user_m, float* user_v,
                                           int64_t user_rows, float* item_tab, float* item_m, float* item_v, int64_t item_rows, int D,
                                           const int64_t* uid, const int64_t* iid, const float* label, int64_t S, int k, float reg_weight,
                                           float lr, float beta1, float beta2, float eps, float weight_decay, int64_t step_user,
                                           int64_t step_item, float* out12, float* GU, float* GI, uint32_t* keys, uint32_t* perm,
                                           uint8_t* flags, uint32_t* heads, void* sort_ws, size_t sort_ws_bytes) {
    CDR_CHECK_ARG(ctx && user_tab && item_tab && uid && iid && label && out12 && GU && GI && keys && perm && flags && heads && sort_ws);
    CDR_CHECK_ARG((loss_kind == CDR_LOSS_MSE || loss_kind == CDR_LOSS_BCE) && D > 0 && (D & 3) == 0 && D <= 256 && S > 0 && k >= 1 && k <= 64);
    const int64_t nI = S + S * (int64_t)k, B = nI;
    CDR_CHECK_ARG(S + nI <= (int64_t)0x7FFFFFFF);
    CDR_CHECK_ARG(opt == 0 || (opt == 1 && user_m && user_v && item_m && item_v && step_user > 0 && step_item > 0));
    hipStream_t s = (hipStream_t)stream;
    const int lpr = cdr_lpr_for(D);
    const int fstride = (2 + k + 3) & ~3;
    const heads_view hv(heads, S);
    const int ngrid = reg_weight != 0.f ? grid_for(S, kBlock / lpr) : 0;
    if (reg_weight != 0.f) {
        cdr_time_scope ts(ctx, CDR_TAG_BATCH_NORMS, s);
        DISPATCH_LPR(lpr, point_norms_kmajor_kernel<L><<<dim3(ngrid), dim3(kBlock), 0, s>>>(user_tab, item_tab, D, uid, iid, S, k, ctx->partials));
        CDR_LAUNCH_CHECK();
    }
    point_coef_kmajor_kernel<<<dim3(1), dim3(kBlock), 0, s>>>(ctx->partials, ngrid, B, k, reg_weight, out12, hv.cnt);
    CDR_LAUNCH_CHECK();
    uint32_t key_base = 0;
    int rc = cdr_sort_ids_two_tables(ctx, stream, uid, S, user_rows, iid, S, iid + S, S * (int64_t)k, item_rows, keys, perm, &key_base, sort_ws, sort_ws_bytes);
    if (rc) return rc;
    rc = occ_flags(ctx, s, keys, perm, S, S + nI, fstride, flags, hv);
    if (rc) return rc;
    const step_tables T = make_tables(opt, user_tab, user_m, user_v, step_user, opt, item_tab, item_m, item_v, step_item, lr, beta1, beta2, eps, weight_decay);
    const int grid = grid_for(S, kBlock / lpr);
    {
        cdr_time_scope ts(ctx, CDR_TAG_POINT_FWD_GRAD, s);
        DISPATCH_LPR_OPT(lpr, opt, {
            constexpr int KW = O == 1 ? 3 : 2;
            auto kern = k <= 1 ? point_fwd_apply_kmajor_kernel<L, O, 2> : point_fwd_apply_kmajor_kernel<L, O, KW>;
            kern<<<dim3(grid), dim3(kBlock), 0, s>>>(loss_kind, T.TU, T.TI, D, uid, iid, label, flags, fstride, S, k, 1.0f / (float)B, out12 + 4, T.hu, T.hi, GU, GI,
                                                     ctx->partials);
        });
    }
    CDR_LAUNCH_CHECK();
    dup_host sides[2];
    make_sides(sides, T, keys, perm, hv, GU, GI, S, nI, nI, nI, out12 + 9, out12 + 5, key_base);
    return finish_and_apply_dups(ctx, s, opt, D, sides, [&](unsigned* za, unsigned* zb) {
        step_finish_keep_kernel<<<dim3(1), dim3(kBlock), 0, s>>>(ctx->partials, grid, B, reg_weight, out12, za, zb);
    });
}

extern "C" int cdr_bpr_step_presort(cdr_ctx* ctx, void* stream, const int64_t* uid, const int64_t* pid, const int64_t* nid, int64_t B,
                                    int64_t user_rows, int64_t item_rows, uint32_t* keys, uint32_t* perm, uint8_t* flags, uint32_t* heads,
                                    void* sort_ws, size_t sort_ws_bytes, uint32_t* key_base_out) {
    CDR_CHECK_ARG(ctx && uid && pid && nid && keys && perm && flags && heads && sort_ws && key_base_out && B > 0 && 3 * B <= (int64_t)0x7FFFFFFF);
    CDR_CHECK_ARG(((uintptr_t)flags & 3) == 0);
    hipStream_t s = (hipStream_t)stream;
    int rc = cdr_sort_ids_two_tables(ctx, stream, uid, B, user_rows, pid, B, nid, B, item_rows, keys, perm, key_base_out, sort_ws, sort_ws_bytes);
    if (rc) return rc;
    CDR_HIP(cdr_zero_u32(heads, 4, s));
    return occ_flags(ctx, s, keys, perm, B, 3 * B, 4, flags, heads_view(heads, B));
}

extern "C" int cdr_bpr_step_from_diff(cdr_ctx* ctx, void* stream, int opt, float* user_tab, float* user_m, float* user_v, float* item_tab,
                                      float* item_m, float* item_v, int Ds, const int64_t* uid, const int64_t* pid, const int64_t* nid,
                                      int64_t B, float gamma, float reg_weight, float lr, float beta1, float beta2, float eps,
                                      float weight_decay, int64_t step_user, int64_t step_item, const float* diff, uint32_t key_base,
                                      float* out9, float* GU, float* GP, const uint32_t* keys, const uint32_t* perm, const uint8_t* flags,
// ... 578 lines not shown
```

Measured before the change: 581.6 million interactions/s.

## Emit sparse dup flags, pair records and long segments from occ-flags pass

Adds a new occupancy-flags kernel that writes per-element flags only for ids that repeat, and pre-fills the flag array during key construction. Rows that occur exactly twice are emitted as compact pair records. Long-segment detection moves into the same pass so the apply kernel can skip its own scan. The dup-apply kernel gains a record path that updates paired rows directly, which removes the head scan and separate passes over flags and keys. This adds complexity: atomics for record slots, a binary search for long segments, and a new env-controlled mask whose default enables all three features.

```diff
diff --git a/include/cdr_hip.h b/include/cdr_hip.h
--- a/include/cdr_hip.h
+++ b/include/cdr_hip.h
@@ -25,6 +25,7 @@
 int cdr_norm_rec_floats(void);
 int cdr_row_norms_build(void* stream, const float* table, int64_t rows, int D, float* n2);
 int cdr_ctx_set_norm_cache(cdr_ctx* ctx, float* user_n2, int64_t user_rows, float* item_n2, int64_t item_rows);
+int cdr_ctx_set_dup_records(cdr_ctx* ctx, unsigned mask);
 #define CDR_ABI_VERSION 64
 int cdr_abi_version(void);
 
diff --git a/recbole-cdr_amd/binding.py b/recbole-cdr_amd/binding.py
--- a/recbole-cdr_amd/binding.py
+++ b/recbole-cdr_amd/binding.py
@@ -61,6 +61,7 @@
     'cdr_norm_rec_floats': [],
     'cdr_row_norms_build': [_c_ptr, _c_ptr, _c_i64, _c_int, _c_ptr],
     'cdr_ctx_set_norm_cache': [_c_ptr, _c_ptr, _c_i64, _c_ptr, _c_i64],
+    'cdr_ctx_set_dup_records': [_c_ptr, ctypes.c_uint],
     'cdr_bpr_fwd': [_c_ptr, _c_ptr, _c_ptr, _c_ptr, _c_int, _c_ptr, _c_ptr, _c_ptr, _c_i64, _c_f32, _c_f32, _c_ptr, _c_ptr],
     'cdr_bpr_bwd_dense': [_c_ptr, _c_ptr, _c_ptr, _c_ptr, _c_int, _c_ptr, _c_ptr, _c_ptr, _c_i64, _c_ptr, _c_ptr, _c_f32,
                           _c_ptr, _c_ptr, _c_ptr],
diff --git a/recbole-cdr_amd/csrc/cdr_common.h b/recbole-cdr_amd/csrc/cdr_common.h
--- a/recbole-cdr_amd/csrc/cdr_common.h
+++ b/recbole-cdr_amd/csrc/cdr_common.h
@@ -24,6 +24,7 @@
     void* idc_list; size_t idc_list_bytes;
     float* n2_user; int64_t n2_user_rows;
     float* n2_item; int64_t n2_item_rows;
+    unsigned dup_records;
     unsigned long long* conet_tab_dev; unsigned long long* conet_tab_pin; unsigned long long* conet_tab_shadow; int conet_tab_cap, conet_tab_n;
     int conet_defer, conet_pending, conet_fin_grid;
     int64_t conet_fin_ns, conet_fin_R;
diff --git a/recbole-cdr_amd/csrc/cdr_ctx.hip b/recbole-cdr_amd/csrc/cdr_ctx.hip
--- a/recbole-cdr_amd/csrc/cdr_ctx.hip
+++ b/recbole-cdr_amd/csrc/cdr_ctx.hip
@@ -36,6 +36,10 @@
     c->scrub_ptr = nullptr; c->scrub_bytes = 0;
     c->idc_user = c->idc_item = nullptr; c->idc_user_rows = c->idc_item_rows = 0; c->idc_list = nullptr; c->idc_list_bytes = 0;
     c->n2_user = c->n2_item = nullptr; c->n2_user_rows = c->n2_item_rows = 0;
+    {
+        const char* e = getenv("CDR_DUP_RECORDS");
+        c->dup_records = e && e[0] >= '0' && e[0] <= '7' && !e[1] ? (unsigned)(e[0] - '0') : 7u;
+    }
     c->partials = nullptr;
     c->tickets = nullptr;
     hipError_t e = hipMalloc(&c->partials, sizeof(double) * CDR_MAX_PARTIAL_BLOCKS * CDR_PARTIAL_STRIDE);
@@ -141,3 +145,9 @@
     ctx->n2_user = user_n2; ctx->n2_user_rows = user_rows; ctx->n2_item = item_n2; ctx->n2_item_rows = item_rows;
     return CDR_OK;
 }
+
+extern "C" int cdr_ctx_set_dup_records(cdr_ctx* ctx, unsigned mask) {
+    CDR_CHECK_ARG(ctx != nullptr && mask <= 7u);
+    ctx->dup_records = mask;
+    return CDR_OK;
+}
diff --git a/recbole-cdr_amd/csrc/cdr_step.hip b/recbole-cdr_amd/csrc/cdr_step.hip
--- a/recbole-cdr_amd/csrc/cdr_step.hip
+++ b/recbole-cdr_amd/csrc/cdr_step.hip
@@ -288,6 +288,16 @@
 __device__ __forceinline__ void sort_state_clear(uint32_t* __restrict__ zspan, int64_t zwords) {
     if (!zspan) return;
     for (int64_t i = (int64_t)blockIdx.x * blockDim.x + threadIdx.x; i < zwords; i += (int64_t)gridDim.x * blockDim.x) zspan[i] = 0u;
+}
+
+struct key_extras { uint32_t* fill; int64_t fwords; unsigned* zero[3]; };
+__device__ __forceinline__ void key_extras_apply(const key_extras& x) {
+    if (x.fill)
+        for (int64_t i = (int64_t)blockIdx.x * blockDim.x + threadIdx.x; i < x.fwords; i += (int64_t)gridDim.x * blockDim.x) x.fill[i] = 0x01010101u;
+    if (blockIdx.x == 0 && threadIdx.x < 12) {
+        unsigned* z = x.zero[threadIdx.x >> 2];
+        if (z) z[threadIdx.x & 3] = 0u;
+    }
 }
 
 __global__ __launch_bounds__(kBlock) void make_keys_kernel(const int64_t* __restrict__ ids0, int64_t n0,
@@ -534,8 +544,9 @@
 __global__ __launch_bounds__(kBlock) void make_keys2_kernel(const int64_t* __restrict__ a, int64_t na, const int64_t* __restrict__ b0,
                                                             int64_t nb0, const int64_t* __restrict__ b1, int64_t nb1, uint32_t key_base,
                                                             uint32_t* __restrict__ keys, uint32_t* __restrict__ vals,
-                                                            uint32_t* __restrict__ zspan, int64_t zwords) {
+                                                            uint32_t* __restrict__ zspan, int64_t zwords, key_extras extras = key_extras{}) {
     sort_state_clear(zspan, zwords);
+    key_extras_apply(extras);
     const int64_t n = na + nb0 + nb1, stride = (int64_t)gridDim.x * kBlock;
     for (int64_t e = (int64_t)blockIdx.x * kBlock + threadIdx.x; e < n; e += stride) {
         if (e < na) { keys[e] = (uint32_t)a[e]; vals[e] = (uint32_t)e; }
@@ -555,10 +566,12 @@
                                                                         int64_t nb0, const int64_t* __restrict__ b1, int64_t nb1,
                                                                         uint32_t key_base, uint32_t* __restrict__ keys, uint32_t* __restrict__ vals,
                                                                         uint32_t* __restrict__ zspan, int64_t zwords,
-                                                                        sort_offs_t* __restrict__ counts, unsigned* __restrict__ ticket, unsigned places) {
+                                                                        sort_offs_t* __restrict__ counts, unsigned* __restrict__ ticket, unsigned places,
+                                                                        key_extras extras = key_extras{}) {
     constexpr unsigned kStripes = 4;
     __shared__ unsigned hist[kSortMaxPlaces * kSortRadix * kStripes];
     sort_state_clear(zspan, zwords);
+    key_extras_apply(extras);
     const unsigned tid = threadIdx.x, bins = places * kSortRadix;
     for (unsigned i = tid; i < bins * kStripes; i += kSortBlock) hist[i] = 0u;
     __syncthreads();
@@ -800,6 +813,132 @@
         for (int j = 0; j < kFlagIT; ++j) {
             if ((hA >> j) & 1u) headsA[sA++] = (uint32_t)(q0 + j);
             if ((hB >> j) & 1u) headsB[sB++] = (uint32_t)(q0 + j - nA);
+        }
+        __syncthreads();
+    }
+}
+
+constexpr unsigned kDupSparseFlags = 1u, kDupPairRecs = 2u, kDupLongHere = 4u, kDupAll = 7u;
+struct occ_recs {
+    uint4* pairs[2]; unsigned* pcnt;
+    unsigned* counters[2]; seg_long* longs[2]; seg_piece* pieces[2];
+    unsigned mask;
+};
+__global__ __launch_bounds__(kBlock) void occ_flags_sparse_kernel(const uint32_t* __restrict__ keys, const uint32_t* __restrict__ perm,
+                                                                  int64_t nA, int64_t n, uint8_t* __restrict__ flags,
+                                                                  uint32_t* __restrict__ headsA, uint32_t* __restrict__ headsB,
+                                                                  unsigned* __restrict__ cnt, bool stat, occ_recs r) {
+    constexpr int NW = kBlock / 64, NL = 4;
+    __shared__ unsigned wcnt[NL + 1][NW], wbase[NL][NW];
+    const int lane = threadIdx.x & 63, wave = threadIdx.x >> 6;
+    const bool sparse = (r.mask & kDupSparseFlags) != 0, recs = (r.mask & kDupPairRecs) != 0, longs_here = (r.mask & kDupLongHere) != 0;
+    for (int64_t base = (int64_t)blockIdx.x * kBlock * kFlagIT; base < n; base += (int64_t)gridDim.x * kBlock * kFlagIT) {
+        const int64_t q0 = base + (int64_t)threadIdx.x * kFlagIT;
+        uint32_t k[kFlagIT + 3], o[kFlagIT + 1];
+#pragma unroll
+        for (int j = 0; j < kFlagIT + 3; ++j) {
+            const int64_t q = q0 - 1 + j;
+            k[j] = (q >= 0 && q < n) ? keys[q] : 0u;
+        }
+        unsigned hd = 0, pr = 0, na = 0;
+#pragma unroll
+        for (int j = 0; j < kFlagIT; ++j) {
+            const int64_t q = q0 + j;
+            if (q < n) {
+                const uint32_t row = k[j + 1];
+                const bool first = q == 0 || k[j] != row, last = q + 1 >= n || k[j + 2] != row;
+                na |= (unsigned)!(first && last) << j;
+                hd |= (unsigned)(first && !last) << j;
+                pr |= (unsigned)(recs && first && !last && (q + 2 >= n || k[j + 3] != row)) << j;
+            }
+        }
+#pragma unroll
+        for (int j = 0; j < kFlagIT; ++j) o[j] = (q0 + j < n && (!sparse || ((na >> j) & 1u))) ? perm[q0 + j] : 0u;
+        o[kFlagIT] = ((pr >> (kFlagIT - 1)) & 1u) ? perm[q0 + kFlagIT] : 0u;
+#pragma unroll
+        for (int j = 0; j < kFlagIT; ++j) {
+            const int64_t q = q0 + j;
+            const bool alone = !((na >> j) & 1u);
+            if (q < n && !(sparse && alone)) {
+                const int64_t ob = o[j];
+                const int64_t fi = q < nA ? 4 * ob : (ob < nA ? 4 * ob + 1 : 4 * (ob - nA) + 2);
+                flags[fi] = (uint8_t)alone;
+            }
+        }
+        if (longs_here) {
+#pragma unroll
+            for (int j = 0; j < kFlagIT; ++j) {
+                const int64_t q = q0 + j;
+                if (!((hd >> j) & 1u) || q + kLongSeg >= n) continue;
+                const uint32_t row = k[j + 1];
+                if (keys[q + kLongSeg] != row) continue;
+                const int t = q < nA ? 0 : 1;
+                const int64_t s0 = t ? nA : 0;
+                int64_t lo = q + kLongSeg, hi = t ? n : nA;
+                while (lo + 1 < hi) {
+                    const int64_t mid = (lo + hi) >> 1;
+                    if (keys[mid] == row) lo = mid; else hi = mid;
+                }
+                const int64_t len = hi - q;
+                const unsigned np = (unsigned)((len + kPiece - 1) / kPiece);
+                const unsigned pb = atomicAdd(&r.counters[t][0], np);
+                const unsigned li = atomicAdd(&r.counters[t][1], 1u);
+                r.longs[t][li] = seg_long{q - s0, len, (int64_t)pb};
+                for (unsigned i = 0; i < np; ++i) {
+                    const int64_t st = q + (int64_t)i * kPiece;
+                    r.pieces[t][pb + i] = seg_piece{st - s0, (hi - st) < kPiece ? (hi - st) : (int64_t)kPiece};
+                }
+            }
+        }
+        const int64_t ra = nA - q0;
+        const unsigned mA = ra >= kFlagIT ? 0xFFu : ra <= 0 ? 0u : (1u << (int)ra) - 1u, hh = hd & ~pr;
+        const unsigned bits[NL] = {hh & mA, hh & ~mA, pr & mA, pr & ~mA};
+        unsigned c[NL], p[NL], nd = (unsigned)__popc(na);
+#pragma unroll
+        for (int l = 0; l < NL; ++l) c[l] = p[l] = (unsigned)__popc(bits[l]);
+#pragma unroll
+        for (int d = 1; d < 64; d <<= 1) {
+#pragma unroll
+            for (int l = 0; l < NL; ++l) {
+                const unsigned a = __shfl_up(p[l], d, 64);
+                if (lane >= d) p[l] += a;
+            }
+        }
+        if (stat) {
+#pragma unroll
+            for (int d = 1; d < 64; d <<= 1) nd += __shfl_xor(nd, d, 64);
+        }
+        if (lane == 63) {
+#pragma unroll
+            for (int l = 0; l < NL; ++l) wcnt[l][wave] = p[l];
+            wcnt[NL][wave] = nd;
+        }
+        __syncthreads();
+        if (stat && threadIdx.x == NL) {
+            unsigned tot = 0;
+            for (int w = 0; w < NW; ++w) tot += wcnt[NL][w];
+            if (tot) atomicAdd(&cnt[2], tot);
+        }
+        if (threadIdx.x < NL) {
+            const int t = threadIdx.x;
+            unsigned tot = 0;
+            for (int w = 0; w < NW; ++w) { wbase[t][w] = tot; tot += wcnt[t][w]; }
+            const unsigned b = tot ? atomicAdd(t < 2 ? &cnt[t] : &r.pcnt[t - 2], tot) : 0u;
+            for (int w = 0; w < NW; ++w) wbase[t][w] += b;
+        }
+        __syncthreads();
+        unsigned s[NL];
+#pragma unroll
+        for (int l = 0; l < NL; ++l) s[l] = wbase[l][wave] + p[l] - c[l];
+#pragma unroll
+        for (int j = 0; j < kFlagIT; ++j) {
+            const int64_t q = q0 + j;
+            if (!((hd >> j) & 1u)) continue;
+            if ((pr >> j) & 1u) {
+                const uint4 rec = make_uint4(k[j + 1], o[j], o[j + 1], 0u);
+                if (q < nA) r.pairs[0][s[2]++] = rec; else r.pairs[1][s[3]++] = rec;
+            } else if (q < nA) headsA[s[0]++] = (uint32_t)q;
+            else headsB[s[1]++] = (uint32_t)(q - nA);
         }
         __syncthreads();
     }
@@ -1283,7 +1422,7 @@
     else return (int64_t)perm[e];
 }
 
-template <int LPR, int OPT, bool SIGNED, bool NC = false>
+template <int LPR, int OPT, bool SIGNED, bool NC = false, bool REC = false>
 __device__ __forceinline__ void rowwise_apply_dups_body(float* __restrict__ W, float* __restrict__ Mo, float* __restrict__ Vo,
                                                         int D, const uint32_t* __restrict__ keys,
                                                         const uint32_t* __restrict__ perm, int64_t n,
@@ -1291,7 +1430,9 @@
                                                         const float* __restrict__ G, int64_t neg_start, int64_t reg_limit,
                                                         const float* __restrict__ reg_coef, apply_hp hp,
                                                         unsigned* __restrict__ counters, seg_long* __restrict__ longs,
-                                                        seg_piece* __restrict__ pieces, float* __restrict__ n2 = nullptr) {
+                                                        seg_piece* __restrict__ pieces, float* __restrict__ n2 = nullptr,
+                                                        const uint4* __restrict__ pairs = nullptr, const unsigned* __restrict__ npairs = nullptr,
+                                                        bool scan = true) {
     HP_FROM_DEV(hp);
     const tab_ptrs T{W, Mo, Vo};
     constexpr int GPB = kBlock / LPR;
@@ -1302,6 +1443,46 @@
     const int D4 = D >> 2;
     const float c = reg_coef ? reg_coef[0] : 0.f;
     const int64_t nh = (int64_t)nheads[0];
+    if constexpr (REC) {
+        const bool live = sub < D4;
+        const float4 z4 = make_float4(0.f, 0.f, 0.f, 0.f);
+        const int64_t np = pairs ? (int64_t)npairs[0] : 0;
+        for (int64_t p0 = gg * SU; p0 < np; p0 += TG * SU) {
+            uint4 rec[SU];
+#pragma unroll
+            for (int j = 0; j < SU; ++j) rec[j] = pairs[p0 + j < np ? p0 + j : np - 1];
+            float4 w[SU], m[SU], v[SU], g0[SU], g1[SU];
+            int64_t off[SU];
+#pragma unroll
+            for (int j = 0; j < SU; ++j) {
+                off[j] = (int64_t)rec[j].x * D + 4 * sub;
+                w[j] = m[j] = v[j] = g0[j] = g1[j] = z4;
+                if (p0 + j < np && live) {
+                    w[j] = ld4n<(LPR >= 32)>(W + off[j]);
+                    row_moments<LPR, OPT>(T, off[j], m[j], v[j]);
+                    const bool n0 = SIGNED && (int64_t)rec[j].y >= neg_start, n1 = SIGNED && (int64_t)rec[j].z >= neg_start;
+                    g0[j] = ld4n<(LPR >= 32)>(G + (n0 ? (int64_t)rec[j].y - neg_start : (int64_t)rec[j].y) * D + 4 * sub);
+                    g1[j] = ld4n<(LPR >= 32)>(G + (n1 ? (int64_t)rec[j].z - neg_start : (int64_t)rec[j].z) * D + 4 * sub);
+                }
+            }
+#pragma unroll
+            for (int j = 0; j < SU; ++j) {
+                if (p0 + j >= np) continue;
+                float4 acc = z4;
+                int cnt = 0;
+                const bool n0 = SIGNED && (int64_t)rec[j].y >= neg_start, n1 = SIGNED && (int64_t)rec[j].z >= neg_start;
+                if (n0) { acc.x -= g0[j].x; acc.y -= g0[j].y; acc.z -= g0[j].z; acc.w -= g0[j].w; }
+                else { acc.x += g0[j].x; acc.y += g0[j].y; acc.z += g0[j].z; acc.w += g0[j].w; }
+                cnt += ((int64_t)rec[j].y < reg_limit) ? 1 : 0;
+                if (n1) { acc.x -= g1[j].x; acc.y -= g1[j].y; acc.z -= g1[j].z; acc.w -= g1[j].w; }
+                else { acc.x += g1[j].x; acc.y += g1[j].y; acc.z += g1[j].z; acc.w += g1[j].w; }
+                cnt += ((int64_t)rec[j].z < reg_limit) ? 1 : 0;
+                const float4 wn = upd_math<OPT>(w[j], m[j], v[j], acc, c * (float)cnt, hp);
+                if (live) row_store<LPR, OPT>(T, off[j], wn, m[j], v[j]);
+                if (NC) norm_rec_store<LPR>(n2 + (int64_t)rec[j].x * kNormRecFloats, group_sum<LPR>(sqnorm4<LPR>(wn)), sub);
+            }
+        }
+    }
     if (D4 <= LPR) {
         const bool live = sub < D4;
         const float4 z4 = make_float4(0.f, 0.f, 0.f, 0.f);
@@ -1403,6 +1584,7 @@
         }
     }
     if (counters == nullptr) return;
+    if constexpr (REC) { if (!scan) return; }
     for (int64_t q = (int64_t)blockIdx.x * kBlock + threadIdx.x; q + kLongSeg < n; q += (int64_t)gridDim.x * kBlock) {
         const uint32_t row = keys[q];
         const uint32_t before = keys[q > 0 ? q - 1 : 0];
@@ -1436,6 +1618,14 @@
     const dup_side& t = blockIdx.y ? b : a;
     rowwise_apply_dups_body<LPR, OPT, true, NC>(t.W, t.M, t.V, D, t.keys, t.perm, t.n, t.heads, t.nheads, t.G, t.neg_start, t.reg_limit, t.reg_coef, t.hp,
                                                 t.counters, t.longs, t.pieces, t.n2);
+}
+struct dup_recs { const uint4* pairs; const unsigned* npairs; };
+template <int LPR, int OPT, bool NC = false>
+__global__ __launch_bounds__(kBlock) void rowwise_apply_dups2_rec_kernel(int D, dup_side a, dup_side b, dup_recs ra, dup_recs rb, bool scan) {
+    const dup_side& t = blockIdx.y ? b : a;
+    const dup_recs& r = blockIdx.y ? rb : ra;
+    rowwise_apply_dups_body<LPR, OPT, true, NC, true>(t.W, t.M, t.V, D, t.keys, t.perm, t.n, t.heads, t.nheads, t.G, t.neg_start, t.reg_limit, t.reg_coef, t.hp,
+                                                      t.counters, t.longs, t.pieces, t.n2, r.pairs, r.npairs, scan);
 }
 template <int LPR>
 __global__ __launch_bounds__(kBlock) void seg_piece_sum2_kernel(int D, dup_side a, dup_side b) {
@@ -2123,6 +2313,11 @@
     unsigned* cnt; uint32_t* headsA; uint32_t* headsB;
     heads_view(uint32_t* heads, int64_t n_a) : cnt((unsigned*)heads), headsA(heads + 4), headsB(headsA + (n_a / 2 + 1)) {}
     static int64_t words(int64_t n_a, int64_t n_b) { return 4 + (n_a / 2 + 1) + (n_b / 2 + 1); }
+    static int64_t pair_base(int64_t n_a, int64_t n_b) { return (words(n_a, n_b) + 3) & ~(int64_t)3; }
+    static int64_t words_with_pairs(int64_t n_a, int64_t n_b) { return pair_base(n_a, n_b) + 4 + 4 * ((n_a / 2 + 1) + (n_b / 2 + 1)); }
+    unsigned* pcnt(int64_t n_a, int64_t n_b) const { return cnt + pair_base(n_a, n_b); }
+    uint4* pairsA(int64_t n_a, int64_t n_b) const { return (uint4*)(pcnt(n_a, n_b) + 4); }
+    uint4* pairsB(int64_t n_a, int64_t n_b) const { return pairsA(n_a, n_b) + (n_a / 2 + 1); }
 };
 
 inline size_t count_list_bytes(int64_t B) {
@@ -2244,7 +2439,7 @@
 
 static int sort_two_tables(cdr_ctx* ctx, void* stream, const int64_t* ids_a, int64_t n_a, int64_t rows_a, const int64_t* ids_b0,
                            int64_t n_b0, const int64_t* ids_b1, int64_t n_b1, int64_t rows_b, uint32_t* keys_sorted, uint32_t* perm,
-                           uint32_t* key_base_out, void* workspace, size_t workspace_bytes, sort_clear span_a) {
+                           uint32_t* key_base_out, void* workspace, size_t workspace_bytes, sort_clear span_a, key_extras extras = key_extras{}) {
     const int64_t n = n_a + n_b0 + n_b1;
     CDR_CHECK_ARG(ids_a && n_a > 0 && ids_b0 && n_b0 > 0 && (n_b1 == 0 || ids_b1) && keys_sorted && perm && key_base_out && workspace);
     CDR_CHECK_ARG(rows_a > 0 && rows_b > 0);
@@ -2256,9 +2451,9 @@
             const unsigned places = (bits_for((int64_t)key_base * 2) + kSortRadixBits - 1) / kSortRadixBits;
             const unsigned kgrid = (unsigned)((n + (int64_t)kSortBlock * kSortItems - 1) / ((int64_t)kSortBlock * kSortItems));
             make_keys2_offsets_kernel<<<dim3(kgrid), dim3(kSortBlock), 0, s>>>(ids_a, n_a, ids_b0, n_b0, ids_b1, n_b1, key_base, keys_in, vals_in, z.p, z.words,
-                                                                               (sort_offs_t*)span_a.p, (unsigned*)span_a.p + span_a.words - 32, places);
+                                                                               (sort_offs_t*)span_a.p, (unsigned*)span_a.p + span_a.words - 32, places, extras);
         } else {
-            make_keys2_kernel<<<dim3(grid_for(n, kBlock)), dim3(kBlock), 0, s>>>(ids_a, n_a, ids_b0, n_b0, ids_b1, n_b1, key_base, keys_in, vals_in, z.p, z.words);
+            make_keys2_kernel<<<dim3(grid_for(n, kBlock)), dim3(kBlock), 0, s>>>(ids_a, n_a, ids_b0, n_b0, ids_b1, n_b1, key_base, keys_in, vals_in, z.p, z.words, extras);
         }
     }, span_a.p != nullptr);
     if (rc) return rc;
@@ -2418,17 +2613,14 @@
     template <int L, int OPT> static constexpr auto long_finish = shard_long_finish_kernel<L, OPT>;
 };
 
+inline int dups_grid(int D, const dups_plan& pl) {
+    const int64_t nmax = pl.side[0].n > pl.side[1].n ? pl.side[0].n : pl.side[1].n;
+    return grid_for(nmax / 16 + 1, kBlock / cdr_lpr_for(D));
+}
+
 template <class K>
-int apply_dups_pair(cdr_ctx* ctx, hipStream_t s, int opt, int D, const dups_plan& pl) {
+int apply_long_pair(cdr_ctx* ctx, hipStream_t s, int opt, int D, const dups_plan& pl) {
     const int lpr = cdr_lpr_for(D);
-    const int64_t nmax = pl.side[0].n > pl.side[1].n ? pl.side[0].n : pl.side[1].n;
-    const int grid = grid_for(nmax / 16 + 1, kBlock / lpr);
-    {
-        cdr_time_scope ts(ctx, CDR_TAG_APPLY_SIGNED, s);
-        if constexpr (K::adagrad) DISPATCH_LPR_OPT3(lpr, opt, K::template dups<L, O><<<dim3(grid, 2), dim3(kBlock), 0, s>>>(D, pl.side[0], pl.side[1]));
-        else DISPATCH_LPR_OPT(lpr, opt, K::template dups<L, O><<<dim3(grid, 2), dim3(kBlock), 0, s>>>(D, pl.side[0], pl.side[1]));
-    }
-    CDR_LAUNCH_CHECK();
     if (pl.ls[0].long_cap || pl.ls[1].long_cap) {
         const int64_t pc = pl.ls[0].piece_cap > pl.ls[1].piece_cap ? pl.ls[0].piece_cap : pl.ls[1].piece_cap;
         const int64_t lc = pl.ls[0].long_cap > pl.ls[1].long_cap ? pl.ls[0].long_cap : pl.ls[1].long_cap;
@@ -2443,6 +2635,19 @@
     return CDR_OK;
 }
 
+template <class K>
+int apply_dups_pair(cdr_ctx* ctx, hipStream_t s, int opt, int D, const dups_plan& pl) {
+    const int lpr = cdr_lpr_for(D);
+    const int grid = dups_grid(D, pl);
+    {
+        cdr_time_scope ts(ctx, CDR_TAG_APPLY_SIGNED, s);
+        if constexpr (K::adagrad) DISPATCH_LPR_OPT3(lpr, opt, K::template dups<L, O><<<dim3(grid, 2), dim3(kBlock), 0, s>>>(D, pl.side[0], pl.side[1]));
+        else DISPATCH_LPR_OPT(lpr, opt, K::template dups<L, O><<<dim3(grid, 2), dim3(kBlock), 0, s>>>(D, pl.side[0], pl.side[1]));
+    }
+    CDR_LAUNCH_CHECK();
+    return apply_long_pair<K>(ctx, s, opt, D, pl);
+}
+
 template <class K = table_dups, class Finish>
 int finish_and_apply_dups(cdr_ctx* ctx, hipStream_t s, int opt, int D, const dup_host (&sides)[2], Finish&& finish) {
     dups_plan pl;
@@ -2457,7 +2662,7 @@
 
 extern "C" int cdr_bpr_step_fused_heads_words(int64_t B, int64_t* words) {
     CDR_CHECK_ARG(words && B > 0);
-    *words = heads_view::words(B, 2 * B);
+    *words = heads_view::words_with_pairs(B, 2 * B);
     return CDR_OK;
 }
 
@@ -2478,6 +2683,18 @@
     const bool cached = !count_path && ctx->n2_user && ctx->n2_item && ctx->n2_user_rows == user_rows && ctx->n2_item_rows == item_rows;
     float* NU = cached ? ctx->n2_user : nullptr;
     float* NI = cached ? ctx->n2_item : nullptr;
+    const unsigned dup_mask = count_path ? 0u : ctx->dup_records;
+    CDR_CHECK_ARG(!(dup_mask & kDupPairRecs) || ((uintptr_t)heads & 15) == 0);
+    step_tables T = make_tables(opt, user_tab, user_m, user_v, step_user, opt, item_tab, item_m, item_v, step_item, lr, beta1, beta2, eps, weight_decay);
+    if (hp_dev && opt == 1) { T.hu.dev = hp_dev; T.hi.dev = hp_dev + 2; }
+    const uint32_t kb = two_table_key_base(user_rows, item_rows);
+    dup_host sides[2];
+    make_sides(sides, T, keys, perm, hv, GU, GP, B, 2 * B, B, B, out9 + 4, out9 + 5, kb);
+    sides[0].n2 = NU; sides[1].n2 = NI;
+    dups_plan pl;
+    rc = dups_plan_make(ctx, D, sides, pl);
+    if (rc) return rc;
+    const bool longs_here = (dup_mask & kDupLongHere) && (pl.side[0].counters || pl.side[1].counters);
     if (count_path) {
         const unsigned hb = two_table_bits(user_rows, item_rows);
         CDR_CHECK_ARG(hb < 31);
@@ -2505,18 +2722,28 @@
         CDR_LAUNCH_CHECK();
     } else {
         static const bool keys_make_offsets = [] { const char* e = getenv("CDR_OWN_SORT"); return !(e && e[0] == '1'); }();
-        const uint32_t kb = two_table_key_base(user_rows, item_rows);
         const sort_clear span_a = keys_make_offsets && kb ? own_sort_span_a(3 * B, (int64_t)kb * 2, sort_ws, sort_ws_bytes) : sort_clear{nullptr, 0};
         rc = embloss_head(ctx, s, user_tab, item_tab, D, uid, pid, B, B, 1, reg_weight, out9, hv.cnt, step_user_dev, step_item_dev, hp_dev, lr, beta1, beta2,
                           NU, NI, span_a);
         if (rc) return rc;
-        rc = sort_two_tables(ctx, stream, uid, B, user_rows, pid, B, nid, B, item_rows, keys, perm, &key_base, sort_ws, sort_ws_bytes, span_a);
+        key_extras extras{};
+        if (dup_mask & kDupSparseFlags) { extras.fill = (uint32_t*)flags; extras.fwords = B; }
+        if (dup_mask & kDupPairRecs) extras.zero[0] = hv.pcnt(B, 2 * B);
+        if (longs_here) { extras.zero[1] = pl.side[0].counters; extras.zero[2] = pl.side[1].counters; }
+        rc = sort_two_tables(ctx, stream, uid, B, user_rows, pid, B, nid, B, item_rows, keys, perm, &key_base, sort_ws, sort_ws_bytes, span_a, extras);
         if (rc) return rc;
-        rc = occ_flags(ctx, s, keys, perm, B, 3 * B, 4, flags, hv, B <= kCountMaxB);
-        if (rc) return rc;
-    }
-    step_tables T = make_tables(opt, user_tab, user_m, user_v, step_user, opt, item_tab, item_m, item_v, step_item, lr, beta1, beta2, eps, weight_decay);
-    if (hp_dev && opt == 1) { T.hu.dev = hp_dev; T.hi.dev = hp_dev + 2; }
+        if (dup_mask) {
+            const occ_recs r{{hv.pairsA(B, 2 * B), hv.pairsB(B, 2 * B)}, hv.pcnt(B, 2 * B), {pl.side[0].counters, pl.side[1].counters},
+                             {pl.side[0].longs, pl.side[1].longs}, {pl.side[0].pieces, pl.side[1].pieces}, longs_here ? dup_mask : dup_mask & ~kDupLongHere};
+            cdr_time_scope ts(ctx, CDR_TAG_OCC_FLAGS, s);
+            occ_flags_sparse_kernel<<<dim3(grid_for(3 * B, kBlock * kFlagIT)), dim3(kBlock), 0, s>>>(keys, perm, B, 3 * B, flags, hv.headsA, hv.headsB, hv.cnt,
+                                                                                                  B <= kCountMaxB, r);
+            CDR_LAUNCH_CHECK();
+        } else {
+            rc = occ_flags(ctx, s, keys, perm, B, 3 * B, 4, flags, hv, B <= kCountMaxB);
+            if (rc) return rc;
+        }
+    }
     static const int un = [] { const char* e = getenv("CDR_FWD_APPLY_UN"); return (e && e[0] == '2') ? 2 : 1; }();
     const int grid = grid_for((B + un - 1) / un, kBlock / lpr);
     {
@@ -2530,13 +2757,22 @@
         });
     }
     CDR_LAUNCH_CHECK();
-    dup_host sides[2];
-    make_sides(sides, T, keys, perm, hv, GU, GP, B, 2 * B, B, B, out9 + 4, out9 + 5, key_base);
-    sides[0].n2 = NU; sides[1].n2 = NI;
-    auto finish = [&](unsigned* za, unsigned* zb) {
-        step_finish_keep_kernel<<<dim3(1), dim3(kBlock), 0, s>>>(ctx->partials, grid, B, reg_weight, out9, za, zb);
-    };
-    return cached ? finish_and_apply_dups<table_dups_nc>(ctx, s, opt, D, sides, finish) : finish_and_apply_dups(ctx, s, opt, D, sides, finish);
+    step_finish_keep_kernel<<<dim3(1), dim3(kBlock), 0, s>>>(ctx->partials, grid, B, reg_weight, out9, longs_here ? nullptr : pl.side[0].counters,
+                                                             longs_here ? nullptr : pl.side[1].counters);
+    CDR_LAUNCH_CHECK();
+    if (!dup_mask) return cached ? apply_dups_pair<table_dups_nc>(ctx, s, opt, D, pl) : apply_dups_pair<table_dups>(ctx, s, opt, D, pl);
+    {
+        const bool pairs = (dup_mask & kDupPairRecs) != 0;
+        const dup_recs ra{pairs ? hv.pairsA(B, 2 * B) : nullptr, hv.pcnt(B, 2 * B)}, rb{pairs ? hv.pairsB(B, 2 * B) : nullptr, hv.pcnt(B, 2 * B) + 1};
+        const int dgrid = dups_grid(D, pl);
+        cdr_time_scope ts(ctx, CDR_TAG_APPLY_SIGNED, s);
+        DISPATCH_LPR_OPT3(lpr, opt, {
+            auto kern = cached ? rowwise_apply_dups2_rec_kernel<L, O, true> : rowwise_apply_dups2_rec_kernel<L, O>;
+            kern<<<dim3(dgrid, 2), dim3(kBlock), 0, s>>>(D, pl.side[0], pl.side[1], ra, rb, !longs_here);
+        });
+    }
+    CDR_LAUNCH_CHECK();
+    return cached ? apply_long_pair<table_dups_nc>(ctx, s, opt, D, pl) : apply_long_pair<table_dups>(ctx, s, opt, D, pl);
 }
 
 extern "C" int cdr_norm_rec_floats(void) { return kNormRecFloats; }
```

Result: no change. 583.3 million interactions/s, median of 6 (+0.3%).
